# Nishad-Sharma/gpuRaytracer

Measured on AMD Instinct MI355X. Metric: Msamples/sec (pixels×spp) Cornell box 1080p at 1/2/4/8 MI355X; HBM GB/s, higher is better.
Workload: dtype f32; 1 GPU; cornell_1920x1080_256spp_b3; width=1920, height=1080, spp_per_gpu=256, spp_frame=256, bounces=3, parallelism=single GPU

## Files before the change

### gpuraytracer_amd/_native.py

```python
from __future__ import annotations

import ctypes
import os

ABI_VERSION = 11
_HERE = os.path.dirname(os.path.abspath(__file__))
library_path = os.environ.get("RTPT_LIB") or os.path.join(_HERE, "librtpt.so")


class float3(ctypes.Structure):

    _fields_ = [("x", ctypes.c_float), ("y", ctypes.c_float), ("z", ctypes.c_float),
                ("_pad", ctypes.c_float)]

    def __iter__(self):
        return iter((self.x, self.y, self.z))


class float4(ctypes.Structure):
    _fields_ = [("x", ctypes.c_float), ("y", ctypes.c_float), ("z", ctypes.c_float),
                ("w", ctypes.c_float)]


class int2(ctypes.Structure):
    _fields_ = [("x", ctypes.c_int32), ("y", ctypes.c_int32)]


class MaterialGPU(ctypes.Structure):
    _fields_ = [("diffuse", float4), ("metallic", ctypes.c_float),
                ("roughness", ctypes.c_float), ("_pad", ctypes.c_float * 2),
                ("emissive", float3)]


class SphereGPU(ctypes.Structure):
    _fields_ = [("center", float3), ("material", MaterialGPU), ("radius", ctypes.c_float),
                ("_pad", ctypes.c_float * 3)]


class CameraGPU(ctypes.Structure):
    _fields_ = [("position", float3), ("direction", float3), ("up", float3),
                ("resolution", int2), ("horizontalFov", ctypes.c_float),
                ("ev100", ctypes.c_float)]


class SquareLightGPU(ctypes.Structure):
    _fields_ = [("center", float3), ("color", float4), ("emittedRadiance", float3),
                ("width", ctypes.c_float), ("depth", ctypes.c_float),
                ("_pad", ctypes.c_float * 2)]


for _t, _n in ((float3, 16), (MaterialGPU, 48), (SphereGPU, 80), (CameraGPU, 64),
               (SquareLightGPU, 64)):
    assert ctypes.sizeof(_t) == _n, (_t.__name__, ctypes.sizeof(_t))
assert MaterialGPU.emissive.offset == 32 and SphereGPU.radius.offset == 64
assert CameraGPU.resolution.offset == 48 and CameraGPU.horizontalFov.offset == 56
assert SquareLightGPU.width.offset == 48


class SceneDesc(ctypes.Structure):
    _fields_ = [("camera", ctypes.POINTER(CameraGPU)),
                ("materials", ctypes.POINTER(MaterialGPU)),
                ("square_lights", ctypes.POINTER(SquareLightGPU)),
                ("n_square_lights", ctypes.c_uint32),
                ("vertices", ctypes.POINTER(float3)),
                ("n_triangles", ctypes.c_uint32),
                ("spheres", ctypes.POINTER(SphereGPU)),
                ("n_spheres", ctypes.c_uint32),
                ("device", ctypes.c_int32)]


class RenderParamsC(ctypes.Structure):
    _fields_ = [(n, ctypes.c_uint32) for n in
                ("spp", "bounces", "sample_base", "row_start", "row_step", "row_count",
                 "accumulate", "flags")]


class SceneInfo(ctypes.Structure):
    _fields_ = [(n, ctypes.c_uint32) for n in
                ("n_triangles", "n_triangle_pairs", "n_spheres", "lds_bytes",
                 "n_sphere_nodes", "n_triangle_bvh_nodes", "n_box_clusters", "pair_free_mask",
                 "sphere_kernel_lds_bytes", "kernel_layout", "kernel_lds_bytes")]


class CreateOptions(ctypes.Structure):
    _fields_ = [("scene_layout", ctypes.c_uint32), ("lanes_per_pixel", ctypes.c_uint32),
                ("tri_bvh_build", ctypes.c_uint32), ("tri_leaf_max", ctypes.c_uint32),
                ("tri_leaf_cost", ctypes.c_float), ("sphere_leaf_max", ctypes.c_uint32),
                ("sphere_median", ctypes.c_uint32), ("walk_scheduler", ctypes.c_uint32),
                ("walk_leaf_den", ctypes.c_uint32), ("reserved", ctypes.c_uint32 * 7)]


assert ctypes.sizeof(CreateOptions) == 64

LAYOUTS = {"auto": 0, "pairs": 1, "single": 2, "global": 3, "smem": 3, "pairsmem": 4, "sorted": 5, "bvh": 6}
TRI_BUILDS = {"default": 0, "host": 1, "lbvh": 2, "gpusah": 3}
WALKS = {"auto": 0, "lockstep": 1, "free": 2, "sorted": 3}

RT_OK = 0
RT_OUT_DEVICE, RT_OUT_FP16, RT_OUT_NONE, RT_KEEP_SUM, RT_OUT_RGBA8 = 0x1, 0x2, 0x4, 0x8, 0x10
RT_RAYS_ANY, RT_RAYS_EXACT = 0x100, 0x200
RT_AOV_CENTER = 0x400
RT_RAYS_CHUNK = 2048
RT_MAX_BOUNCES = 4
RT_COMM_ID_BYTES = 128
STATUS = {0: "RT_OK", 1: "RT_ERR_INVALID_ARG", 2: "RT_ERR_NO_DEVICE", 3: "RT_ERR_OUT_OF_MEMORY",
          4: "RT_ERR_LAUNCH", 5: "RT_ERR_STATE", 6: "RT_ERR_COMM"}

class LaunchInfo(ctypes.Structure):
    _fields_ = [("kernel", ctypes.c_char * 96)] + [(n, ctypes.c_uint32) for n in
                ("lanes_per_pixel", "halton_tables", "small_index", "block_threads", "grid_x",
                 "grid_y", "lds_bytes")]

    def as_dict(self) -> dict:
        d = {k: getattr(self, k) for k, _ in self._fields_}
        d["kernel"] = self.kernel.decode()
        return d


class BuildStats(ctypes.Structure):
    _fields_ = [("tri_bvh_build", ctypes.c_uint32), ("tri_bvh_nodes", ctypes.c_uint32),
                ("tri_bvh_build_ms", ctypes.c_float), ("scene_compile_ms", ctypes.c_float),
                ("tri_bvh_temp_kib", ctypes.c_uint32)]


class TriBvhDump(ctypes.Structure):
    _fields_ = [("n_triangles", ctypes.c_uint32), ("nodes_per_layout", ctypes.c_uint32),
                ("leaf_max", ctypes.c_uint32), ("margin", ctypes.c_float),
                ("nodes", ctypes.c_void_p), ("sorted", ctypes.c_void_p),
                ("perm", ctypes.c_void_p), ("isect", ctypes.c_void_p)]


assert ctypes.sizeof(TriBvhDump) == 48


class TileLayout(ctypes.Structure):
    _fields_ = [("rows", ctypes.c_uint32), ("rows_max", ctypes.c_uint32),
                ("row_bytes", ctypes.c_uint64), ("tile_bytes", ctypes.c_uint64)]


class Ray(ctypes.Structure):
    _fields_ = [("origin", ctypes.c_float * 3), ("tmin", ctypes.c_float),
                ("dir", ctypes.c_float * 3), ("tmax", ctypes.c_float)]


class RayHit(ctypes.Structure):
    _fields_ = [("t", ctypes.c_float), ("id", ctypes.c_int32)]


class RayDomainInfo(ctypes.Structure):
    _fields_ = [(n, ctypes.c_float) for n in ("origin_max", "dir_len2_min", "dir_len2_max", "tmax_max")]


assert ctypes.sizeof(Ray) == 32 and ctypes.sizeof(RayHit) == 8 and Ray.dir.offset == 16


class AovParams(ctypes.Structure):
    _fields_ = [(n, ctypes.c_uint32) for n in
                ("spp", "sample_base", "row_start", "row_step", "row_count", "flags")]


class AovBuffers(ctypes.Structure):
    _fields_ = [("albedo", ctypes.c_void_p), ("normal_depth", ctypes.c_void_p),
                ("first_hit", ctypes.c_void_p)]


assert ctypes.sizeof(AovParams) == 24 and ctypes.sizeof(AovBuffers) == 24


class MisParamsC(ctypes.Structure):
    _fields_ = [(n, ctypes.c_uint32) for n in
                ("camera_rays", "mis_samples", "row_start", "row_step", "row_count", "flags")]


_P = ctypes.c_void_p
SIGNATURES = {
    "rt_create": (ctypes.c_int, [ctypes.POINTER(SceneDesc), ctypes.POINTER(_P)]),
    "rt_create_ex": (ctypes.c_int, [ctypes.POINTER(SceneDesc), ctypes.POINTER(CreateOptions),
                                    ctypes.POINTER(_P)]),
    "rt_create_options_default": (None, [ctypes.POINTER(CreateOptions)]),
    "rt_set_seeds": (ctypes.c_int, [_P, _P, ctypes.c_int32, ctypes.c_int32]),
    "rt_fill_seeds": (ctypes.c_int, [_P, ctypes.c_uint64]),
    "rt_render": (ctypes.c_int, [_P, ctypes.POINTER(RenderParamsC), _P]),
    "rt_render_async": (ctypes.c_int, [_P, ctypes.POINTER(RenderParamsC), _P, _P]),
    "rt_trace_rays": (ctypes.c_int, [_P, _P, ctypes.c_uint64, ctypes.c_uint32, _P]),
    "rt_trace_rays_async": (ctypes.c_int, [_P, _P, ctypes.c_uint64, ctypes.c_uint32, _P, _P]),
    "rt_render_aov": (ctypes.c_int, [_P, ctypes.POINTER(AovParams), ctypes.POINTER(AovBuffers)]),
    "rt_render_aov_async": (ctypes.c_int, [_P, ctypes.POINTER(AovParams), ctypes.POINTER(AovBuffers), _P]),
    "rt_debug_ray_domain": (ctypes.c_int, [ctypes.POINTER(SceneDesc), ctypes.POINTER(RayDomainInfo)]),
    "rt_last_kernel_ms": (ctypes.c_int, [_P, ctypes.POINTER(ctypes.c_float)]),
    "rt_destroy": (ctypes.c_int, [_P]),
    "rt_last_launch": (ctypes.c_int, [_P, ctypes.POINTER(LaunchInfo)]),
    "rt_build_info": (ctypes.c_int, [_P, ctypes.POINTER(BuildStats)]),
    "rt_debug_tri_bvh": (ctypes.c_int, [_P, ctypes.POINTER(TriBvhDump)]),
    "rt_debug_tri_bvh_host": (ctypes.c_int, [ctypes.POINTER(SceneDesc), ctypes.POINTER(CreateOptions),
                                             ctypes.POINTER(TriBvhDump)]),
    "rt_math_selfcheck": (ctypes.c_int, [ctypes.POINTER(ctypes.c_uint64)]),
    "rt_comm_unique_id": (ctypes.c_int, [_P]),
    "rt_comm_init": (ctypes.c_int, [_P, ctypes.c_int32, ctypes.c_int32, _P]),
    "rt_render_gather": (ctypes.c_int, [_P, ctypes.POINTER(RenderParamsC), _P, _P]),
    "rt_comm_info": (ctypes.c_int, [_P, ctypes.POINTER(ctypes.c_int32), ctypes.POINTER(ctypes.c_int32)]),
    "rt_tile_layout": (ctypes.c_int, [ctypes.c_int32, ctypes.c_int32, ctypes.c_int32, ctypes.c_int32,
                                      ctypes.c_uint32, ctypes.POINTER(TileLayout)]),
    "rt_place_tiles": (ctypes.c_int, [_P, _P, ctypes.c_int32, ctypes.c_uint32, _P, _P]),
    "rt_place_tiles_host": (ctypes.c_int, [_P, ctypes.c_int32, ctypes.c_int32, ctypes.c_int32,
                                           ctypes.c_uint32, _P]),
    "rt_build_sha": (ctypes.c_char_p, []),
    "rt_debug_stats": (ctypes.c_int, [_P, _P, ctypes.c_int]),
    "rt_last_error": (ctypes.c_char_p, [_P]),
    "rt_status_string": (ctypes.c_char_p, [ctypes.c_int]),
    "rt_abi_version": (ctypes.c_int, []),
    "rt_seed_splitmix": (None, [ctypes.c_uint64, _P, ctypes.c_size_t]),
    "rt_scene_cornell_box": (ctypes.c_int, [ctypes.c_int32, ctypes.c_int32,
                                            ctypes.POINTER(CameraGPU),
                                            ctypes.POINTER(MaterialGPU),
                                            ctypes.POINTER(float3),
                                            ctypes.POINTER(SquareLightGPU),
                                            ctypes.POINTER(ctypes.c_uint32)]),
    "rt_scene_random_spheres": (ctypes.c_int, [ctypes.c_int32, ctypes.c_int32, ctypes.c_uint32,
                                               ctypes.c_uint64, ctypes.POINTER(CameraGPU),
                                               ctypes.POINTER(MaterialGPU),
                                               ctypes.POINTER(float3),
                                               ctypes.POINTER(SquareLightGPU),
                                               ctypes.POINTER(ctypes.c_uint32),
                                               ctypes.POINTER(SphereGPU)]),
    "rt_render_mis": (ctypes.c_int, [_P, ctypes.POINTER(MisParamsC), _P, _P]),
    "rt_scene_cornell_box_mis": (ctypes.c_int, [ctypes.c_int32, ctypes.c_int32,
                                                ctypes.POINTER(CameraGPU),
                                                ctypes.POINTER(MaterialGPU),
                                                ctypes.POINTER(float3),
                                                ctypes.POINTER(SquareLightGPU),
                                                ctypes.POINTER(ctypes.c_uint32)]),
    "rt_tonemap_rgba8": (None, [_P, ctypes.c_size_t, _P]),
    "rt_scene_describe": (ctypes.c_int, [ctypes.POINTER(SceneDesc), ctypes.POINTER(SceneInfo)]),
    "rt_scene_describe_ex": (ctypes.c_int, [ctypes.POINTER(SceneDesc), ctypes.POINTER(CreateOptions),
                                            ctypes.POINTER(SceneInfo)]),
    "rt_debug_camera_candidates": (ctypes.c_int, [ctypes.POINTER(SceneDesc)] + [ctypes.c_int32] * 4 + [_P]),
    "rt_debug_shadow_candidates": (ctypes.c_int, [ctypes.POINTER(SceneDesc)] + [ctypes.c_int32] * 4 +
                                   [_P, ctypes.POINTER(ctypes.c_int32)]),
    "rt_debug_cluster_kinds": (ctypes.c_int, [ctypes.POINTER(SceneDesc), ctypes.POINTER(ctypes.c_uint32),
                                              ctypes.c_uint32, ctypes.POINTER(ctypes.c_uint32)]),
    "rt_debug_light_mask": (ctypes.c_int, [ctypes.POINTER(SceneDesc), ctypes.POINTER(ctypes.c_uint64), _P,
                                           ctypes.c_uint32]),
}


class RtError(RuntimeError):

    def __init__(self, status: int, message: str):
        super().__init__(f"{STATUS.get(status, status)}: {message}")
        self.status = status


def _preload_hip_runtime():
    if os.environ.get("RTPT_SYSTEM_HIP") == "1":
        return
    import importlib.util
    spec = importlib.util.find_spec("torch")
    if spec is None or not spec.submodule_search_locations:
        return
    for d in spec.submodule_search_locations:
        cand = os.path.join(d, "lib", "libamdhip64.so")
        if os.path.exists(cand):
            ctypes.CDLL(cand, mode=ctypes.RTLD_GLOBAL)
            return


def _load():
    if not os.path.exists(library_path):
        raise ImportError(
            f"{library_path} is missing: build the HIP extension first "
            "(`make` or `python -c 'import __graft_entry__ as g; g.build()'`). "
            "There is no CPU fallback.")
    _preload_hip_runtime()
    handle = ctypes.CDLL(library_path)
    for name, (res, args) in SIGNATURES.items():
        fn = getattr(handle, name)
        fn.restype = res
        fn.argtypes = args
    if handle.rt_abi_version() != ABI_VERSION:
        raise ImportError(f"librtpt.so ABI {handle.rt_abi_version()} != {ABI_VERSION}")
    if not os.environ.get("RTPT_LIB"):
        from .srchash import have_sources, kernel_source_sha
        built = handle.rt_build_sha().decode()
        if not have_sources() or built == "unknown":
            import warnings
            warnings.warn(f"{library_path}: source hash not checked (library hash {built!r}, "
                          f"sources {'present' if have_sources() else 'absent'})")
        elif built != kernel_source_sha():
            raise ImportError(f"{library_path} was built from other sources (hash {built}, "
                              f"tree {kernel_source_sha()}): rebuild it with `make`")
    return handle


lib = _load()
```

### gpuraytracer_amd/csrc/rt_api.cpp

```cpp
#include <hip/hip_runtime.h>
#include <rccl/rccl.h>

#include <stdio.h>
#include <stdlib.h>
#include <string.h>

#include <algorithm>
#include <chrono>
#include <new>
#include <string>
#include <vector>

#include "../../include/rtpt.h"
#include "rt_beam.hpp"
#include "rt_shaft.hpp"
#include "rt_kernel.hpp"
#include "rt_scene.hpp"

constexpr uint32_t kDefaultTriBuild = RT_TRI_BVH_GPU_SAH;

struct rt_ctx {
    int device = 0;
    hipStream_t stream = nullptr;
    rt::CompiledScene scene;
    float4* d_tri_isect = nullptr;
    float4* d_tri_shade = nullptr;
    float4* d_pair_isect = nullptr;
    float4* d_clusters = nullptr;
    uint32_t* d_sph_lds = nullptr;
    uint16_t* d_sph_lds_id = nullptr;
    uint4* d_sph_box = nullptr;
    float4* d_sph_isect = nullptr;
    float4* d_sph_shade = nullptr;
    float4* d_sph_nodes = nullptr;
    uint32_t* d_sph_perm = nullptr;
    uint4* d_tri_nodes = nullptr;
    uint32_t tri_build = kDefaultTriBuild;
    float4* d_tri_sorted = nullptr;
    uint32_t* d_tri_perm = nullptr;
    uint32_t tri_bvh_nodes = 0;
    rt::SceneTables tab{};
    bool sph_compact = false;
    uint64_t light_mask = 0;
    uint32_t tri_bvh_build_used = 0;
    uint32_t tri_leaf_max = 1;
    float tri_bvh_build_ms = 0.0f;
    size_t tri_bvh_temp_bytes = 0;
    float scene_compile_ms = 0.0f;
    float4* d_mis_shade = nullptr;
    float4* d_mis_tab = nullptr;
    uint32_t mis_tab_S = 0;
    void* d_out8 = nullptr;
    size_t out8_cap = 0;
    void* d_rays = nullptr;
    size_t rays_cap = 0;
    void* d_hits = nullptr;
    size_t hits_cap = 0;
    void* d_aov[3] = {nullptr, nullptr, nullptr};
    size_t aov_cap[3] = {0, 0, 0};
    void* d_mis_part = nullptr;
    size_t mis_part_cap = 0;
    uint32_t* d_seeds = nullptr;
    bool seeds_ready = false;
    uint32_t seed_max = 0xFFFFFFFFu;
    float4* d_sum = nullptr;
    size_t sum_cap = 0;
    bool sum_valid = false;
    uint32_t sum_row_start = 0, sum_row_step = 0, sum_row_count = 0;
    uint32_t sum_first = 0, sum_samples = 0;
    void* d_out = nullptr;
    size_t out_cap = 0;
    hipEvent_t ev0 = nullptr, ev1 = nullptr;
    bool timed = false;
    rt::LaunchInfo launch{};
    bool launched = false;
    ncclComm_t comm = nullptr;
    int rank = 0, world = 1;
    void* d_tile = nullptr;
    size_t tile_cap = 0;
    void* d_gather = nullptr;
    size_t gather_cap = 0;
    hipEvent_t ev_tiles = nullptr;
    bool tiles_pending = false;
    uint32_t lanes = 0;
    rt::SceneMem scene_mem = rt::SceneMem::kAuto;
    uint32_t walk = 0;
    uint32_t walk_leaf_den = 0;
    std::string err;
};

namespace {

thread_local std::string g_create_err = "no error";

int fail(rt_ctx* ctx, int status, const std::string& msg) {
    if (ctx)
        ctx->err = msg;
    else
        g_create_err = msg;
    return status;
}

int hip_fail(rt_ctx* ctx, int status, const char* what, hipError_t e) {
    return fail(ctx, status, std::string(what) + ": " + hipGetErrorString(e));
}

struct DeviceGuard {
    int prev = -1;
    explicit DeviceGuard(int dev) {
        if (hipGetDevice(&prev) != hipSuccess) prev = -1;
        if (prev != dev) (void)hipSetDevice(dev);
    }
    ~DeviceGuard() {
        int cur = -1;
        if (prev >= 0 && hipGetDevice(&cur) == hipSuccess && cur != prev) (void)hipSetDevice(prev);
    }
};

template <typename T>
hipError_t upload(T** dptr, const void* src, size_t bytes, hipStream_t s) {
    *dptr = nullptr;
    if (bytes == 0) return hipSuccess;
    hipError_t e = hipMalloc((void**)dptr, bytes);
    if (e != hipSuccess) return e;
    e = hipMemcpyAsync(*dptr, src, bytes, hipMemcpyHostToDevice, s);
    if (e != hipSuccess) return e;
    return hipStreamSynchronize(s);
}

rt::SceneTables scene_tables(const rt::CompiledScene& s, uint32_t nTN, const rt_ctx* c) {
    rt::SceneTables t{};
    t.nT = (uint32_t)s.tri_isect.size();
    t.nP = (uint32_t)s.pair_isect.size();
    t.nS = (uint32_t)s.sph_isect.size();
    t.nN = s.sph_layout_nodes;
    t.nTN = nTN;
    t.nC = (uint32_t)(s.clusters.size() / (4 * rt::kCluF4));
    t.pair_free = s.pair_free_mask;
    if (!c) return t;
    t.tri_isect = c->d_tri_isect;
    t.pair_isect = c->d_pair_isect;
    t.clusters = c->d_clusters;
    t.sph_isect = c->d_sph_isect;
    t.sph_nodes = c->d_sph_nodes;
    t.sph_perm = c->d_sph_perm;
    t.sph_box = rt::sphere_compact_usable(s) ? c->d_sph_box : nullptr;
    t.tri_nodes = c->d_tri_nodes;
    t.tri_sorted = c->d_tri_sorted;
    t.tri_perm = c->d_tri_perm;
    return t;
}

void set_tables(rt::KParams* K, const rt::SceneTables& t) {
    K->tri_isect = t.tri_isect;
    K->pair_isect = t.pair_isect;
    K->clusters = t.clusters;
    K->sph_isect = t.sph_isect;
    K->sph_nodes = t.sph_nodes;
    K->sph_perm = t.sph_perm;
    K->sph_box = t.sph_box;
    K->tri_nodes = t.tri_nodes;
    K->tri_sorted = t.tri_sorted;
    K->tri_perm = t.tri_perm;
    K->nT = t.nT;
    K->nP = t.nP;
    K->nS = t.nS;
    K->nN = t.nN;
    K->nTN = t.nTN;
    K->nC = t.nC;
    K->pair_free = t.pair_free;
}

void release(rt_ctx* c) {
    if (!c) return;
    DeviceGuard g(c->device);
    if (c->tiles_pending) (void)hipEventSynchronize(c->ev_tiles);
    (void)hipFree(c->d_tri_isect);
    (void)hipFree(c->d_tri_shade);
    (void)hipFree(c->d_pair_isect);
    (void)hipFree(c->d_clusters);
    (void)hipFree(c->d_sph_lds);
    (void)hipFree(c->d_sph_lds_id);
    (void)hipFree(c->d_sph_box);
    (void)hipFree(c->d_sph_isect);
    (void)hipFree(c->d_sph_shade);
    (void)hipFree(c->d_sph_nodes);
    (void)hipFree(c->d_sph_perm);
    (void)hipFree(c->d_tri_nodes);
    (void)hipFree(c->d_tri_sorted);
    (void)hipFree(c->d_tri_perm);
    (void)hipFree(c->d_mis_shade);
    (void)hipFree(c->d_mis_tab);
    (void)hipFree(c->d_out8);
    (void)hipFree(c->d_mis_part);
    (void)hipFree(c->d_rays);
    (void)hipFree(c->d_hits);
    for (void* b : c->d_aov) (void)hipFree(b);
    (void)hipFree(c->d_seeds);
    (void)hipFree(c->d_sum);
    (void)hipFree(c->d_out);
    if (c->comm) (void)ncclCommDestroy(c->comm);
    (void)hipFree(c->d_tile);
    (void)hipFree(c->d_gather);
    if (c->ev_tiles) (void)hipEventDestroy(c->ev_tiles);
    if (c->ev0) (void)hipEventDestroy(c->ev0);
    if (c->ev1) (void)hipEventDestroy(c->ev1);
    if (c->stream) (void)hipStreamDestroy(c->stream);
}

bool resolve_rows(const rt_ctx* c, const rt_render_params* p, uint32_t* start, uint32_t* step,
                  uint32_t* count) {
    const uint32_t H = (uint32_t)c->scene.cam.H;
    *start = p->row_start;
    *step = p->row_step ? p->row_step : 1u;
    if (*start >= H) return false;
    const uint32_t avail = (H - 1u - *start) / *step + 1u;
    *count = p->row_count ? p->row_count : avail;
    return *count <= avail;
}

int render_impl(rt_ctx* c, const rt_render_params* p, void* out, bool out_is_device,
                hipStream_t stream, bool sync) {
    if (!p) return fail(c, RT_ERR_INVALID_ARG, "params is null");
    if (p->bounces > RT_MAX_BOUNCES)
        return fail(c, RT_ERR_INVALID_ARG,
                    "bounces > 4: Halton dimensions would leave primes[24] (sampling.metal:97)");
    if (!c->seeds_ready) return fail(c, RT_ERR_STATE, "seeds not set (rt_set_seeds/rt_fill_seeds)");
    uint32_t start, step, count;
    if (!resolve_rows(c, p, &start, &step, &count))
        return fail(c, RT_ERR_INVALID_ARG, "row partition outside the frame");
    const bool want_out = !(p->flags & RT_OUT_NONE);
    const bool keep_sum = (p->flags & RT_KEEP_SUM) != 0;
    if (want_out && !out) return fail(c, RT_ERR_INVALID_ARG, "out is null");
    if (p->accumulate) {
        if (!c->sum_valid || c->sum_row_start != start || c->sum_row_step != step ||
            c->sum_row_count != count ||
            (uint64_t)c->sum_first + c->sum_samples != (uint64_t)p->sample_base)
            return fail(c, RT_ERR_STATE,
                        "accumulate: context sum does not end at sample_base for these rows "
                        "(render with RT_KEEP_SUM first)");
    }
    const uint64_t total = (uint64_t)(p->accumulate ? c->sum_samples : 0u) + p->spp;
    if (total == 0 || total > 0xFFFFFFFFull)
        return fail(c, RT_ERR_INVALID_ARG, "samples in the sum must be in [1, 2^32)");

    const size_t W = (size_t)c->scene.cam.W;
    const size_t pixels = (size_t)count * W;
    if ((p->flags & RT_OUT_FP16) && (p->flags & RT_OUT_RGBA8))
        return fail(c, RT_ERR_INVALID_ARG, "RT_OUT_FP16 and RT_OUT_RGBA8 are exclusive");
    const size_t px_bytes = (p->flags & RT_OUT_RGBA8) ? 4u : (p->flags & RT_OUT_FP16) ? 8u : 16u;
    hipError_t e;
    if (keep_sum || p->accumulate) {
        if (c->sum_cap < pixels) {
            (void)hipFree(c->d_sum);
            c->d_sum = nullptr;
            c->sum_cap = 0;
            c->sum_valid = false;
            if ((e = hipMalloc((void**)&c->d_sum, pixels * sizeof(float4))) != hipSuccess)
                return hip_fail(c, RT_ERR_OUT_OF_MEMORY, "hipMalloc(sum)", e);
            c->sum_cap = pixels;
        }
    }
    void* kout = nullptr;
    if (want_out) {
        if (out_is_device) {
            kout = out;
        } else {
            if (c->out_cap < pixels * px_bytes) {
                (void)hipFree(c->d_out);
                c->d_out = nullptr;
                c->out_cap = 0;
                if ((e = hipMalloc(&c->d_out, pixels * px_bytes)) != hipSuccess)
                    return hip_fail(c, RT_ERR_OUT_OF_MEMORY, "hipMalloc(out staging)", e);
                c->out_cap = pixels * px_bytes;
            }
            kout = c->d_out;
        }
    }

    rt::KParams K;
    memset(&K, 0, sizeof(K));
    set_tables(&K, c->tab);
    K.tri_shade = c->d_tri_shade;
    K.light_mask = c->light_mask;
    K.sph_lds = c->sph_compact ? c->d_sph_lds : nullptr;
    K.sph_lds_id = c->d_sph_lds_id;
    K.sph_shade = c->d_sph_shade;
    K.seeds = c->d_seeds;
    K.sum = (keep_sum || p->accumulate) ? c->d_sum : nullptr;
    K.out = kout;
    K.nE = c->scene.sph_lds_entries;
    const rt::CamConst& cam = c->scene.cam;
    memcpy(K.cam_pos, cam.pos, sizeof(K.cam_pos));
    memcpy(K.cam_u, cam.u, sizeof(K.cam_u));
    memcpy(K.cam_v, cam.v, sizeof(K.cam_v));
    memcpy(K.cam_w, cam.w, sizeof(K.cam_w));
    K.halfW = cam.halfW;
    K.halfH = cam.halfH;
    K.W = cam.W;
    K.H = cam.H;
    memcpy(K.light_center, c->scene.light.center, sizeof(K.light_center));
    {
        uint32_t by, bz;
        memcpy(&by, &K.light_center[1], 4);
        memcpy(&bz, &K.light_center[2], 4);
        K.light_plain = (by != 0x80000000u && bz != 0x80000000u) ? 1u : 0u;
    }
    memcpy(K.light_color, c->scene.light.color, sizeof(K.light_color));
    K.spp = p->spp;
    K.sample_base = p->sample_base;
    K.row_start = start;
    K.row_step = step;
    K.row_count = count;
    K.accumulate = p->accumulate ? 1u : 0u;
    K.samples_total = (uint32_t)total;
    K.flags = ((p->flags & RT_OUT_FP16) ? rt::kOutFp16 : 0u) | ((p->flags & RT_OUT_RGBA8) ? rt::kOutRgba8 : 0u);
    K.lanes = c->lanes;
    K.walk = c->walk;
    K.walk_leaf_den = c->walk_leaf_den;
    {
        const uint64_t imax = (uint64_t)c->seed_max + p->sample_base + (p->spp ? p->spp - 1u : 0u);
        K.max_index = imax > 0xFFFFFFFFull ? 0xFFFFFFFFu : (uint32_t)imax;
    }

    if (keep_sum && !p->accumulate) c->sum_valid = false;
    (void)hipEventRecord(c->ev0, stream);
    e = rt::launch_path_trace(K, p->bounces, c->scene_mem, stream, &c->launch);
    if (e != hipSuccess) return hip_fail(c, RT_ERR_LAUNCH, "path_trace launch", e);
    c->launched = true;
    (void)hipEventRecord(c->ev1, stream);
    c->timed = true;
    if (keep_sum || p->accumulate) {
        c->sum_valid = true;
        c->sum_row_start = start;
        c->sum_row_step = step;
        c->sum_row_count = count;
        if (!p->accumulate) c->sum_first = p->sample_base;
        c->sum_samples = (uint32_t)total;
    }
    if (want_out && !out_is_device) {
        if ((e = hipMemcpyAsync(out, kout, pixels * px_bytes, hipMemcpyDeviceToHost, stream)) !=
            hipSuccess)
            return hip_fail(c, RT_ERR_LAUNCH, "hipMemcpyAsync(out)", e);
    }
    if (sync) {
        if ((e = hipStreamSynchronize(stream)) != hipSuccess)
            return hip_fail(c, RT_ERR_LAUNCH, "path_trace execution", e);
        uint32_t short_end = 0;
        if (rt::lds_check_result(&short_end) == hipSuccess && short_end)
            return fail(c, RT_ERR_LAUNCH, "LDS overflow: staged records end at byte " + std::to_string(short_end) +
                                              ", past the dispatch's dynamic LDS");
    }
    return RT_OK;
}

int ensure_staging(rt_ctx* c, void** buf, size_t* cap, size_t bytes, const char* what);

int nccl_fail(rt_ctx* ctx, const char* what, ncclResult_t r) {
    return fail(ctx, RT_ERR_COMM, std::string(what) + ": " + ncclGetErrorString(r));
}

size_t pixel_bytes(uint32_t flags) {
    return (flags & RT_OUT_RGBA8) ? 4u : (flags & RT_OUT_FP16) ? 8u : 16u;
}

struct TileLayout {
    uint32_t rows, rows_max;
    size_t row_bytes, tile_bytes;
};

TileLayout tile_layout(uint32_t W, uint32_t H, uint32_t N, uint32_t rank, uint32_t flags) {
    TileLayout L;
    L.rows = rank < H ? (H - 1u - rank) / N + 1u : 0u;
    L.rows_max = (H + N - 1u) / N;
    L.row_bytes = (size_t)W * pixel_bytes(flags);
    L.tile_bytes = (size_t)L.rows_max * L.row_bytes;
    return L;
}

bool tile_args_ok(int32_t W, int32_t H, int32_t N) { return W > 0 && H > 0 && N > 0; }

int place_tiles_impl(rt_ctx* c, const void* gathered, uint32_t N, uint32_t flags, void* frame,
                     hipStream_t stream) {
    const uint32_t W = (uint32_t)c->scene.cam.W, H = (uint32_t)c->scene.cam.H;
    const TileLayout L = tile_layout(W, H, N, 0, flags);
    const bool dev = (flags & RT_OUT_DEVICE) != 0;
    const size_t frame_bytes = (size_t)H * L.row_bytes;
    void* dst = frame;
    int st;
    if (!dev) {
        if ((st = ensure_staging(c, &c->d_out, &c->out_cap, frame_bytes, "hipMalloc(frame staging)")) != RT_OK)
            return st;
        dst = c->d_out;
    }
    hipError_t e = rt::launch_place_tiles(gathered, dst, L.row_bytes, L.tile_bytes, H, N, stream);
    if (e != hipSuccess) return hip_fail(c, RT_ERR_LAUNCH, "place_tiles launch", e);
    if (!dev) {
        if ((e = hipStreamSynchronize(stream)) != hipSuccess ||
            (e = hipMemcpyAsync(frame, dst, frame_bytes, hipMemcpyDeviceToHost, stream)) != hipSuccess ||
            (e = hipStreamSynchronize(stream)) != hipSuccess)
            return hip_fail(c, RT_ERR_LAUNCH, "frame copy to host", e);
    }
    return RT_OK;
}

int render_gather_impl(rt_ctx* c, const rt_render_params* p, void* frame, hipStream_t stream) {
    if (!p) return fail(c, RT_ERR_INVALID_ARG, "params is null");
    if (!c->comm) return fail(c, RT_ERR_STATE, "no communicator (rt_comm_init)");
    if (p->row_start || p->row_step > 1 || p->row_count)
        return fail(c, RT_ERR_INVALID_ARG, "rt_render_gather partitions the rows itself: "
                                           "params must name the whole frame (row_start 0, "
                                           "row_step 0 or 1, row_count 0)");
    if ((p->flags & RT_OUT_FP16) && (p->flags & RT_OUT_RGBA8))
        return fail(c, RT_ERR_INVALID_ARG, "RT_OUT_FP16 and RT_OUT_RGBA8 are exclusive");
    const bool want_out = !(p->flags & RT_OUT_NONE);
    const bool dev = (p->flags & RT_OUT_DEVICE) != 0;
    if (want_out && c->rank == 0 && !frame) return fail(c, RT_ERR_INVALID_ARG, "frame is null on rank 0");
    const uint32_t H = (uint32_t)c->scene.cam.H, W = (uint32_t)c->scene.cam.W, N = (uint32_t)c->world;
    const TileLayout L = tile_layout(W, H, N, (uint32_t)c->rank, p->flags);
    hipError_t e;
    if (c->tiles_pending && (e = hipStreamWaitEvent(stream, c->ev_tiles, 0)) != hipSuccess)
        return hip_fail(c, RT_ERR_LAUNCH, "hipStreamWaitEvent(previous gather)", e);
    int st;
    if (want_out && (st = ensure_staging(c, &c->d_tile, &c->tile_cap, L.tile_bytes, "hipMalloc(tile)")) != RT_OK)
        return st;
    if (L.rows > 0) {
        rt_render_params q = *p;
        q.row_start = (uint32_t)c->rank;
        q.row_step = N;
        q.row_count = L.rows;
        q.flags = p->flags | RT_OUT_DEVICE;
        if ((st = render_impl(c, &q, c->d_tile, true, stream, false)) != RT_OK) return st;
    }
    if (!want_out) return RT_OK;
    if (c->rank == 0 && (st = ensure_staging(c, &c->d_gather, &c->gather_cap, L.tile_bytes * N,
                                             "hipMalloc(gather)")) != RT_OK)
        return st;
// ... 348 lines not shown

int rt_abi_version(void) { return RTPT_ABI_VERSION; }

const char* rt_status_string(int s) {
    switch (s) {
        case RT_OK: return "RT_OK";
        case RT_ERR_INVALID_ARG: return "RT_ERR_INVALID_ARG";
        case RT_ERR_NO_DEVICE: return "RT_ERR_NO_DEVICE";
        case RT_ERR_OUT_OF_MEMORY: return "RT_ERR_OUT_OF_MEMORY";
        case RT_ERR_LAUNCH: return "RT_ERR_LAUNCH";
        case RT_ERR_STATE: return "RT_ERR_STATE";
        case RT_ERR_COMM: return "RT_ERR_COMM";
        default: return "RT_ERR_UNKNOWN";
    }
}

const char* rt_last_error(const rt_ctx* ctx) {
    return ctx ? ctx->err.c_str() : g_create_err.c_str();
}

int rt_create(const rt_scene_desc* d, rt_ctx** out_ctx) { return rt_create_ex(d, nullptr, out_ctx); }

int rt_create_ex(const rt_scene_desc* d, const rt_create_options* opt, rt_ctx** out_ctx) {
    if (!out_ctx) return fail(nullptr, RT_ERR_INVALID_ARG, "out_ctx is null");
    *out_ctx = nullptr;
    if (!d) return fail(nullptr, RT_ERR_INVALID_ARG, "scene desc is null");
    if (!d->camera) return fail(nullptr, RT_ERR_INVALID_ARG, "camera is null");
    if (!d->square_lights || d->n_square_lights < 1)
        return fail(nullptr, RT_ERR_INVALID_ARG, "square_lights[0] is required (raytrace.metal:22)");
    Resolved ro;
    const char* why = nullptr;
    if (!resolve_options(opt, &ro, &why)) return fail(nullptr, RT_ERR_INVALID_ARG, why);
    int count = 0;
    hipError_t e = hipGetDeviceCount(&count);
    if (e != hipSuccess || count <= 0)
        return fail(nullptr, RT_ERR_NO_DEVICE,
                    std::string("no HIP device: ") + (e != hipSuccess ? hipGetErrorString(e) : "count 0"));
    if (d->device < 0 || d->device >= count)
        return fail(nullptr, RT_ERR_NO_DEVICE, "device ordinal out of range");

    rt_ctx* c = new (std::nothrow) rt_ctx();
    if (!c) return fail(nullptr, RT_ERR_OUT_OF_MEMORY, "host allocation");
    c->device = d->device;
    c->lanes = ro.lanes;
    c->tri_build = ro.tri_build;
    c->scene_mem = ro.mem;
    c->walk = ro.walk;
    c->walk_leaf_den = ro.walk_leaf_den;
    DeviceGuard g(c->device);
    const char* err = nullptr;
    using clk = std::chrono::steady_clock;
    const auto t_compile = clk::now();
    if (!rt::compile_scene(*d->camera, d->materials, d->vertices, d->n_triangles,
                           d->square_lights[0], d->spheres, d->n_spheres, &c->scene, &err, ro.build)) {
        delete c;
        return fail(nullptr, RT_ERR_INVALID_ARG, err);
    }
    c->scene_compile_ms = std::chrono::duration<float, std::milli>(clk::now() - t_compile).count();
    int status = RT_OK;
    std::string msg;
    do {
        if ((e = hipStreamCreateWithFlags(&c->stream, hipStreamNonBlocking)) != hipSuccess) {
            status = RT_ERR_NO_DEVICE; msg = std::string("hipStreamCreate: ") + hipGetErrorString(e); break;
        }
        if ((e = hipEventCreate(&c->ev0)) != hipSuccess || (e = hipEventCreate(&c->ev1)) != hipSuccess ||
            (e = hipEventCreateWithFlags(&c->ev_tiles, hipEventDisableTiming)) != hipSuccess) {
            status = RT_ERR_NO_DEVICE; msg = std::string("hipEventCreate: ") + hipGetErrorString(e); break;
        }
        const rt::CompiledScene& s = c->scene;
        if ((e = upload(&c->d_tri_isect, s.tri_isect.data(), s.tri_isect.size() * sizeof(rt::TriIsect), c->stream)) != hipSuccess ||
            (e = upload(&c->d_tri_shade, s.tri_shade.data(), s.tri_shade.size() * sizeof(rt::TriShade), c->stream)) != hipSuccess ||
            (e = upload(&c->d_pair_isect, s.pair_isect.data(), s.pair_isect.size() * sizeof(rt::PairIsect), c->stream)) != hipSuccess ||
            (e = upload(&c->d_clusters, s.clusters.data(), s.clusters.size() * sizeof(float), c->stream)) != hipSuccess ||
            (e = upload(&c->d_sph_lds, s.sph_lds.data(), s.sph_lds.size() * sizeof(uint32_t), c->stream)) != hipSuccess ||
            (e = upload(&c->d_sph_lds_id, s.sph_lds_id.data(), s.sph_lds_id.size() * sizeof(uint16_t), c->stream)) != hipSuccess ||
            (e = upload(&c->d_sph_box, s.sph_box.data(), s.sph_box.size() * sizeof(uint32_t), c->stream)) != hipSuccess ||
            (e = upload(&c->d_sph_isect, s.sph_isect.data(), s.sph_isect.size() * sizeof(rt::SphIsect), c->stream)) != hipSuccess ||
            (e = upload(&c->d_sph_shade, s.sph_shade.data(), s.sph_shade.size() * sizeof(rt::SphShade), c->stream)) != hipSuccess ||
            (e = upload(&c->d_sph_nodes, s.sph_nodes.data(), s.sph_nodes.size() * sizeof(rt::BvhNode), c->stream)) != hipSuccess ||
            (e = upload(&c->d_sph_perm, s.sph_perm.data(), s.sph_perm.size() * sizeof(uint32_t), c->stream)) != hipSuccess ||
            (e = upload(&c->d_mis_shade, s.mis_shade.data(), s.mis_shade.size() * sizeof(rt::MisShade), c->stream)) != hipSuccess) {
            status = RT_ERR_OUT_OF_MEMORY; msg = std::string("scene upload: ") + hipGetErrorString(e); break;
        }
        const uint32_t nT = (uint32_t)s.tri_isect.size();
        const size_t lds_pairs = rt::kernel_lds_bytes(nT, (uint32_t)s.pair_isect.size(), 0, 0);
        const size_t lds_single = rt::kernel_lds_bytes(nT, 0, 0, 0);
        const bool need_bvh = nT > 0 && (c->scene_mem == rt::SceneMem::kTriBvh ||
                                         (c->scene_mem == rt::SceneMem::kAuto &&
                                          (nT > rt::kTriBvhMinTriangles ||
                                           std::min(lds_pairs, lds_single) > rt::kMaxLdsBytes)));
        if (need_bvh) {
            const size_t nn = 2 * (size_t)nT - 1;
            const auto t_build = clk::now();
            if (c->tri_build == RT_TRI_BVH_GPU_SAH) {
                if ((e = hipMalloc((void**)&c->d_tri_nodes, rt::kTriCompactLayouts * nn * sizeof(uint4))) != hipSuccess ||
                    (e = hipMalloc((void**)&c->d_tri_sorted, 3 * (size_t)nT * sizeof(float4))) != hipSuccess ||
                    (e = hipMalloc((void**)&c->d_tri_perm, (size_t)nT * sizeof(uint32_t))) != hipSuccess) {
                    status = RT_ERR_OUT_OF_MEMORY; msg = std::string("hipMalloc(triangle BVH): ") + hipGetErrorString(e); break;
                }
                uint32_t total = 0;
                size_t temp = 0;
                if ((e = rt::build_tri_gsah(c->d_tri_isect, nT, s.margin, ro.tri_leaf_max, ro.tri_leaf_cost,
                                            c->d_tri_nodes, c->d_tri_sorted, c->d_tri_perm, &total, &temp,
                                            c->stream)) != hipSuccess) {
                    status = (e == hipErrorInvalidValue) ? RT_ERR_INVALID_ARG
                             : (e == hipErrorOutOfMemory) ? RT_ERR_OUT_OF_MEMORY : RT_ERR_LAUNCH;
                    msg = std::string("triangle BVH build: ") + hipGetErrorString(e); break;
                }
                c->tri_bvh_nodes = total;
                c->tri_bvh_temp_bytes = temp;
            } else if (c->tri_build == RT_TRI_BVH_GPU_LBVH) {
                if ((e = hipMalloc((void**)&c->d_tri_nodes, rt::kTriCompactLayouts * nn * sizeof(uint4))) != hipSuccess ||
                    (e = hipMalloc((void**)&c->d_tri_sorted, 3 * (size_t)nT * sizeof(float4))) != hipSuccess ||
                    (e = hipMalloc((void**)&c->d_tri_perm, (size_t)nT * sizeof(uint32_t))) != hipSuccess) {
                    status = RT_ERR_OUT_OF_MEMORY; msg = std::string("hipMalloc(triangle BVH): ") + hipGetErrorString(e); break;
                }
                if ((e = rt::build_tri_lbvh(c->d_tri_isect, nT, s.tri_lo, s.tri_hi, s.margin, c->d_tri_nodes,
                                            c->d_tri_sorted, c->d_tri_perm, c->stream)) != hipSuccess) {
                    status = (e == hipErrorInvalidValue) ? RT_ERR_INVALID_ARG : RT_ERR_LAUNCH;
                    msg = std::string("triangle BVH build: ") + hipGetErrorString(e); break;
                }
            } else {
                std::vector<uint32_t> nodes, perm;
                std::vector<rt::TriIsect> sorted;
                if (!rt::build_tri_sah(s.tri_isect, s.margin, &nodes, &sorted, &perm, ro.tri_leaf_max,
                                       ro.tri_leaf_cost)) {
                    status = RT_ERR_INVALID_ARG; msg = "triangle BVH build: too many triangles (2^24)"; break;
                }
                if ((e = upload(&c->d_tri_nodes, nodes.data(), nodes.size() * sizeof(uint32_t), c->stream)) != hipSuccess ||
                    (e = upload(&c->d_tri_sorted, sorted.data(), sorted.size() * sizeof(rt::TriIsect), c->stream)) != hipSuccess ||
                    (e = upload(&c->d_tri_perm, perm.data(), perm.size() * sizeof(uint32_t), c->stream)) != hipSuccess) {
                    status = RT_ERR_OUT_OF_MEMORY; msg = std::string("triangle BVH upload: ") + hipGetErrorString(e); break;
                }
                c->tri_bvh_nodes = (uint32_t)(nodes.size() / (4 * rt::kTriCompactLayouts));
            }
            if (c->tri_build == RT_TRI_BVH_GPU_LBVH) c->tri_bvh_nodes = (uint32_t)nn;
            c->tri_leaf_max = c->tri_build == RT_TRI_BVH_GPU_LBVH ? 1u : std::min(128u, std::max(1u, ro.tri_leaf_max));
            c->tri_bvh_build_used = c->tri_build;
            c->tri_bvh_build_ms = std::chrono::duration<float, std::milli>(clk::now() - t_build).count();
        }
        const size_t npx = (size_t)s.cam.W * (size_t)s.cam.H;
        if ((e = hipMalloc((void**)&c->d_seeds, npx * sizeof(uint32_t))) != hipSuccess) {
            status = RT_ERR_OUT_OF_MEMORY; msg = std::string("hipMalloc(seeds): ") + hipGetErrorString(e); break;
        }
    } while (0);
    if (status != RT_OK) {
        release(c);
        delete c;
        return fail(nullptr, status, msg);
    }
    c->sph_compact = rt::sphere_compact_usable(c->scene);
    c->tab = scene_tables(c->scene, c->tri_bvh_nodes, c);
    c->light_mask = rt::light_mask(c->scene);
    *out_ctx = c;
    return RT_OK;
}

int rt_set_seeds(rt_ctx* c, const uint32_t* seeds, int32_t width, int32_t height) {
    if (!c) return fail(nullptr, RT_ERR_INVALID_ARG, "ctx is null");
    if (!seeds) return fail(c, RT_ERR_INVALID_ARG, "seeds is null");
    if (width != c->scene.cam.W || height != c->scene.cam.H)
        return fail(c, RT_ERR_INVALID_ARG, "seed texture size must equal the camera resolution");
    DeviceGuard g(c->device);
    const size_t bytes = (size_t)width * (size_t)height * sizeof(uint32_t);
    hipError_t e = hipMemcpyAsync(c->d_seeds, seeds, bytes, hipMemcpyHostToDevice, c->stream);
    if (e == hipSuccess) e = hipStreamSynchronize(c->stream);
    if (e != hipSuccess) return hip_fail(c, RT_ERR_LAUNCH, "seed upload", e);
    uint32_t mx = 0;
    for (size_t k = 0, n = (size_t)width * (size_t)height; k < n; ++k) mx = seeds[k] > mx ? seeds[k] : mx;
    c->seed_max = mx;
    c->seeds_ready = true;
    return RT_OK;
}

int rt_fill_seeds(rt_ctx* c, uint64_t key) {
    if (!c) return fail(nullptr, RT_ERR_INVALID_ARG, "ctx is null");
    DeviceGuard g(c->device);
    const uint64_t n = (uint64_t)c->scene.cam.W * (uint64_t)c->scene.cam.H;
    hipError_t e = rt::launch_fill_seeds(c->d_seeds, key, n, c->stream);
    if (e == hipSuccess) e = hipStreamSynchronize(c->stream);
    if (e != hipSuccess) return hip_fail(c, RT_ERR_LAUNCH, "fill_seeds", e);
    c->seed_max = 0xFFFFFu;
    c->seeds_ready = true;
    return RT_OK;
}

int rt_render(rt_ctx* c, const rt_render_params* p, void* out) {
    if (!c) return fail(nullptr, RT_ERR_INVALID_ARG, "ctx is null");
    DeviceGuard g(c->device);
    const bool dev = p && (p->flags & RT_OUT_DEVICE);
    return render_impl(c, p, out, dev, c->stream, true);
}

int rt_render_async(rt_ctx* c, const rt_render_params* p, void* out_device, void* hip_stream) {
    if (!c) return fail(nullptr, RT_ERR_INVALID_ARG, "ctx is null");
    DeviceGuard g(c->device);
    return render_impl(c, p, out_device, true, (hipStream_t)hip_stream, false);
}

int rt_trace_rays(rt_ctx* c, const rt_ray* rays, uint64_t n, uint32_t flags, rt_ray_hit* hits) {
    if (!c) return fail(nullptr, RT_ERR_INVALID_ARG, "ctx is null");
    DeviceGuard g(c->device);
    return trace_rays_impl(c, rays, n, flags, hits, (flags & RT_OUT_DEVICE) != 0, c->stream, true);
}

int rt_trace_rays_async(rt_ctx* c, const rt_ray* rays_dev, uint64_t n, uint32_t flags, rt_ray_hit* hits_dev,
                        void* hip_stream) {
    if (!c) return fail(nullptr, RT_ERR_INVALID_ARG, "ctx is null");
    DeviceGuard g(c->device);
    return trace_rays_impl(c, rays_dev, n, flags, hits_dev, true, (hipStream_t)hip_stream, false);
}

int rt_render_aov(rt_ctx* c, const rt_aov_params* p, const rt_aov_buffers* b) {
    if (!c) return fail(nullptr, RT_ERR_INVALID_ARG, "ctx is null");
    DeviceGuard g(c->device);
    return render_aov_impl(c, p, b, p && (p->flags & RT_OUT_DEVICE), c->stream, true);
}

int rt_render_aov_async(rt_ctx* c, const rt_aov_params* p, const rt_aov_buffers* b_dev, void* hip_stream) {
    if (!c) return fail(nullptr, RT_ERR_INVALID_ARG, "ctx is null");
    DeviceGuard g(c->device);
    return render_aov_impl(c, p, b_dev, true, (hipStream_t)hip_stream, false);
}

int rt_debug_ray_domain(const rt_scene_desc* d, rt_ray_domain_info* info) {
    if (!d || !info || !d->camera || !d->square_lights)
        return fail(nullptr, RT_ERR_INVALID_ARG, "null argument");
    rt::CompiledScene s;
    const char* err = nullptr;
    if (!rt::compile_scene(*d->camera, d->materials, d->vertices, d->n_triangles, d->square_lights[0],
                           d->spheres, d->n_spheres, &s, &err))
        return fail(nullptr, RT_ERR_INVALID_ARG, err);
    const rt::RayDomain D = rt::ray_domain(s.extent);
    info->origin_max = D.origin_max;
    info->dir_len2_min = D.dir_len2_min;
    info->dir_len2_max = D.dir_len2_max;
    info->tmax_max = D.tmax_max;
    return RT_OK;
}

int rt_last_kernel_ms(rt_ctx* c, float* ms) {
    if (!c || !ms) return fail(c, RT_ERR_INVALID_ARG, "null argument");
    if (!c->timed) return fail(c, RT_ERR_STATE, "no render or ray query yet");
    DeviceGuard g(c->device);
    hipError_t e = hipEventSynchronize(c->ev1);
    if (e == hipSuccess) e = hipEventElapsedTime(ms, c->ev0, c->ev1);
    if (e != hipSuccess) return hip_fail(c, RT_ERR_LAUNCH, "hipEventElapsedTime", e);
    return RT_OK;
}

int rt_comm_unique_id(uint8_t id[RT_COMM_ID_BYTES]) {
    if (!id) return fail(nullptr, RT_ERR_INVALID_ARG, "id is null");
    static_assert(sizeof(ncclUniqueId) == RT_COMM_ID_BYTES, "ncclUniqueId size");
    ncclUniqueId u;
    const ncclResult_t r = ncclGetUniqueId(&u);
    if (r != ncclSuccess) return nccl_fail(nullptr, "ncclGetUniqueId", r);
    memcpy(id, &u, sizeof(u));
    return RT_OK;
}

int rt_comm_init(rt_ctx* c, int32_t rank, int32_t world, const uint8_t id[RT_COMM_ID_BYTES]) {
    if (!c) return fail(nullptr, RT_ERR_INVALID_ARG, "ctx is null");
    if (!id) return fail(c, RT_ERR_INVALID_ARG, "id is null");
    if (world < 1 || rank < 0 || rank >= world)
        return fail(c, RT_ERR_INVALID_ARG, "need 0 <= rank < world");
    if (c->comm) return fail(c, RT_ERR_STATE, "context already has a communicator");
    DeviceGuard g(c->device);
    ncclUniqueId u;
    memcpy(&u, id, sizeof(u));
    ncclComm_t comm = nullptr;
    const ncclResult_t r = ncclCommInitRank(&comm, world, u, rank);
    if (r != ncclSuccess) return nccl_fail(c, "ncclCommInitRank", r);
    c->comm = comm;
    c->rank = rank;
    c->world = world;
    return RT_OK;
}

int rt_render_gather(rt_ctx* c, const rt_render_params* p, void* frame, void* hip_stream) {
    if (!c) return fail(nullptr, RT_ERR_INVALID_ARG, "ctx is null");
    DeviceGuard g(c->device);
    hipStream_t s = (hipStream_t)hip_stream;
    return render_gather_impl(c, p, frame, s);
}

int rt_comm_info(const rt_ctx* c, int32_t* count, int32_t* rank) {
    if (!c || !count || !rank) return fail(nullptr, RT_ERR_INVALID_ARG, "null argument");
    rt_ctx* m = const_cast<rt_ctx*>(c);
    if (!c->comm) return fail(m, RT_ERR_STATE, "rt_comm_info: no communicator (rt_comm_init first)");
    int n = 0, r = 0;
    ncclResult_t res = ncclCommCount(c->comm, &n);
    if (res != ncclSuccess) return nccl_fail(m, "ncclCommCount", res);
    res = ncclCommUserRank(c->comm, &r);
    if (res != ncclSuccess) return nccl_fail(m, "ncclCommUserRank", res);
    *count = n;
    *rank = r;
    return RT_OK;
}

int rt_tile_layout(int32_t width, int32_t height, int32_t world, int32_t rank, uint32_t flags,
                   rt_tile_layout_info* out) {
    if (!out || !tile_args_ok(width, height, world) || rank < 0 || rank >= world)
        return RT_ERR_INVALID_ARG;
    const TileLayout L = tile_layout((uint32_t)width, (uint32_t)height, (uint32_t)world, (uint32_t)rank, flags);
    out->rows = L.rows;
    out->rows_max = L.rows_max;
// ... 111 lines not shown
    info->halton_tables = c->launch.tables;
    info->small_index = c->launch.small;
    info->block_threads = c->launch.threads;
    info->grid_x = c->launch.grid_x;
    info->grid_y = c->launch.grid_y;
    info->lds_bytes = c->launch.lds;
    return RT_OK;
}

#ifndef RT_SRC_SHA
#define RT_SRC_SHA "unknown"
#endif
const char* rt_build_sha(void) { return RT_SRC_SHA; }

int rt_destroy(rt_ctx* c) {
    if (!c) return RT_OK;
    release(c);
    delete c;
    return RT_OK;
}

int rt_scene_describe(const rt_scene_desc* d, rt_scene_info* info) {
    return rt_scene_describe_ex(d, nullptr, info);
}

int rt_scene_describe_ex(const rt_scene_desc* d, const rt_create_options* opt, rt_scene_info* info) {
    if (!d || !info || !d->camera || !d->square_lights)
        return fail(nullptr, RT_ERR_INVALID_ARG, "null argument");
    Resolved ro;
    const char* why = nullptr;
    if (!resolve_options(opt, &ro, &why)) return fail(nullptr, RT_ERR_INVALID_ARG, why);
    rt::CompiledScene s;
    const char* err = nullptr;
    if (!rt::compile_scene(*d->camera, d->materials, d->vertices, d->n_triangles,
                           d->square_lights[0], d->spheres, d->n_spheres, &s, &err, ro.build))
        return fail(nullptr, RT_ERR_INVALID_ARG, err);
    rt::SceneTables t = scene_tables(s, 0, nullptr);
    info->n_triangles = t.nT;
    info->n_triangle_pairs = t.nP;
    info->n_box_clusters = t.nC;
    info->pair_free_mask = t.pair_free;
    info->n_spheres = t.nS;
    info->n_sphere_nodes = t.nN;
    const size_t lds = rt::kernel_lds_bytes(info->n_triangles, info->n_triangle_pairs, info->n_spheres,
                                            s.sph_layout_nodes);
    const size_t lds_single = rt::kernel_lds_bytes(info->n_triangles, 0, 0, 0);
    const bool bvh = info->n_triangles > 0 &&
                     (ro.mem == rt::SceneMem::kTriBvh ||
                      (ro.mem == rt::SceneMem::kAuto && (info->n_triangles > rt::kTriBvhMinTriangles ||
                                                         std::min(lds, lds_single) > rt::kMaxLdsBytes)));
    info->n_triangle_bvh_nodes = t.nTN = bvh ? 2 * info->n_triangles - 1 : 0u;
    info->sphere_kernel_lds_bytes = (rt::sphere_compact_usable(s) && info->n_triangle_pairs > 0 && !bvh &&
                                     ro.mem == rt::SceneMem::kAuto && lds <= rt::kSphPairLdsMaxBytes)
                                        ? (uint32_t)lds
                                        : 0u;
    const size_t lds_clu =
        lds + (t.nS ? 0u : 16 * rt::staged_f4<size_t>(rt::kLayPairClu, t.nT, t.nP, t.nC).clu);
    info->lds_bytes = (!bvh && lds <= rt::kMaxLdsBytes)
                          ? (uint32_t)(lds_clu <= rt::kMaxLdsBytes ? lds_clu : lds)
                          : 0u;
    const rt::KernelChoice kc = rt::choose_kernel(t, rt::sphere_compact_usable(s), 3, ro.mem, ro.walk);
    info->kernel_layout = (uint32_t)kc.layout;
    info->kernel_lds_bytes = (uint32_t)kc.lds_bytes;
    return RT_OK;
}

int rt_debug_camera_candidates(const rt_scene_desc* d, int32_t x0, int32_t x1, int32_t y0, int32_t y1,
                               uint8_t* may_hit) {
    if (!d || !may_hit || !d->camera || !d->square_lights || x1 < x0 || y1 < y0 || x0 < 0 || y0 < 0)
        return fail(nullptr, RT_ERR_INVALID_ARG, "null argument or empty rectangle");
    rt::CompiledScene s;
    const char* err = nullptr;
    if (!rt::compile_scene(*d->camera, d->materials, d->vertices, d->n_triangles, d->square_lights[0],
                           d->spheres, d->n_spheres, &s, &err))
        return fail(nullptr, RT_ERR_INVALID_ARG, err);
    memset(may_hit, 1, d->n_triangles);
    const rt::CamConst& c = s.cam;
    const rt::Beam beam = rt::make_beam(rt::f3{c.pos[0], c.pos[1], c.pos[2]}, rt::f3{c.u[0], c.u[1], c.u[2]},
                                        rt::f3{c.v[0], c.v[1], c.v[2]}, rt::f3{c.w[0], c.w[1], c.w[2]}, c.halfW,
                                        c.halfH, (float)c.W, (float)c.H, (float)(uint32_t)x0, (float)(uint32_t)x1,
                                        (float)(uint32_t)y0, (float)(uint32_t)y1);
    for (size_t k = 0; k < s.pair_isect.size(); ++k)
        if (rt::beam_excludes_pair(beam, s.pair_isect[k].q)) may_hit[2 * k] = may_hit[2 * k + 1] = 0;
    return RT_OK;
}

int rt_debug_shadow_candidates(const rt_scene_desc* d, int32_t x0, int32_t x1, int32_t y0, int32_t y1,
                               uint8_t* may_occlude, int32_t* available) {
    if (!d || !may_occlude || !available || !d->camera || !d->square_lights || x1 < x0 || y1 < y0 || x0 < 0 ||
        y0 < 0)
        return fail(nullptr, RT_ERR_INVALID_ARG, "null argument or empty rectangle");
    rt::CompiledScene s;
    const char* err = nullptr;
    if (!rt::compile_scene(*d->camera, d->materials, d->vertices, d->n_triangles, d->square_lights[0],
                           d->spheres, d->n_spheres, &s, &err))
        return fail(nullptr, RT_ERR_INVALID_ARG, err);
    memset(may_occlude, 1, d->n_triangles);
    *available = 0;
    const size_t nP = s.pair_isect.size();
    if (nP == 0) return RT_OK;
    const rt::CamConst& c = s.cam;
    const rt::Beam beam = rt::make_beam(rt::f3{c.pos[0], c.pos[1], c.pos[2]}, rt::f3{c.u[0], c.u[1], c.u[2]},
                                        rt::f3{c.v[0], c.v[1], c.v[2]}, rt::f3{c.w[0], c.w[1], c.w[2]}, c.halfW,
                                        c.halfH, (float)c.W, (float)c.H, (float)(uint32_t)x0, (float)(uint32_t)x1,
                                        (float)(uint32_t)y0, (float)(uint32_t)y1);
    const rt::ShaftLight L = rt::shaft_light(rt::f3{s.light.center[0], s.light.center[1], s.light.center[2]});
    std::vector<uint8_t> keep(nP, 0);
    bool ok = true;
    for (size_t k = 0; k < nP; ++k) {
        if (rt::beam_excludes_pair(beam, s.pair_isect[k].q)) continue;
        for (int tb = 0; tb < 2; ++tb) {
            const float* sh = s.tri_shade[2 * k + tb].s;
            if (sh[3] != 0.0f) continue;
            const rt::ShaftSrc S = rt::shaft_source(beam, s.pair_isect[k].q, tb, rt::f3{sh[0], sh[1], sh[2]}, L);
            ok = ok && S.ok;
            for (size_t j = 0; j < nP; ++j)
                if (!rt::shaft_excludes_pair(S, L, s.pair_isect[j].q)) keep[j] = 1;
        }
    }
    if (!ok) return RT_OK;
    *available = 1;
    for (size_t j = 0; j < nP; ++j) may_occlude[2 * j] = may_occlude[2 * j + 1] = keep[j];
    return RT_OK;
}

int rt_debug_cluster_kinds(const rt_scene_desc* d, uint32_t* flags, uint32_t capacity, uint32_t* n_clusters) {
    if (!d || !n_clusters || (!flags && capacity) || !d->camera || !d->square_lights)
        return fail(nullptr, RT_ERR_INVALID_ARG, "null argument");
    rt::CompiledScene s;
    const char* err = nullptr;
    if (!rt::compile_scene(*d->camera, d->materials, d->vertices, d->n_triangles, d->square_lights[0],
                           d->spheres, d->n_spheres, &s, &err))
        return fail(nullptr, RT_ERR_INVALID_ARG, err);
    const size_t rec = 4 * rt::kCluF4, nC = s.clusters.size() / rec;
    *n_clusters = (uint32_t)nC;
    for (size_t c = 0; c < nC && c < capacity; ++c) memcpy(&flags[c], &s.clusters[c * rec + 15], 4);
    return RT_OK;
}

int rt_debug_light_mask(const rt_scene_desc* d, uint64_t* mask, float* records, uint32_t capacity_triangles) {
    if (!d || !mask || (!records && capacity_triangles) || !d->camera || !d->square_lights)
        return fail(nullptr, RT_ERR_INVALID_ARG, "null argument");
    rt::CompiledScene s;
    const char* err = nullptr;
    if (!rt::compile_scene(*d->camera, d->materials, d->vertices, d->n_triangles, d->square_lights[0],
                           d->spheres, d->n_spheres, &s, &err))
        return fail(nullptr, RT_ERR_INVALID_ARG, err);
    *mask = rt::light_mask(s);
    for (size_t k = 0; k < s.tri_shade.size() && k < capacity_triangles; ++k)
        memcpy(records + 16 * k, s.tri_shade[k].s, sizeof(s.tri_shade[k].s));
    return RT_OK;
}

int rt_debug_stats(rt_ctx* c, uint64_t* out, int n) {
    if (!c || !out || n <= 0) return fail(c, RT_ERR_INVALID_ARG, "null argument");
    DeviceGuard g(c->device);
    hipError_t e = rt::read_debug_stats(reinterpret_cast<unsigned long long*>(out), n);
    if (e == hipErrorNotSupported) return fail(c, RT_ERR_STATE, "not an RT_STATS build");
    if (e != hipSuccess) return hip_fail(c, RT_ERR_LAUNCH, "read stats", e);
    return RT_OK;
}

void rt_seed_splitmix(uint64_t key, uint32_t* seeds, size_t n) {
    if (!seeds) return;
    for (size_t p = 0; p < n; ++p) seeds[p] = rt::seed_splitmix(key, p);
}

static void fill_scene_arrays(const rt::Scene& s, CameraGPU* camera, MaterialGPU* materials,
                              rt_float3* vertices, SquareLightGPU* light) {
    *camera = rt::convert_camera(s.camera);
    for (size_t k = 0; k < s.triangles.size(); ++k) {
        materials[k] = rt::convert_material(s.triangles[k].material);
        for (int v = 0; v < 3; ++v) vertices[3 * k + v] = rt::to_abi(s.triangles[k].vertices[v]);
    }
    *light = rt::convert_square_light(s.light);
}

int rt_scene_cornell_box(int32_t width, int32_t height, CameraGPU* camera, MaterialGPU* materials,
                         rt_float3* vertices, SquareLightGPU* light, uint32_t* n_triangles) {
    if (!camera || !materials || !vertices || !light || !n_triangles || width <= 0 || height <= 0)
        return RT_ERR_INVALID_ARG;
    const rt::Scene s = rt::init_cornell_box(width, height);
    fill_scene_arrays(s, camera, materials, vertices, light);
    *n_triangles = (uint32_t)s.triangles.size();
    return RT_OK;
}

int rt_render_mis(rt_ctx* ctx, const rt_mis_params* params, float* out_rgba32f, uint8_t* out_rgba8) {
    if (!ctx) return fail(nullptr, RT_ERR_INVALID_ARG, "ctx is null");
    DeviceGuard g(ctx->device);
    return render_mis_impl(ctx, params, out_rgba32f, out_rgba8);
}

int rt_scene_cornell_box_mis(int32_t width, int32_t height, CameraGPU* camera, MaterialGPU* materials,
                             rt_float3* vertices, SquareLightGPU* light, uint32_t* n_triangles) {
    if (!camera || !materials || !vertices || !light || !n_triangles || width <= 0 || height <= 0)
        return RT_ERR_INVALID_ARG;
    const rt::Scene s = rt::init_cornell_box_mis(width, height);
    fill_scene_arrays(s, camera, materials, vertices, light);
    *n_triangles = (uint32_t)s.triangles.size();
    return RT_OK;
}

int rt_scene_random_spheres(int32_t width, int32_t height, uint32_t n_spheres, uint64_t seed,
                            CameraGPU* camera, MaterialGPU* materials, rt_float3* vertices,
                            SquareLightGPU* light, uint32_t* n_triangles, SphereGPU* spheres) {
    if (!camera || !materials || !vertices || !light || !n_triangles || width <= 0 ||
        height <= 0 || (n_spheres && !spheres))
        return RT_ERR_INVALID_ARG;
    const rt::Scene s = rt::init_random_spheres(width, height, n_spheres, seed);
    fill_scene_arrays(s, camera, materials, vertices, light);
    *n_triangles = (uint32_t)s.triangles.size();
    for (uint32_t k = 0; k < n_spheres; ++k) spheres[k] = rt::convert_sphere(s.spheres[k]);
    return RT_OK;
}

}
```

### gpuraytracer_amd/csrc/rt_halton.hpp

```cpp
#pragma once
#include <hip/hip_runtime.h>

#include "rt_kernel.hpp"

namespace rt {
namespace {

constexpr uint32_t kPrimes[24] = RT_PRIMES_INIT;

template <uint32_t D>
__device__ __forceinline__ float halton(uint32_t i) {
    static_assert(D < 24, "Halton dimension outside primes[]");
    constexpr uint32_t b = kPrimes[D];
    constexpr float invB = 1.0f / (float)b;
    float f = 1.0f;
    float r = 0.0f;
    while (i > 0) {
        f = f * invB;
        r = r + f * (float)(i % b);
        i = i / b;
    }
    return r;
}

constexpr int halton_digits(uint32_t b, uint64_t imax) {
    uint64_t cap = 1;
    int n = 0;
    while (cap < imax) {
        cap *= b;
        ++n;
    }
    return n;
}

constexpr float recip_up(uint32_t n) {
    float c = 1.0f / (float)n;
    if ((double)c * (double)n < 1.0) c = __builtin_bit_cast(float, __builtin_bit_cast(uint32_t, c) + 1u);
    return c;
}

template <uint32_t b>
__device__ __forceinline__ float digit_step(float x, float& digit) {
    constexpr float c = recip_up(b);
    const float q = __builtin_floorf(x * c);
    digit = __builtin_fmaf(q, -(float)b, x);
    return q;
}

constexpr uint32_t kSmallIndexMax = 1594323;
constexpr int kSmallIndexBits = 21;
static_assert(kSmallIndexMax <= (1u << kSmallIndexBits), "float digit steps need x < 2^21");
template <uint32_t D>
__device__ __forceinline__ float halton_small(uint32_t i) {
    constexpr uint32_t b = kPrimes[D];
    if constexpr (b == 2) {
        return (float)(__builtin_bitreverse32(i) >> (32 - kSmallIndexBits)) *
               (1.0f / (float)(1u << kSmallIndexBits));
    } else {
        constexpr int nd = halton_digits(b, kSmallIndexMax);
        constexpr float invB = 1.0f / (float)b;
        float x = (float)i;
        float f = 1.0f;
        float r = 0.0f;
#pragma unroll
        for (int k = 0; k < nd; ++k) {
            f = f * invB;
            float digit;
            x = digit_step<b>(x, digit);
            r = r + f * digit;
        }
        return r;
    }
}

constexpr int kTabDigits[24] = {0, 6, 4, 3, 2, 2, 0, 2, 2, 2, 2, 0, 0, 0, 0, 0, 0, 0, 0, 0, 0, 0, 0, 0};
constexpr uint32_t ipow(uint32_t b, int k) { return k == 0 ? 1u : b * ipow(b, k - 1); }
constexpr uint32_t tab_size(int D) { return kTabDigits[D] ? ipow(kPrimes[D], kTabDigits[D]) : 0u; }
constexpr uint32_t tab_offset(int D) { return D == 0 ? 0u : tab_offset(D - 1) + tab_size(D - 1); }
constexpr uint32_t kHaltonTabFloats = tab_offset(24);
constexpr float f_after(uint32_t b, int k) {
    float f = 1.0f;
    for (int j = 0; j < k; ++j) f = f * (1.0f / (float)b);
    return f;
}

template <uint32_t D>
__device__ __forceinline__ void fill_halton_table(float* tab, uint32_t tid, uint32_t nthreads) {
    constexpr uint32_t b = kPrimes[D];
    constexpr int k = kTabDigits[D];
    constexpr float invB = 1.0f / (float)b;
    constexpr uint32_t off = tab_offset(D), size = tab_size(D);
    for (uint32_t v0 = tid; v0 < size; v0 += nthreads) {
        uint32_t v = v0;
        float f = 1.0f;
        float r = 0.0f;
#pragma unroll
        for (int j = 0; j < k; ++j) {
            f = f * invB;
            r = r + f * (float)(v % b);
            v = v / b;
        }
        tab[off + v0] = r;
    }
}

__device__ __forceinline__ void fill_halton_tables(float* tab, uint32_t tid, uint32_t nthreads) {
    fill_halton_table<1>(tab, tid, nthreads);
    fill_halton_table<2>(tab, tid, nthreads);
    fill_halton_table<3>(tab, tid, nthreads);
    fill_halton_table<4>(tab, tid, nthreads);
    fill_halton_table<5>(tab, tid, nthreads);
    fill_halton_table<7>(tab, tid, nthreads);
    fill_halton_table<8>(tab, tid, nthreads);
    fill_halton_table<9>(tab, tid, nthreads);
    fill_halton_table<10>(tab, tid, nthreads);
    static_assert(kHaltonTabFloats == 729 + 625 + 343 + 121 + 169 + 361 + 529 + 841 + 961,
                  "table list");
}

template <uint32_t D>
__device__ __forceinline__ float halton_tab(uint32_t i, const float* tab) {
    constexpr uint32_t b = kPrimes[D];
    constexpr int k = kTabDigits[D];
    constexpr int nd = halton_digits(b, kSmallIndexMax);
    constexpr float invB = 1.0f / (float)b;
    constexpr uint32_t bk = ipow(b, k), off = tab_offset(D);
    static_assert(k > 0 && k < nd, "dimension without a table");
    float low;
    float x = digit_step<bk>((float)i, low);
    float r = tab[off + (uint32_t)low];
    constexpr float fk = f_after(b, k);
    float f = fk;
#pragma unroll
    for (int j = k; j < nd; ++j) {
        f = f * invB;
        float digit;
        x = digit_step<b>(x, digit);
        r = r + f * digit;
    }
    return r;
}

template <uint32_t D, bool SMALL, bool TAB = false>
__device__ __forceinline__ float halton_dim(uint32_t i, const float* tab = nullptr) {
    if constexpr (TAB && SMALL && kTabDigits[D] > 0)
        if (tab != nullptr) return halton_tab<D>(i, tab);
    if (SMALL) return halton_small<D>(i);
    return halton<D>(i);
}

}
}
```

### gpuraytracer_amd/csrc/rt_kernel.hip

```cpp
#include <hip/hip_runtime.h>
#include <hip/hip_fp16.h>

#include <stddef.h>
#include <stdio.h>
#ifdef RT_LDS_CHECK
#include <hsa/hsa.h>
#endif

#include "rt_kernel.hpp"
#include "rt_halton.hpp"
#include "rt_beam.hpp"
#include "rt_shaft.hpp"
#include "rt_pixel.hpp"
#include "rt_trace.hpp"

namespace rt {

#ifdef RT_LDS_CHECK
__device__ uint32_t g_lds_overflow;
__device__ __forceinline__ bool lds_short(size_t end) {
    const uint32_t grp = ((const uint32_t*)__builtin_amdgcn_dispatch_ptr())[7];
    const size_t dyn = grp - __builtin_amdgcn_groupstaticsize();
    if (end <= dyn) return false;
    if (threadIdx.x == 0) atomicMax(&g_lds_overflow, (uint32_t)end);
    return true;
}
static_assert(offsetof(hsa_kernel_dispatch_packet_t, group_segment_size) == 28, "AQL packet layout");
#define RT_LDS_GUARD(end)            \
    do {                             \
        if (lds_short(end)) return;  \
    } while (0)
#else
#define RT_LDS_GUARD(end) ((void)0)
#endif

namespace {

#ifndef RT_CENSUS
#define RT_CENSUS 0
#endif
template <typename T>
__device__ __forceinline__ T cz(T v) {
    asm volatile("" : "+v"(v));
    return v;
}
__device__ __forceinline__ f3 cz(f3 v) { return f3{cz(v.x), cz(v.y), cz(v.z)}; }
__device__ __forceinline__ void cz_sink(float v) { asm volatile("" ::"v"(v)); }
__device__ __forceinline__ void cz_sink(f3 v) {
    cz_sink(v.x);
    cz_sink(v.y);
    cz_sink(v.z);
}

struct PathState {
    f3 o, d, acc, thr;
    uint32_t i;
};

template <int b, int B, int GEO, bool SPH, bool SMALL, bool FUSE = false, bool STASH = false>
__device__ __forceinline__ bool shade(const KParams& P, const SceneView& sv, PathState& s, int id,
                                      float t, int* nid = nullptr, float* nt = nullptr) {
    f3 N, right, fwd, diffuse;
    if constexpr (GEO == kGeoPairClu && !SPH) {
        if ((P.light_mask >> (uint32_t)id) & 1ull) {
            const float4 s3 = P.tri_shade[4 * id + 3];
            s.acc = f3{s3.x, s3.y, s3.z};
            return false;
        }
        const float4* sh = P.tri_shade + 4 * id;
        const float4 s0 = sh[0], s1 = sh[1], s2 = sh[2];
        N = f3{s0.x, s0.y, s0.z};
        right = f3{s1.x, s1.y, s1.z};
        fwd = f3{s2.x, s2.y, s2.z};
        diffuse = f3{s1.w, s2.w, sh[3].w};
    } else if (!SPH || (uint32_t)id < sv.nT) {
        const float4* sh = P.tri_shade + 4 * id;
        const float4 s0 = sh[0];
        const float4 s3 = sh[3];
        if (s0.w != 0.0f) {
            s.acc = f3{s3.x, s3.y, s3.z};
            return false;
        }
        const float4 s1 = sh[1], s2 = sh[2];
        N = f3{s0.x, s0.y, s0.z};
        right = f3{s1.x, s1.y, s1.z};
        fwd = f3{s2.x, s2.y, s2.z};
        diffuse = f3{s1.w, s2.w, s3.w};
    } else {
        const uint32_t k = (uint32_t)id - sv.nT;
        const float4* sh = P.sph_shade + 3 * k;
        const float4 s0 = sh[0];
        if (s0.w != 0.0f) {
            const float4 s1 = sh[1];
            s.acc = f3{s1.x, s1.y, s1.z};
            return false;
        }
        const float4 S = sh[2];
        N = normalize((s.o + s.d * t) - f3{S.x, S.y, S.z});
        shading_frame(N, &right, &fwd);
        diffuse = f3{s0.x, s0.y, s0.z};
    }
    f3 p = (s.o + s.d * t) + N * 1e-3f;

#if RT_CENSUS == 4
    {
        const uint32_t i2 = cz(s.i);
        float h = halton_dim<2 + 5 * b, SMALL, GEO == kGeoPairClu>(i2, sv.htab) +
                  halton_dim<3 + 5 * b, SMALL, GEO == kGeoPairClu>(i2, sv.htab);
        if (b + 1 < B)
            h = h + halton_dim<4 + 5 * b, SMALL, GEO == kGeoPairClu>(i2, sv.htab) +
                halton_dim<5 + 5 * b, SMALL, GEO == kGeoPairClu>(i2, sv.htab);
        cz_sink(h);
    }
#endif
    const float ux = halton_dim<2 + 5 * b, SMALL, GEO == kGeoPairClu>(s.i, sv.htab) * 2.0f - 1.0f;
    const float uy = halton_dim<3 + 5 * b, SMALL, GEO == kGeoPairClu>(s.i, sv.htab) * 2.0f - 1.0f;
#if RT_CENSUS == 5
    {
        const f3 o2 = cz(s.o), dd = cz(s.d), N2 = cz(N), r2 = cz(right), f2 = cz(fwd), df = cz(diffuse);
        const float t2 = cz(t), ux2 = cz(ux), uy2 = cz(uy);
        const f3 p2 = (o2 + dd * t2) + N2 * 1e-3f;
        const f3 q2 = (ld_f3(P.light_center) + f3{0.25f, 0.0f, 0.0f} * ux2) + f3{0.0f, 0.0f, 0.25f} * uy2;
        f3 L2 = q2 - p2;
        const float dist2 = length(L2);
        const float inv2 = 1.0f / fmaxf(dist2, 1e-3f);
        L2 = L2 * inv2;
        f3 lc2 = ld_f3(P.light_color) * (inv2 * inv2);
        lc2 = lc2 * saturate(dot(-L2, f3{0.0f, -1.0f, 0.0f}));
        lc2 = lc2 * saturate(dot(N2, L2));
        const f3 c2 = lc2 * (cz(s.thr) * df);
        cz_sink(c2);
        cz_sink(f3{fminf(p2.x, q2.x), fminf(p2.y, q2.y), fminf(p2.z, q2.z)});
        cz_sink(f3{fmaxf(p2.x, q2.x), fmaxf(p2.y, q2.y), fmaxf(p2.z, q2.z)});
        if (b + 1 < B) {
            float sp2, cp2;
            sincos_pt(6.28318548f * cz(ux), &sp2, &cp2);
            const float ct2 = sqrtf(cz(uy));
            const float st2 = sqrtf(1.0f - ct2 * ct2);
            cz_sink((r2 * (st2 * cp2) + N2 * ct2) + f2 * (st2 * sp2));
        }
    }
#endif
    const f3 lcen = ld_f3(P.light_center);
    f3 q;
    if (P.light_plain)
        q = f3{lcen.x + 0.25f * ux, lcen.y, lcen.z + 0.25f * uy};
    else
        q = (lcen + f3{0.25f, 0.0f, 0.0f} * ux) + f3{0.0f, 0.0f, 0.25f} * uy;
    f3 L = q - p;
    constexpr bool CR = GEO != kGeoTriBvh;
    const float dist = CR ? length(L) : length_ieee(L);
    const float inv = CR ? rcp_cr(fmaxf(dist, 1e-3f)) : 1.0f / fmaxf(dist, 1e-3f);
    L = L * inv;
    f3 lc = ld_f3(P.light_color) * (inv * inv);
    lc = lc * saturate(L.y);
    lc = lc * saturate(dot(N, L));
    s.thr = s.thr * diffuse;
    const f3 contrib = lc * s.thr;
    const f3 seg_lo{fminf(p.x, q.x), fminf(p.y, q.y), fminf(p.z, q.z)};
    const f3 seg_hi{fmaxf(p.x, q.x), fmaxf(p.y, q.y), fmaxf(p.z, q.z)};
    f3 d2{0.0f, 0.0f, 0.0f};
    if (b + 1 < B) {
        const float cu = halton_dim<4 + 5 * b, SMALL, GEO == kGeoPairClu>(s.i, sv.htab);
        const float cv = halton_dim<5 + 5 * b, SMALL, GEO == kGeoPairClu>(s.i, sv.htab);
        float sp, cp;
        sincos_pt(6.28318548f * cu, &sp, &cp);
        const float ct = CR ? sqrt_cr(cv) : sqrtf(cv);
        const float st = CR ? sqrt_cr(1.0f - ct * ct) : sqrtf(1.0f - ct * ct);
        d2 = (right * (st * cp) + N * ct) + fwd * (st * sp);
    }
    if (FUSE && b + 1 < B) {
        const FusedHit h = fused_shadow_closest(sv, p, L, dist - 1e-3f, seg_lo, seg_hi, d2);
        if (!h.occluded) s.acc = s.acc + contrib;
        s.d = d2;
        s.o = p;
        *nid = h.id;
        *nt = h.t;
        return true;
    }
    const bool lit = (GEO == kGeoTriBvh && b == 0) || contrib.x != 0.0f || contrib.y != 0.0f ||
                     contrib.z != 0.0f;
    if constexpr (STASH) {
        constexpr uint32_t SS = kSphBlockThreads;
        uint32_t t = threadIdx.x;
        asm volatile("" : "+v"(t));
        float* st = sv.xstash;
        st[t] = contrib.x;
        st[SS + t] = contrib.y;
        st[2 * SS + t] = contrib.z;
        if (b + 1 < B) {
            st[3 * SS + t] = d2.x;
            st[4 * SS + t] = d2.y;
            st[5 * SS + t] = d2.z;
        }
        const bool occluded =
            lit && any_hit<GEO, SPH, b == 0 && !SPH>(sv, p, L, 0.0f, dist - 1e-3f, seg_lo, seg_hi);
        uint32_t t2 = threadIdx.x;
        asm volatile("" : "+v"(t2));
        if (lit && !occluded)
            s.acc = s.acc + f3{st[t2], st[SS + t2], st[2 * SS + t2]};
        if (b + 1 < B) {
            s.d = f3{st[3 * SS + t2], st[4 * SS + t2], st[5 * SS + t2]};
            s.o = p;
        }
        return true;
    }
#if RT_CENSUS == 3
    if (lit) {
        f3 p2 = cz(p), L2 = cz(L);
        cz_sink(any_hit<GEO, SPH, b == 0 && !SPH>(sv, p2, L2, 0.0f, cz(dist) - 1e-3f, cz(seg_lo), cz(seg_hi)) ? 1.0f
                                                                                                            : 0.0f);
    }
#endif
    if (lit && !any_hit<GEO, SPH, b == 0 && !SPH>(sv, p, L, 0.0f, dist - 1e-3f, seg_lo, seg_hi))
        s.acc = s.acc + contrib;
    if (b + 1 < B) {
        s.d = d2;
        s.o = p;
    }
    return true;
}

template <int b, int B, int GEO, bool SPH, bool SMALL>
__device__ __forceinline__ bool bounce(const KParams& P, const SceneView& sv, PathState& s) {
    float t = 1000.0f;
    const int id = closest_hit<GEO, SPH, b == 0, (b == 0 ? 0 : 1)>(sv, s.o, s.d, 0.001f, &t);
#if RT_CENSUS == 2
    {
        f3 o2 = cz(s.o), d2 = cz(s.d);
        float t2 = cz(1000.0f);
        const int id2 = closest_hit<GEO, SPH, b == 0, (b == 0 ? 0 : 1)>(sv, o2, d2, 0.001f, &t2);
        cz_sink(t2 + (float)id2);
    }
#endif
    if (id < 0) return false;
    return shade<b, B, GEO, SPH, SMALL, false, GEO == kGeoSphLds>(P, sv, s, id, t);
}

template <int b, int B, int GEO, bool SPH, bool SMALL>
struct BounceChain {
    __device__ __forceinline__ static void run(const KParams& P, const SceneView& sv,
                                               PathState& s) {
#ifdef RT_STATS
        if constexpr (!SPH && GEO != kGeoTriBvh) {
            const unsigned long long t0 = clock64();
            const unsigned long long live = (unsigned long long)__popcll(__ballot(1));
            const bool ok = bounce<b, B, GEO, SPH, SMALL>(P, sv, s);
            const unsigned long long dt = clock64() - t0;
            RT_STAT(16 + b, dt);
            RT_STAT(20 + b, dt * live);
            if (!ok) return;
            BounceChain<b + 1, B, GEO, SPH, SMALL>::run(P, sv, s);
            return;
        }
#endif
        if (!bounce<b, B, GEO, SPH, SMALL>(P, sv, s)) return;
        BounceChain<b + 1, B, GEO, SPH, SMALL>::run(P, sv, s);
    }
};
template <int B, int GEO, bool SPH, bool SMALL>
struct BounceChain<B, B, GEO, SPH, SMALL> {
    __device__ __forceinline__ static void run(const KParams&, const SceneView&, PathState&) {}
};

template <int b, int B, int GEO, bool SMALL>
struct FusedChain {
    __device__ __forceinline__ static void run(const KParams& P, const SceneView& sv,
                                               PathState& s, int id, float t) {
        int nid = -1;
        float nt = 0.0f;
        if (!shade<b, B, GEO, false, SMALL, true>(P, sv, s, id, t, &nid, &nt)) return;
        if (b + 1 < B && nid >= 0) FusedChain<b + 1, B, GEO, SMALL>::run(P, sv, s, nid, nt);
    }
};
template <int B, int GEO, bool SMALL>
struct FusedChain<B, B, GEO, SMALL> {
    __device__ __forceinline__ static void run(const KParams&, const SceneView&, PathState&, int,
                                               float) {}
};

template <int B, int GEO, bool SPH, bool SMALL>
__device__ __forceinline__ void trace_path(const KParams& P, const SceneView& sv, PathState& s) {
    if (geo_pairs(GEO) && !SPH && B > 1) {
        float t = 1000.0f;
        const int id = closest_hit<GEO, false, true, 0>(sv, s.o, s.d, 0.001f, &t);
        if (id >= 0) FusedChain<0, B, GEO, SMALL>::run(P, sv, s, id, t);
    } else {
        BounceChain<0, B, GEO, SPH, SMALL>::run(P, sv, s);
    }
}

template <int k>
__device__ __forceinline__ float row_shl(float v) {
    if constexpr (k == 0) {
        return v;
    } else {
        return __int_as_float(__builtin_amdgcn_update_dpp(0, __float_as_int(v), 0x100 + k, 0xF, 0xF, false));
    }
}
template <int L, int k>
struct row_sum_in_order {
    __device__ __forceinline__ static void run(f3& acc, f3 c, uint32_t n0, uint32_t spp) {
        if (n0 + (uint32_t)k < spp)
            acc = acc + f3{row_shl<k>(c.x), row_shl<k>(c.y), row_shl<k>(c.z)};
        row_sum_in_order<L, k + 1>::run(acc, c, n0, spp);
    }
};
template <int L>
struct row_sum_in_order<L, L> {
    __device__ __forceinline__ static void run(f3&, f3, uint32_t, uint32_t) {}
};

__device__ __forceinline__ void store_pixel(const KParams& P, size_t o, float r, float g, float b) {
    if (P.flags & kOutRgba8) {
        const uint8_t cr = tonemap_channel(__half2float(__float2half_rn(r)));
        const uint8_t cg = tonemap_channel(__half2float(__float2half_rn(g)));
        const uint8_t cb = tonemap_channel(__half2float(__float2half_rn(b)));
        reinterpret_cast<uchar4*>(P.out)[o] = make_uchar4(cr, cg, cb, 255);
    } else if (P.flags & kOutFp16) {
        ushort4 h;
        h.x = __half_as_ushort(__float2half_rn(r));
        h.y = __half_as_ushort(__float2half_rn(g));
        h.z = __half_as_ushort(__float2half_rn(b));
        h.w = __half_as_ushort(__float2half_rn(1.0f));
        reinterpret_cast<ushort4*>(P.out)[o] = h;
    } else {
        reinterpret_cast<float4*>(P.out)[o] = make_float4(r, g, b, 1.0f);
    }
}

__device__ __forceinline__ void finish_pixel(const KParams& P, size_t o, f3 lum) {
    if (P.sum) P.sum[o] = make_float4(lum.x, lum.y, lum.z, (float)P.samples_total);
    if (P.out) {
        const float fs = (float)P.samples_total;
        const float r = lum.x / fs, g = lum.y / fs, bl = lum.z / fs;
        store_pixel(P, o, r, g, bl);
    }
}

constexpr uint32_t kSortBuckets = 9;
constexpr uint32_t kSortA = 0;
constexpr uint32_t kSortB = kBlockThreads;
constexpr uint32_t kSortC = 2 * kBlockThreads;
constexpr uint32_t kSortD = 3 * kBlockThreads;
constexpr uint32_t kSortLum = kSortD + kBlockThreads / 2;
constexpr uint32_t kSortCnt = kSortLum + 3 * kBlockThreads / 4;
constexpr uint32_t kSortF4 = kSortCnt + (kSortBuckets * 4 + 3) / 4;

__device__ __forceinline__ uint32_t sort_octant(f3 d) {
    return (d.x > 0.0f ? 4u : 0u) | (d.y > 0.0f ? 2u : 0u) | (d.z > 0.0f ? 1u : 0u);
}

__device__ __forceinline__ void sort_paths(float4* lds, PathState& s, uint32_t& owner,
                                           bool& alive) {
    const uint32_t tid = threadIdx.x, wave = tid >> 6, lane = tid & 63u;
    uint32_t* counts = reinterpret_cast<uint32_t*>(lds + kSortCnt);
    const uint32_t key = alive ? sort_octant(s.d) : 8u;
    uint32_t my_count = 0, slot = 0;
#pragma unroll
    for (uint32_t k = 0; k < kSortBuckets - 1; ++k) {
        const unsigned long long m = __ballot(key == k);
        if (lane == k) my_count = (uint32_t)__popcll(m);
        if (key == k) slot = (uint32_t)__popcll(m & ((1ull << lane) - 1ull));
    }
    if (lane < kSortBuckets - 1) counts[lane * 4u + wave] = my_count;
    __syncthreads();
    const uint32_t idx = lane & 31u;
    const uint32_t c = counts[idx];
    uint32_t v = c;
#pragma unroll
    for (uint32_t off = 1; off < 32; off <<= 1) {
        const uint32_t t = __shfl_up(v, off);
        if (idx >= off) v += t;
    }
    const uint32_t live = __shfl(v, 31);
    slot += __shfl(v - c, (int)(key * 4u + wave));
    if (alive) {
        lds[kSortA + slot] = make_float4(s.o.x, s.o.y, s.o.z, s.thr.x);
        lds[kSortB + slot] = make_float4(s.d.x, s.d.y, s.d.z, s.thr.y);
        lds[kSortC + slot] = make_float4(s.acc.x, s.acc.y, s.acc.z, s.thr.z);
        reinterpret_cast<uint2*>(lds + kSortD)[slot] = make_uint2(s.i, owner);
    }
    s.thr = f3{0.0f, 0.0f, 0.0f};
    s.acc = f3{0.0f, 0.0f, 0.0f};
    __syncthreads();
    alive = tid < live;
    if (alive) {
        const float4 a = lds[kSortA + tid], bq = lds[kSortB + tid];
        const uint2 dd = reinterpret_cast<const uint2*>(lds + kSortD)[tid];
        s.o = f3{a.x, a.y, a.z};
        s.d = f3{bq.x, bq.y, bq.z};
        s.i = dd.x;
        owner = dd.y;
    }
}

__device__ __forceinline__ void load_thr_acc(const float4* lds, PathState& s) {
    const uint32_t tid = threadIdx.x;
    const float4 c = lds[kSortC + tid];
    s.thr = f3{lds[kSortA + tid].w, lds[kSortB + tid].w, c.w};
    s.acc = f3{c.x, c.y, c.z};
}

__device__ __forceinline__ void deliver(float4* lds, uint32_t owner, f3 acc) {
    float* sum = reinterpret_cast<float*>(lds + kSortLum);
    sum[owner] = sum[owner] + acc.x;
    sum[kBlockThreads + owner] = sum[kBlockThreads + owner] + acc.y;
    sum[2 * kBlockThreads + owner] = sum[2 * kBlockThreads + owner] + acc.z;
}

template <int b, int B, int GEO, bool SPH, bool SMALL>
struct SortedChain {
    __device__ __forceinline__ static void run(const KParams& P, const SceneView& sv, float4* lds,
                                               PathState& s, uint32_t& owner, bool& alive) {
        if (b > 0) sort_paths(lds, s, owner, alive);
        if (alive) {
            float t = 1000.0f;
            constexpr bool cull = GEO == kGeoTriBvh ? b == 0 : true;
            const int id = closest_hit<GEO, SPH, cull, (b == 0 ? 0 : 1)>(sv, s.o, s.d, 0.001f, &t);
            if (b > 0) load_thr_acc(lds, s);
            alive = id >= 0 && shade<b, B, GEO, SPH, SMALL>(P, sv, s, id, t);
            if (!alive || b + 1 == B) deliver(lds, owner, s.acc);
        }
        SortedChain<b + 1, B, GEO, SPH, SMALL>::run(P, sv, lds, s, owner, alive);
    }
};
template <int B, int GEO, bool SPH, bool SMALL>
struct SortedChain<B, B, GEO, SPH, SMALL> {
    __device__ __forceinline__ static void run(const KParams&, const SceneView&, float4*,
                                               PathState&, uint32_t&, bool&) {}
};


}

constexpr int kMinWavesPerEu = 8;
constexpr int kMinWavesPerEuSph = 8;
#ifndef RT_CLU_WAVES
#define RT_CLU_WAVES 7
#endif
constexpr int kMinWavesPerEuClu = RT_CLU_WAVES;
constexpr uint32_t block_threads(int geo) { return geo == kGeoSphLds ? kSphBlockThreads : kBlockThreads; }
constexpr uint32_t waves_per_row(int geo) { return block_threads(geo) >= 128 ? 2u : 1u; }
constexpr uint32_t waves_per_col(int geo) { return block_threads(geo) / 64u / waves_per_row(geo); }

template <int B, int GEO, bool SPH, bool SMALL, int L = 1>
#ifndef RT_TRI_WAVES
#define RT_TRI_WAVES 8
#endif
__global__ __launch_bounds__(block_threads(GEO),
                             SPH ? kMinWavesPerEuSph
                                 : (GEO == kGeoPairClu ? kMinWavesPerEuClu
                                                       : (GEO == kGeoTriBvh ? RT_TRI_WAVES : kMinWavesPerEu)))
void path_trace_kernel(KParams P) {
    constexpr uint32_t NT = block_threads(GEO), WR = waves_per_row(GEO), WC = waves_per_col(GEO);
    extern __shared__ float4 lds[];
    SceneView sv;
    const SceneTables T = tables_of(P);
    if (geo_staged(GEO)) {
        const StagedF4<uint32_t> n = staged_f4(GEO, T.nT, T.nP, T.nC);
        RT_LDS_GUARD(16 * (size_t)(n.rec + n.clu) + (GEO == kGeoPairClu ? 4 * (size_t)kHaltonTabFloats : 0));
        stage_records<GEO, NT>(lds, T);
        if (GEO == kGeoSphLds) {
            __shared__ float sph_stash[GEO == kGeoSphLds ? 6 * kSphBlockThreads : 1];
            sv.xstash = sph_stash;
        }
        if (GEO == kGeoPairClu) {
            const uint32_t tab0 = n.rec + n.clu;
            const bool tab = halton_tables_on(GEO, SMALL, P.spp, L);
            sv.htab = tab ? reinterpret_cast<const float*>(lds + tab0) : nullptr;
            if (tab) fill_halton_tables(reinterpret_cast<float*>(lds + tab0), threadIdx.x, NT);
        }
        __syncthreads();
    }
    bind_scene<GEO, SPH>(sv, T, lds);

    const uint32_t kWX = (L == 1) ? 8u : P.wave_w, kWY = (64u / L) / kWX;
    uint32_t bx, by;
    xcd_tile(bx, by);
    auto pixel_of = [&](uint32_t t, uint32_t& x, uint32_t& j) {
        const uint32_t lane = t & 63u, wave = t >> 6, pix = lane / L;
        x = bx * (WR * kWX) + (wave % WR) * kWX + (pix % kWX);
        j = by * (WC * kWY) + (wave / WR) * kWY + (pix / kWX);
    };
    if constexpr (RT_CAM_CAND && GEO == kGeoPairClu) {
        if (sv.nP - 1u < 32u) {
            const uint32_t wave = wave_uniform(threadIdx.x >> 6);
            const uint32_t wx0 = bx * (WR * kWX) + (wave % WR) * kWX;
            const uint32_t wj0 = by * (WC * kWY) + (wave / WR) * kWY;
            const float y0 = (float)(P.row_start + wj0 * P.row_step);
            const float y1 = (float)(P.row_start + (wj0 + kWY - 1u) * P.row_step);
            const Beam beam = make_beam(ld_f3(P.cam_pos), ld_f3(P.cam_u), ld_f3(P.cam_v), ld_f3(P.cam_w), P.halfW,
                                        P.halfH, (float)P.W, (float)P.H, (float)wx0, (float)(wx0 + kWX - 1u), y0, y1);
            const uint32_t k = threadIdx.x & 63u;
            const uint32_t kc = min(k, sv.nP - 1u);
            const bool keep = !beam_excludes_pair(beam, reinterpret_cast<const float*>(sv.pair + kPairF4 * kc));
            sv.cam_mask = wave_uniform((uint32_t)__builtin_amdgcn_ballot_w64(k < sv.nP && keep));
            sv.cam_avail = true;
            if constexpr (RT_SHD_CAND) {
                const uint32_t tb = k >> 5, kt = min(k & 31u, sv.nP - 1u);
                bool occ = false, bad = (sv.cam_mask & (sv.cam_mask - 1u)) != 0u;
                if (sv.cam_mask != 0u && !bad) {
                    const uint32_t sp = (uint32_t)__builtin_ctz(sv.cam_mask);
                    const float4 s0 = P.tri_shade[4 * (2u * sp + tb)];
                    if (s0.w == 0.0f) {
                        const ShaftLight lq = shaft_light(ld_f3(P.light_center));
                        const ShaftSrc src = shaft_source(beam, reinterpret_cast<const float*>(sv.pair + kPairF4 * sp),
                                                          (int)tb, f3{s0.x, s0.y, s0.z}, lq);
                        bad = !src.ok;
                        occ = !shaft_excludes_pair(src, lq, reinterpret_cast<const float*>(sv.pair + kPairF4 * kt));
                    }
                }
                const unsigned long long ob = __builtin_amdgcn_ballot_w64((k & 31u) < sv.nP && occ);
                sv.shd_mask = wave_uniform((uint32_t)ob | (uint32_t)(ob >> 32));
                sv.shd_avail = __builtin_amdgcn_ballot_w64(bad) == 0ull && sv.nC <= 32u;
                if (sv.nC != 0u) {
                    const uint32_t kc2 = min(k, sv.nC - 1u);
                    const uint32_t all = __float_as_uint(reinterpret_cast<const float*>(sv.clu + kCluF4 * kc2)[22]);
                    sv.shd_cskip = wave_uniform(
                        (uint32_t)__builtin_amdgcn_ballot_w64(k < sv.nC && (all & sv.shd_mask) == 0u));
                }
            }
        }
    }
    constexpr bool kRemat = GEO == kGeoPairClu || GEO == kGeoSphLds;
    auto opaque_tid = []() {
        uint32_t t = threadIdx.x;
        if constexpr (kRemat) asm volatile("" : "+v"(t));
        return t;
    };
    {
        uint32_t x, j;
        pixel_of(threadIdx.x, x, j);
        if (x >= (uint32_t)P.W || j >= P.row_count) return;
    }
    __shared__ uint32_t seed_s[NT];
    __shared__ float lum_s[L > 1 ? 3 * (NT / L) : 1];
    f3 lum{0.0f, 0.0f, 0.0f};
    {
        const uint32_t t = threadIdx.x, sub = t % L;
        uint32_t x, j;
        pixel_of(t, x, j);
        const uint32_t y = P.row_start + j * P.row_step;
        seed_s[t] = P.seeds[(size_t)y * (size_t)P.W + x] + P.sample_base;
        if (P.accumulate) {
            const float4 prev = P.sum[(size_t)j * (size_t)P.W + x];
            lum = f3{prev.x, prev.y, prev.z};
        }
        const uint32_t slot = t / L;
        if (L > 1 && sub == 0) {
            lum_s[3 * slot] = lum.x;
            lum_s[3 * slot + 1] = lum.y;
            lum_s[3 * slot + 2] = lum.z;
        }
    }
    const f3 cu = ld_f3(P.cam_u), cv = ld_f3(P.cam_v), cw = ld_f3(P.cam_w);
    const float fW = (float)P.W, fH = (float)P.H;
    const uint32_t rounds = (P.spp + (L - 1)) / L;
    for (uint32_t r = 0; r < rounds; ++r) {
#ifdef RT_STATS
        const unsigned long long t_round = clock64();
#endif
        const uint32_t t = opaque_tid(), sub = t % L;
        const uint32_t n = (L == 1) ? r : min(r * L + sub, P.spp - 1u);
        PathState s;
        s.acc = f3{0.0f, 0.0f, 0.0f};
        {
            uint32_t x, j;
            pixel_of(t, x, j);
            const float fx = (float)x, fy = (float)(P.row_start + j * P.row_step);
            s.i = seed_s[t] + n;
            const float jx = halton_dim<0, SMALL>(s.i);
            const float jy = halton_dim<1, SMALL, GEO == kGeoPairClu>(s.i, sv.htab);
            s.d = camera_dir<GEO == kGeoTriBvh>(P, cu, cv, cw, fW, fH, fx, fy, jx, jy);
            s.o = ld_f3(P.cam_pos);
            s.thr = f3{1.0f, 1.0f, 1.0f};
#if RT_CENSUS == 1
            {
                const uint32_t i2 = cz(s.i);
                const float jx2 = halton_dim<0, SMALL>(i2);
                const float jy2 = halton_dim<1, SMALL, GEO == kGeoPairClu>(i2, sv.htab);
                cz_sink(camera_dir(P, cu, cv, cw, fW, fH, cz(fx), cz(fy), jx2, jy2));
            }
#endif
#ifndef RT_TIMING_NO_TRACE
            trace_path<B, GEO, SPH, SMALL>(P, sv, s);
#else
            s.acc = s.d;
#endif
        }
        if (L == 1) {
            lum = lum + s.acc;
        } else if (L <= 16 && !SPH) {
            const uint32_t t2 = opaque_tid(), sub2 = t2 % L, slot = t2 / L;
            f3 acc{lum_s[3 * slot], lum_s[3 * slot + 1], lum_s[3 * slot + 2]};
#if RT_CENSUS == 6
            {
                f3 a2 = cz(acc);
                row_sum_in_order<L, 0>::run(a2, cz(s.acc), r * L, P.spp);
                cz_sink(a2);
            }
#endif
            row_sum_in_order<L, 0>::run(acc, s.acc, r * L, P.spp);
            if (sub2 == 0) {
                lum_s[3 * slot] = acc.x;
                lum_s[3 * slot + 1] = acc.y;
                lum_s[3 * slot + 2] = acc.z;
            }
        } else {
            const uint32_t t2 = opaque_tid(), lane = t2 & 63u, sub2 = t2 % L, slot = t2 / L;
            const int base = (int)(lane - sub2);
            f3 c[L];
#pragma unroll
            for (int k = 0; k < L; ++k)
                c[k] = f3{__shfl(s.acc.x, base + k), __shfl(s.acc.y, base + k),
                          __shfl(s.acc.z, base + k)};
            if (sub2 == 0) {
                f3 acc{lum_s[3 * slot], lum_s[3 * slot + 1], lum_s[3 * slot + 2]};
#pragma unroll
                for (int k = 0; k < L; ++k)
                    if (r * L + (uint32_t)k < P.spp) acc = acc + c[k];
                lum_s[3 * slot] = acc.x;
                lum_s[3 * slot + 1] = acc.y;
                lum_s[3 * slot + 2] = acc.z;
            }
        }
#ifdef RT_STATS
        if (!SPH && GEO != kGeoTriBvh) {
            RT_STAT(24, clock64() - t_round);
            RT_STAT(25, 1);
        }
#endif
    }
    uint32_t t = threadIdx.x;
    asm volatile("" : "+v"(t));
    if (L > 1) {
        if (t % L != 0) return;
        const uint32_t slot = t / L;
        lum = f3{lum_s[3 * slot], lum_s[3 * slot + 1], lum_s[3 * slot + 2]};
    }
    uint32_t x, j;
    pixel_of(t, x, j);
    const size_t o = (size_t)j * (size_t)P.W + x;
    if (P.sum) P.sum[o] = make_float4(lum.x, lum.y, lum.z, (float)P.samples_total);
    if (P.out) {
        const float fs = (float)P.samples_total;
        const float r = lum.x / fs, g = lum.y / fs, bl = lum.z / fs;
        store_pixel(P, o, r, g, bl);
    }
}

#include "rt_free.hpp"

#ifndef RT_SORTED_BVH_WAVES
#define RT_SORTED_BVH_WAVES 4
#endif
template <int B, int GEO, bool SPH, bool SMALL>
__global__ __launch_bounds__(kBlockThreads, GEO == kGeoPairLds ? kMinWavesPerEu : RT_SORTED_BVH_WAVES)
void path_trace_sorted_kernel(
    KParams P) {
    extern __shared__ float4 lds[];
    SceneView sv;
    const SceneTables T = tables_of(P);
    RT_LDS_GUARD(16 * (size_t)(kSortF4 + staged_f4(GEO, T.nT, T.nP, T.nC).rec));
    float4* scene = lds + kSortF4;
    stage_records<GEO, kBlockThreads>(scene, T);
    bind_scene<GEO, SPH>(sv, T, scene);

    const uint32_t tid = threadIdx.x, lane = tid & 63u, wave = tid >> 6;
    const uint32_t x = blockIdx.x * kTile + (wave & 1u) * 8u + (lane & 7u);
    const uint32_t j = blockIdx.y * kTile + (wave >> 1) * 8u + (lane >> 3);
    const bool valid = x < (uint32_t)P.W && j < P.row_count;
    const uint32_t y = P.row_start + j * P.row_step;
    const size_t o = (size_t)j * (size_t)P.W + x;
    const uint32_t seed = valid ? P.seeds[(size_t)y * (size_t)P.W + x] : 0u;
    float* sum = reinterpret_cast<float*>(lds + kSortLum);
    {
        float4 prev = make_float4(0.0f, 0.0f, 0.0f, 0.0f);
        if (valid && P.accumulate) prev = P.sum[o];
        sum[tid] = prev.x;
        sum[kBlockThreads + tid] = prev.y;
        sum[2 * kBlockThreads + tid] = prev.z;
    }
    __syncthreads();
    const float fx = (float)x, fy = (float)y, fW = (float)P.W, fH = (float)P.H;
    for (uint32_t n = 0; n < P.spp; ++n) {
        PathState s;
        s.i = seed + (P.sample_base + n);
        s.acc = f3{0.0f, 0.0f, 0.0f};
        s.thr = f3{1.0f, 1.0f, 1.0f};
        s.o = ld_f3(P.cam_pos);
        s.d = f3{0.0f, 0.0f, 0.0f};
        if (valid) {
            const float jx = halton_dim<0, SMALL>(s.i), jy = halton_dim<1, SMALL>(s.i);
            s.d = camera_dir(P, ld_f3(P.cam_u), ld_f3(P.cam_v), ld_f3(P.cam_w), fW, fH, fx, fy, jx, jy);
        }
        uint32_t owner = tid;
        bool alive = valid;
        SortedChain<0, B, GEO, SPH, SMALL>::run(P, sv, lds, s, owner, alive);
        __syncthreads();
    }
    if (!valid) return;
    finish_pixel(P, o, f3{sum[tid], sum[kBlockThreads + tid], sum[2 * kBlockThreads + tid]});
}

__global__ void math_check_kernel(uint32_t lo, uint32_t n, unsigned long long* bad) {
    for (uint32_t i = blockIdx.x * blockDim.x + threadIdx.x; i < n; i += gridDim.x * blockDim.x) {
        const float x = __uint_as_float(lo + i);
        float y = x;
        asm volatile("" : "+v"(y));
        const float s = sqrt_cr(x), sr = sqrtf(y);
        const float r = rcp_cr(x), rr = 1.0f / y;
        const bool sbad = !(__float_as_uint(s) == __float_as_uint(sr) || (s != s && sr != sr));
        const bool rbad = !(__float_as_uint(r) == __float_as_uint(rr) || (r != r && rr != rr));
        if (sbad) atomicAdd(&bad[0], 1ull);
        if (rbad) atomicAdd(&bad[1], 1ull);
    }
}

__global__ void fill_seeds_kernel(uint32_t* seeds, uint64_t key, uint64_t n) {
    for (uint64_t p = (uint64_t)blockIdx.x * blockDim.x + threadIdx.x; p < n;
         p += (uint64_t)gridDim.x * blockDim.x) {
        uint64_t z = key + p + 0x9E3779B97F4A7C15ULL;
        z = (z ^ (z >> 30)) * 0xBF58476D1CE4E5B9ULL;
        z = (z ^ (z >> 27)) * 0x94D049BB133111EBULL;
        z = z ^ (z >> 31);
        seeds[p] = (uint32_t)(z & 0xFFFFFu);
    }
}

template <typename U>
__global__ void place_tiles_kernel(const U* __restrict__ gathered, U* __restrict__ frame, uint32_t row_u,
                                   size_t tile_u, uint32_t H, uint32_t N) {
    for (uint32_t y = blockIdx.y; y < H; y += gridDim.y) {
// ... 58 lines not shown
    I.tables = halton_tables_on(GEO, SMALL, P.spp, (uint32_t)L) ? 1u : 0u;
    I.small = SMALL ? 1u : 0u;
    I.threads = threads;
    I.grid_x = grid.x;
    I.grid_y = grid.y;
    I.lds = (uint32_t)lds;
}

inline hipError_t allow_lds(const void* kernel, size_t bytes) {
    if (bytes <= 65536) return hipSuccess;
    return hipFuncSetAttribute(kernel, hipFuncAttributeMaxDynamicSharedMemorySize, (int)bytes);
}

template <int B, int GEO, bool SPH, bool SMALL, int L>
hipError_t launch_tl(const KParams& P, size_t lds_bytes, hipStream_t stream) {
    KParams Q = P;
    if (L > 1) Q.wave_w = (P.row_step > 1) ? 64u / L : (L == 4 ? 4u : 2u);
    constexpr uint32_t WR = waves_per_row(GEO), WC = waves_per_col(GEO);
    const uint32_t WX = (L == 1) ? 8u : Q.wave_w;
    const uint32_t TX = WR * WX, TY = WC * ((64u / L) / WX);
    const dim3 grid((P.W + TX - 1) / TX, (P.row_count + TY - 1) / TY);
    if (GEO == kGeoSphLds) {
        const hipError_t e = allow_lds((const void*)path_trace_kernel<B, GEO, SPH, SMALL, L>, lds_bytes);
        if (e != hipSuccess) return e;
    }
    note_launch<B, GEO, SPH, SMALL, L>("path_trace_kernel", Q, grid, block_threads(GEO), lds_bytes);
    hipLaunchKernelGGL((path_trace_kernel<B, GEO, SPH, SMALL, L>), grid, dim3(block_threads(GEO)),
                       lds_bytes, stream, Q);
    return hipGetLastError();
}

template <int B, int GEO, bool SPH, bool SMALL>
hipError_t launch_t(const KParams& P, size_t lds_bytes, hipStream_t stream) {
    if (SMALL) {
        const int lpp = lanes_per_pixel(P, GEO);
        if (lpp == 16) return launch_tl<B, GEO, SPH, SMALL, 16>(P, lds_bytes, stream);
        if (lpp == 4) return launch_tl<B, GEO, SPH, SMALL, 4>(P, lds_bytes, stream);
    }
    return launch_tl<B, GEO, SPH, SMALL, 1>(P, lds_bytes, stream);
}

template <int B, int GEO, bool SPH, bool SMALL>
hipError_t launch_sorted_t(const KParams& P, size_t lds_bytes, hipStream_t stream) {
    const dim3 grid((P.W + kTile - 1) / kTile, (P.row_count + kTile - 1) / kTile);
    note_launch<B, GEO, SPH, SMALL, 1>("path_trace_sorted_kernel", P, grid, kBlockThreads, lds_bytes);
    hipLaunchKernelGGL((path_trace_sorted_kernel<B, GEO, SPH, SMALL>), grid, dim3(kBlockThreads),
                       lds_bytes, stream, P);
    return hipGetLastError();
}

template <int B, int GEO, bool SORTED, bool SPH, bool SMALL>
hipError_t launch_k(const KParams& P, size_t lds_bytes, hipStream_t stream) {
    if constexpr (SORTED)
        return launch_sorted_t<B, GEO, SPH, SMALL>(P, lds_bytes, stream);
    else
        return launch_t<B, GEO, SPH, SMALL>(P, lds_bytes, stream);
}

template <int B, int GEO, bool SORTED, bool SPH>
hipError_t launch_h(const KParams& P, size_t lds_bytes, hipStream_t stream) {
    return P.max_index < kSmallIndexMax ? launch_k<B, GEO, SORTED, SPH, true>(P, lds_bytes, stream)
                                        : launch_k<B, GEO, SORTED, SPH, false>(P, lds_bytes, stream);
}

template <int B, int GEO, bool SORTED = false>
hipError_t launch_g(const KParams& P, size_t lds_bytes, hipStream_t stream) {
    if constexpr (GEO == (SORTED ? kGeoTriBvh : kGeoPairClu))
        return launch_h<B, GEO, SORTED, false>(P, lds_bytes, stream);
    if (GEO == kGeoSphLds || P.nS > 0) return launch_h<B, GEO, SORTED, true>(P, lds_bytes, stream);
    return launch_h<B, GEO, SORTED, false>(P, lds_bytes, stream);
}

template <int B, int GEO, bool SMALL>
hipError_t launch_free_t(const KParams& P, size_t lds_bytes, hipStream_t stream) {
    KParams Q = P;
    Q.wave_w = (P.row_step > 1) ? 64u : 8u;
    const uint32_t TY = 64u / Q.wave_w;
    const dim3 grid((P.W + Q.wave_w - 1) / Q.wave_w, (P.row_count + TY - 1) / TY);
    note_launch<B, GEO, GEO == kGeoSphLds, SMALL, 1>("path_free_kernel", Q, grid, kFreeThreads, lds_bytes);
    hipLaunchKernelGGL((path_free_kernel<B, GEO, SMALL>), grid, dim3(kFreeThreads), lds_bytes, stream,
                       Q);
    return hipGetLastError();
}

template <int B, int GEO>
hipError_t launch_free(const KParams& P, size_t lds_bytes, hipStream_t stream) {
    if constexpr (B < 1) {
        return hipErrorInvalidValue;
    } else {
        return P.max_index < kSmallIndexMax ? launch_free_t<B, GEO, true>(P, lds_bytes, stream)
                                            : launch_free_t<B, GEO, false>(P, lds_bytes, stream);
    }
}

template <int B>
hipError_t launch_b(const KParams& P, int geo, size_t lds_bytes, hipStream_t stream) {
    if (geo == kGeoFreeSph) return launch_free<B, kGeoSphLds>(P, lds_bytes, stream);
    if (geo == kGeoFreeTri) return launch_free<B, kGeoTriBvh>(P, lds_bytes, stream);
    if (geo == kGeoPairSorted) return launch_g<B, kGeoPairLds, true>(P, lds_bytes, stream);
    if (geo == kGeoSortSph) return launch_g<B, kGeoSphLds, true>(P, lds_bytes, stream);
    if (geo == kGeoSortTri) return launch_g<B, kGeoTriBvh, true>(P, lds_bytes, stream);
    switch (geo) {
        case kGeoPairLds: return launch_g<B, kGeoPairLds>(P, lds_bytes, stream);
        case kGeoPairClu: return launch_g<B, kGeoPairClu>(P, lds_bytes, stream);
        case kGeoSphLds: return launch_g<B, kGeoSphLds>(P, lds_bytes, stream);
        case kGeoPairSmem: return launch_g<B, kGeoPairSmem>(P, lds_bytes, stream);
        case kGeoTriBvh: return launch_g<B, kGeoTriBvh>(P, lds_bytes, stream);
        case kGeoTriLds: return launch_g<B, kGeoTriLds>(P, lds_bytes, stream);
        default: return launch_g<B, kGeoTriGlobal>(P, lds_bytes, stream);
    }
}

}

size_t kernel_lds_bytes(uint32_t n_tri, uint32_t n_pairs, uint32_t n_sph, uint32_t n_nodes) {
    (void)n_sph;
    (void)n_nodes;
    return n_pairs ? staged_lds_bytes(kLayPairLds, n_tri, n_pairs, 0) : staged_lds_bytes(kLayTriLds, n_tri, 0, 0);
}

KernelChoice choose_kernel(const SceneTables& t, bool sph_compact, uint32_t bounces, SceneMem mem, uint32_t walk) {
    const uint32_t nP = t.nP, nS = t.nS, nC = t.nC, nTN = t.nTN;
    auto lds = [&](int lay) { return staged_lds_bytes(lay, t.nT, nP, nC); };
    const bool pairs = nP > 0 && mem != SceneMem::kLdsSingle;
    int geo = kGeoTriGlobal;
    if (mem != SceneMem::kSmem && lds(pairs ? kGeoPairLds : kGeoTriLds) <= kMaxLdsBytes)
        geo = pairs ? kGeoPairLds : kGeoTriLds;
    if (mem == SceneMem::kPairSmem && nP > 0) geo = kGeoPairSmem;
    if (nTN > 0 && (mem == SceneMem::kTriBvh || mem == SceneMem::kAuto)) geo = kGeoTriBvh;
    if (geo == kGeoPairLds && nS > 0 && sph_compact && mem == SceneMem::kAuto &&
        lds(kGeoSphLds) <= kSphPairLdsMaxBytes)
        geo = kGeoSphLds;
    if (geo == kGeoPairLds && nC > 0 && nS == 0 && mem == SceneMem::kAuto && lds(kGeoPairClu) <= kMaxLdsBytes)
        geo = kGeoPairClu;
    if (geo == kGeoPairLds && mem == SceneMem::kPairSorted && lds(kGeoPairSorted) <= kMaxLdsBytes)
        geo = kGeoPairSorted;
    if (bounces >= 1 && walk == kWalkFree) {
        if (geo == kGeoSphLds) geo = kGeoFreeSph;
        if (geo == kGeoTriBvh && nS == 0) geo = kGeoFreeTri;
    }
    if (walk == kWalkSorted) {
        if (geo == kGeoSphLds) geo = kGeoSortSph;
        if (geo == kGeoTriBvh && nS == 0) geo = kGeoSortTri;
    }
    return KernelChoice{geo, lds(geo)};
}

namespace {
hipError_t launch_path_trace_impl(const KParams& P, uint32_t bounces, SceneMem mem,
                                  hipStream_t stream) {
    const KernelChoice kc = choose_kernel(tables_of(P), P.sph_lds != nullptr, bounces, mem, P.walk);
    const int geo = kc.layout;
    const size_t lds_total = kc.lds_bytes;
#ifdef RT_LDS_UNDERSIZE
    const size_t lds_req = lds_total >= 16 ? lds_total - 16 : lds_total;
#else
    const size_t lds_req = lds_total;
#endif
#ifdef RT_DEV_ISA
    if (bounces != 3) return hipErrorInvalidValue;
    if (geo == kGeoFreeSph) return launch_free<3, kGeoSphLds>(P, lds_req, stream);
    if (geo == kGeoFreeTri) return launch_free<3, kGeoTriBvh>(P, lds_req, stream);
    if (geo == kGeoSortSph) return launch_g<3, kGeoSphLds, true>(P, lds_req, stream);
    if (geo == kGeoSortTri) return launch_g<3, kGeoTriBvh, true>(P, lds_req, stream);
    if (geo == kGeoTriBvh) return launch_g<3, kGeoTriBvh>(P, lds_req, stream);
    return geo == kGeoPairClu ? launch_g<3, kGeoPairClu>(P, lds_req, stream)
                              : launch_g<3, kGeoSphLds>(P, lds_req, stream);
#endif
    switch (bounces) {
        case 0: return launch_b<0>(P, geo, lds_req, stream);
        case 1: return launch_b<1>(P, geo, lds_req, stream);
        case 2: return launch_b<2>(P, geo, lds_req, stream);
        case 3: return launch_b<3>(P, geo, lds_req, stream);
        case 4: return launch_b<4>(P, geo, lds_req, stream);
        default: return hipErrorInvalidValue;
    }
}
}

hipError_t launch_path_trace(const KParams& P, uint32_t bounces, SceneMem mem,
                             hipStream_t stream, LaunchInfo* info) {
    const hipError_t e = launch_path_trace_impl(P, bounces, mem, stream);
    if (info) *info = g_last;
    return e;
}


hipError_t lds_check_result(uint32_t* end) {
    *end = 0;
#ifdef RT_LDS_CHECK
    hipError_t e = hipMemcpyFromSymbol(end, HIP_SYMBOL(g_lds_overflow), sizeof(uint32_t));
    if (e != hipSuccess) return e;
    const uint32_t zero = 0;
    return hipMemcpyToSymbol(HIP_SYMBOL(g_lds_overflow), &zero, sizeof(zero));
#else
    return hipSuccess;
#endif
}

hipError_t read_debug_stats(unsigned long long* out, int n) {
#if defined(RT_FREE_DEBUG)
    constexpr int kWords = (int)(sizeof(g_free_dbg) / 8);
    if (n > kWords) n = kWords;
    hipError_t e = hipMemcpyFromSymbol(out, HIP_SYMBOL(g_free_dbg), n * sizeof(unsigned long long));
    if (e != hipSuccess) return e;
    static const uint32_t zero[4] = {0, 0, 0, 0};
    return hipMemcpyToSymbol(HIP_SYMBOL(g_free_dbg), zero, sizeof(zero));
#elif defined(RT_STATS)
    if (n > 40) n = 40;
    hipError_t e = hipMemcpyFromSymbol(out, HIP_SYMBOL(g_rt_stats), n * sizeof(unsigned long long));
    if (e != hipSuccess) return e;
    const unsigned long long zero[40] = {0};
    return hipMemcpyToSymbol(HIP_SYMBOL(g_rt_stats), zero, sizeof(zero));
#else
    (void)out;
    (void)n;
    return hipErrorNotSupported;
#endif
}

hipError_t math_selfcheck(unsigned long long bad[2]) {
    unsigned long long* d = nullptr;
    hipError_t e = hipMalloc((void**)&d, 2 * sizeof(unsigned long long));
    if (e != hipSuccess) return e;
    if ((e = hipMemset(d, 0, 2 * sizeof(unsigned long long))) == hipSuccess) {
        hipLaunchKernelGGL(math_check_kernel, dim3(16384), dim3(256), 0, 0, 0u, 0x80000000u, d);
        hipLaunchKernelGGL(math_check_kernel, dim3(16384), dim3(256), 0, 0, 0x80000000u, 0x80000000u, d);
        if ((e = hipGetLastError()) == hipSuccess && (e = hipDeviceSynchronize()) == hipSuccess)
            e = hipMemcpy(bad, d, 2 * sizeof(unsigned long long), hipMemcpyDeviceToHost);
    }
    (void)hipFree(d);
    return e;
}

hipError_t launch_fill_seeds(uint32_t* seeds, uint64_t key, uint64_t n, hipStream_t stream) {
    if (n == 0) return hipSuccess;
    uint64_t blocks = (n + 255) / 256;
    if (blocks > 8192) blocks = 8192;
    hipLaunchKernelGGL(fill_seeds_kernel, dim3((unsigned)blocks), dim3(256), 0, stream, seeds,
                       key, n);
    return hipGetLastError();
}

}
```

### gpuraytracer_amd/csrc/rt_kernel.hpp

```cpp
#pragma once

#include <hip/hip_runtime.h>
#include <stddef.h>
#include <stdint.h>

#include "rt_math.h"
#include "rt_raydomain.h"

namespace rt {

constexpr uint32_t kBlockThreads = 256;
constexpr uint32_t kTile = 16;
constexpr size_t kMaxLdsBytes = 64 * 1024;
constexpr uint32_t kOutFp16 = 0x2u;
constexpr uint32_t kOutRgba8 = 0x10u;
constexpr uint32_t kPairF4 = 7;
constexpr uint32_t kSphBlockThreads = 64;
constexpr size_t kSphPairLdsMaxBytes = 6 * 1024;
constexpr uint32_t kCluF4 = 7;
#ifndef RT_CAM_CAND
#define RT_CAM_CAND 1
#endif
#ifndef RT_SHD_CAND
#define RT_SHD_CAND 1
#endif
#ifndef RT_CLU_ORDER
#define RT_CLU_ORDER 1
#endif
#ifndef RT_CLU_LEAN
#define RT_CLU_LEAN 1
#endif
constexpr uint32_t kTriCompactLayouts = 8;
constexpr uint32_t kTriBvhMinTriangles = 384;

struct SceneTables {
    const float4* tri_isect;
    const float4* pair_isect;
    const float4* clusters;
    const float4* sph_isect;
    const float4* sph_nodes;
    const uint32_t* sph_perm;
    const uint4* sph_box;
    const uint4* tri_nodes;
    const float4* tri_sorted;
    const uint32_t* tri_perm;
    uint32_t nT, nP, nS, nN;
    uint32_t nTN;
    uint32_t nC;
    uint32_t pair_free;
};
struct KParams {
    const float4* tri_isect;
    const float4* pair_isect;
    const float4* tri_shade;
    const float4* sph_isect;
    const float4* sph_nodes;
    const uint32_t* sph_perm;
    const float4* sph_shade;
    const uint32_t* sph_lds;
    const uint16_t* sph_lds_id;
    const uint4* sph_box;
    const uint4* tri_nodes;
    const float4* tri_sorted;
    const uint32_t* tri_perm;
    const uint32_t* seeds;
    float4* sum;
    void* out;
    uint32_t nT, nP, nS, nN;
    uint32_t nE;
    uint32_t nTN;
    float cam_pos[3], cam_u[3], cam_v[3], cam_w[3];
    float halfW, halfH;
    int32_t W, H;
    float light_center[3], light_color[3];
    uint32_t spp, sample_base;
    uint32_t row_start, row_step, row_count;
    uint32_t accumulate;
    uint32_t samples_total;
    uint32_t flags;
    uint32_t max_index;
    uint32_t lanes;
    uint32_t walk;
    uint32_t wave_w;
    uint32_t walk_leaf_den;
    uint32_t light_plain;
    const float4* clusters;
    uint32_t nC;
    uint32_t pair_free;
    uint64_t light_mask;
};

size_t kernel_lds_bytes(uint32_t n_tri, uint32_t n_pairs, uint32_t n_sph, uint32_t n_nodes);

enum KernelLayout : int {
    kLayTriLds = 0,
    kLayPairLds = 1,
    kLayTriGlobal = 2,
    kLayPairSorted = 3,
    kLayPairSmem = 4,
    kLayTriBvh = 5,
    kLayPairClu = 6,
    kLaySphLds = 7,
    kLayFreeSph = 8,
    kLayFreeTri = 9,
    kLaySortSph = 10,
    kLaySortTri = 11,
};
template <typename N>
struct StagedF4 {
    N rec, clu;
};
template <typename N = uint32_t>
__host__ __device__ __forceinline__ constexpr StagedF4<N> staged_f4(int lay, N nT, N nP, N nC) {
    return StagedF4<N>{lay == kLayTriLds ? 3u * nT
                       : (lay == kLayPairLds || lay == kLayPairClu || lay == kLaySphLds || lay == kLayFreeSph ||
                          lay == kLayPairSorted || lay == kLaySortSph)
                           ? kPairF4 * nP
                           : N(0),
                       lay == kLayPairClu ? kCluF4 * nC : N(0)};
}
constexpr uint32_t kHaltonTabLdsFloats = 4679;
constexpr uint32_t kSortLdsF4 = 1097;
__host__ __device__ constexpr size_t staged_lds_bytes(int lay, uint32_t nT, uint32_t nP, uint32_t nC) {
    const StagedF4<size_t> n = staged_f4<size_t>(lay, nT, nP, nC);
    return 16 * (n.rec + n.clu) + (lay == kLayPairClu ? (size_t)4 * kHaltonTabLdsFloats : (size_t)0) +
           ((lay == kLayPairSorted || lay == kLaySortSph || lay == kLaySortTri) ? (size_t)16 * kSortLdsF4 : (size_t)0);
}
constexpr uint32_t kHaltonTabMinRounds = 8;
__host__ __device__ constexpr bool halton_tables_on(int geo, bool small, uint32_t spp, uint32_t L) {
    return geo == kLayPairClu && small && (spp + L - 1) / L >= kHaltonTabMinRounds;
}
struct KernelChoice {
    int layout;
    size_t lds_bytes;
};
struct LaunchInfo {
    char kernel[96];
    uint32_t lanes, tables, small, threads, grid_x, grid_y, lds;
};
constexpr uint32_t kWalkAuto = 0, kWalkLockstep = 1, kWalkFree = 2, kWalkSorted = 3;
enum class SceneMem { kAuto = 0, kLdsSingle = 1, kSmem = 2, kPairSorted = 3, kPairSmem = 4, kTriBvh = 5, kPairLds = 6 };
hipError_t launch_path_trace(const KParams& P, uint32_t bounces, SceneMem mem, hipStream_t stream,
                             LaunchInfo* info);
KernelChoice choose_kernel(const SceneTables& t, bool sph_compact, uint32_t bounces, SceneMem mem, uint32_t walk);
hipError_t read_debug_stats(unsigned long long* out, int n);
hipError_t lds_check_result(uint32_t* end);
struct MisParams {
    SceneTables tab;
    const float4* mis_shade;
    const float4* u_tab;
    float4* out;
    uchar4* out8;
    float cam_pos[3], cam_u[3], cam_v[3], cam_w[3];
    float halfW, halfH;
    int32_t W, H;
    float l_center[3], l_tangent[3], l_bitangent[3], l_radiance[3];
    float l_width, l_depth, l_area, exposure;
    uint32_t camera_rays, S;
    uint32_t row_start, row_step, row_count;
    float4* part;
};
constexpr uint32_t kRaysAny = 0x100u;
constexpr uint32_t kRaysExact = 0x200u;
constexpr uint32_t kRayChunk = 2048;
constexpr int ray_query_layout(int lay) {
    return (lay == kLayFreeSph || lay == kLaySortSph)   ? (int)kLaySphLds
           : (lay == kLayFreeTri || lay == kLaySortTri) ? (int)kLayTriBvh
           : lay == kLayPairSorted                      ? (int)kLayPairLds
                                                        : lay;
}
__host__ __device__ constexpr size_t ray_query_lds_bytes(int lay, uint32_t nT, uint32_t nP, uint32_t nC) {
    const StagedF4<size_t> n = staged_f4<size_t>(lay, nT, nP, nC);
    return 16 * (n.rec + n.clu);
}
struct RayQueryParams {
    SceneTables tab;
    uint32_t sph_compact;
    const float4* rays;
    uint2* hits;
    uint32_t n;
    uint32_t flags;
    RayDomain dom;
};
hipError_t launch_ray_query(const RayQueryParams& P, SceneMem mem, hipStream_t stream, LaunchInfo* info);

constexpr uint32_t kAovCenter = 0x400u;
constexpr uint32_t kAovTabLdsFloats = 729;
__host__ __device__ constexpr size_t aov_lds_bytes(int lay, uint32_t nT, uint32_t nP, uint32_t nC, bool tables) {
    return ray_query_lds_bytes(lay, nT, nP, nC) + (tables ? (size_t)4 * kAovTabLdsFloats : (size_t)0);
}
struct AovParams {
    SceneTables tab;
    uint32_t sph_compact;
    const float4* tri_shade;
    const float4* sph_shade;
    const uint32_t* seeds;
    float4* albedo;
    float4* normal_depth;
    uint2* first_hit;
    float cam_pos[3], cam_u[3], cam_v[3], cam_w[3];
    float halfW, halfH;
    int32_t W, H;
    uint32_t spp, sample_base;
    uint32_t row_start, row_step, row_count;
    uint32_t flags;
    uint32_t max_index;
};
hipError_t launch_aov(const AovParams& P, SceneMem mem, hipStream_t stream, LaunchInfo* info);

hipError_t launch_mis(const MisParams& P, SceneMem mem, hipStream_t stream);
size_t mis_lds_bytes(uint32_t n_tri, uint32_t n_pairs);
size_t mis_part_bytes(uint32_t camera_rays, size_t pixels);

hipError_t build_tri_lbvh(const float4* d_tri, uint32_t n, const float lo[3], const float hi[3],
                          float margin, uint4* d_nodes, float4* d_sorted, uint32_t* d_perm,
                          hipStream_t s);

hipError_t build_tri_gsah(const float4* d_tri, uint32_t n, float margin, uint32_t leaf_max, double trav_cost,
                          uint4* d_nodes, float4* d_sorted, uint32_t* d_perm, uint32_t* total_nodes,
                          size_t* temp_bytes, hipStream_t s);
hipError_t scan_u32(const uint32_t* in, uint32_t* out, uint32_t n, uint32_t* tile_sums, hipStream_t s);

hipError_t launch_fill_seeds(uint32_t* seeds, uint64_t key, uint64_t n, hipStream_t stream);
hipError_t math_selfcheck(unsigned long long bad[2]);

hipError_t launch_place_tiles(const void* gathered, void* frame, size_t row_bytes, size_t tile_bytes,
                              uint32_t H, uint32_t N, hipStream_t stream);

}
```

### gpuraytracer_amd/csrc/rt_trace.hpp

```cpp
#pragma once
#include <hip/hip_runtime.h>

#include "rt_cluorder.hpp"
#include "rt_kernel.hpp"

namespace rt {
namespace {

__device__ __forceinline__ f3 ld_f3(const float* p) { return f3{p[0], p[1], p[2]}; }

__device__ __forceinline__ bool tri_test(const float4& A, const float4& Bq, const float4& C, f3 o,
                                         f3 d, float tmin, float tmax, float* t_out) {
    const f3 v0{A.x, A.y, A.z}, e1{A.w, Bq.x, Bq.y}, e2{Bq.z, Bq.w, C.x}, n{C.y, C.z, C.w};
    const f3 tv = o - v0;
    const f3 c = cross(tv, d);
    const float den = dot(n, d);
    const uint32_t sgn = __float_as_uint(den) & 0x80000000u;
    const uint32_t nsgn = sgn ^ 0x80000000u;
    const float bu = __uint_as_float(__float_as_uint(dot(e2, c)) ^ nsgn);
    const float bv = __uint_as_float(__float_as_uint(dot(e1, c)) ^ sgn);
    const float aden = fabsf(den);
    if (aden > 0.0f && bu >= 0.0f && bv >= 0.0f && bu + bv <= aden) {
        const float tn = __uint_as_float(__float_as_uint(dot(n, tv)) ^ nsgn);
        const float t = tn / aden;
        if (t > tmin && t < tmax) {
            *t_out = t;
            return true;
        }
    }
    return false;
}

struct PairDots {
    float denA, denB;
    uint32_t a1, a2, b1, b2;
    f3 tv;
};

__device__ __forceinline__ PairDots pair_dots(const float4& r0, const float4& r1,
                                              const float4& r2, const float4& r3,
                                              const float4& r4, f3 o, f3 d) {
    PairDots q;
    const f3 v0{r0.x, r0.y, r0.z}, S{r0.w, r1.x, r1.y}, eA{r1.z, r1.w, r2.x};
    const f3 nA{r2.y, r2.z, r2.w}, eB{r3.x, r3.y, r3.z}, nB{r3.w, r4.x, r4.y};
    const uint32_t m = __float_as_uint(r4.z);
    q.tv = o - v0;
    const f3 c = cross(q.tv, d);
    const uint32_t s = __float_as_uint(dot(S, c));
    const uint32_t ea = __float_as_uint(dot(eA, c));
    const uint32_t eb = __float_as_uint(dot(eB, c));
    q.denA = dot(nA, d);
    q.denB = dot(nB, d);
    const uint32_t sA = (__float_as_uint(q.denA) & 0x80000000u) ^ m;
    const uint32_t sB = (__float_as_uint(q.denB) & 0x80000000u) ^ m;
    q.a1 = s ^ sA;
    q.a2 = ea ^ sA ^ 0x80000000u;
    q.b1 = s ^ sB ^ 0x80000000u;
    q.b2 = eb ^ sB;
    return q;
}

__device__ __forceinline__ bool bary_ok(float den, uint32_t t1, uint32_t t2) {
    const float u = __uint_as_float(t1), v = __uint_as_float(t2);
    return fabsf(den) > 0.0f && u >= 0.0f && v >= 0.0f && u + v <= fabsf(den);
}

__device__ __forceinline__ float pair_t(f3 n, f3 tv, float den) {
    const uint32_t nsgn = (__float_as_uint(den) & 0x80000000u) ^ 0x80000000u;
    const float tn = __uint_as_float(__float_as_uint(dot(n, tv)) ^ nsgn);
    return tn / fabsf(den);
}

__device__ __forceinline__ bool sph_test(const float4& S, f3 o, f3 d, float a, float tmin,
                                         float tmax, float* t_out) {
    const f3 oc = o - f3{S.x, S.y, S.z};
    const float b = 2.0f * dot(oc, d);
    const float cc = dot(oc, oc) - S.w;
    const float disc = b * b - (4.0f * a) * cc;
    if (disc > 0.0f) {
        const float sq = sqrtf(disc);
        const float a2 = 2.0f * a;
        float t = (-b - sq) / a2;
        if (!(t > tmin)) t = (-b + sq) / a2;
        if (t > tmin && t < tmax) {
            *t_out = t;
            return true;
        }
    }
    return false;
}

#ifdef RT_STATS
__device__ unsigned long long g_rt_stats[40];
__device__ __forceinline__ void stat_wave(int slot, unsigned long long v) {
    const unsigned long long m = __ballot(1);
    if ((threadIdx.x & 63u) == (unsigned)(__ffsll((long long)m) - 1)) atomicAdd(&g_rt_stats[slot], v);
}
#define RT_STAT(slot, v) stat_wave((slot), (v))
#else
#define RT_STAT(slot, v) ((void)0)
#endif

enum Geo : int {
    kGeoTriLds = 0,
    kGeoPairLds = 1,
    kGeoPairSmem = 4,
    kGeoTriBvh = 5,
    kGeoTriGlobal = 2,
    kGeoPairClu = 6,
    kGeoSphLds = 7,
};

constexpr bool geo_pairs(int g) { return g == kGeoPairLds || g == kGeoPairSmem || g == kGeoSphLds; }

struct SceneView {
    const float4* tri = nullptr;
    const float4* pair = nullptr;
    const float4* sph = nullptr;
    const float4* node = nullptr;
    const uint32_t* sph_perm = nullptr;
    const uint4* tnode = nullptr;
    const float4* tsorted = nullptr;
    const uint32_t* tperm = nullptr;
    uint32_t nTN = 0;
    uint32_t nT = 0, nP = 0, nS = 0, nN = 0;
    const float4* clu = nullptr;
    uint32_t nC = 0;
    uint32_t pair_free = 0;
    uint32_t cam_mask = 0;
    bool cam_avail = false;
    uint32_t shd_mask = 0;
    uint32_t shd_cskip = 0;
    bool shd_avail = false;
    const float* htab = nullptr;
    const uint4* sent = nullptr;
    const uint16_t* sid = nullptr;
    const uint4* sbox = nullptr;
    uint32_t nSB = 0;
    const float4* shade = nullptr;
    float* xstash = nullptr;
};

__host__ __device__ __forceinline__ SceneTables tables_of(const KParams& P) {
    return SceneTables{P.tri_isect, P.pair_isect, P.clusters,   P.sph_isect, P.sph_nodes, P.sph_perm,
                       P.sph_box,   P.tri_nodes,  P.tri_sorted, P.tri_perm,  P.nT,        P.nP,
                       P.nS,        P.nN,         P.nTN,        P.nC,        P.pair_free};
}

constexpr bool geo_staged(int g) {
    return g == kGeoTriLds || g == kGeoPairLds || g == kGeoPairClu || g == kGeoSphLds;
}

template <int GEO, uint32_t NT>
__device__ __forceinline__ void stage_records(float4* lds, const SceneTables& T) {
    const StagedF4<uint32_t> n = staged_f4(GEO, T.nT, T.nP, T.nC);
    const float4* src = GEO == kGeoTriLds ? T.tri_isect : T.pair_isect;
    for (uint32_t k = threadIdx.x; k < n.rec; k += NT) lds[k] = src[k];
    for (uint32_t k = threadIdx.x; k < n.clu; k += NT) lds[n.rec + k] = T.clusters[k];
}

template <int GEO, bool SPH>
__device__ __forceinline__ void bind_scene(SceneView& sv, const SceneTables& T, const float4* lds) {
    sv.nT = T.nT;
    sv.nP = T.nP;
    sv.nS = SPH ? T.nS : 0u;
    sv.tri = geo_staged(GEO) ? lds : T.tri_isect;
    sv.pair = geo_staged(GEO) ? lds : T.pair_isect;
    if (GEO == kGeoPairClu) {
        sv.clu = lds + staged_f4(GEO, T.nT, T.nP, T.nC).rec;
        sv.nC = T.nC;
        sv.pair_free = T.pair_free;
    }
    sv.tnode = T.tri_nodes;
    sv.tsorted = T.tri_sorted;
    sv.tperm = T.tri_perm;
    sv.nTN = T.nTN;
    sv.node = T.sph_nodes;
    sv.sph = T.sph_isect;
    sv.nN = SPH ? T.nN : 0u;
    sv.sph_perm = T.sph_perm;
    sv.sbox = T.sph_box;
    sv.nSB = T.nN;
}

struct RayBox {
    f3 invd, oinv;
};

__device__ __forceinline__ RayBox ray_box(f3 o, f3 d) {
    RayBox r;
    r.invd = f3{safe_rcp(d.x), safe_rcp(d.y), safe_rcp(d.z)};
    r.oinv = f3{o.x * r.invd.x, o.y * r.invd.y, o.z * r.invd.z};
    return r;
}

__device__ __forceinline__ bool node_hit(const float4& n0, const float4& n1, const RayBox& rb,
                                         float tmin, float tmax) {
    const float tx0 = fmaf(n0.x, rb.invd.x, -rb.oinv.x), tx1 = fmaf(n1.x, rb.invd.x, -rb.oinv.x);
    const float ty0 = fmaf(n0.y, rb.invd.y, -rb.oinv.y), ty1 = fmaf(n1.y, rb.invd.y, -rb.oinv.y);
    const float tz0 = fmaf(n0.z, rb.invd.z, -rb.oinv.z), tz1 = fmaf(n1.z, rb.invd.z, -rb.oinv.z);
    const float tnear = vmax3(vmin(tx0, tx1), vmin(ty0, ty1), vmax(vmin(tz0, tz1), tmin));
    const float tfar = vmin3(vmax(tx0, tx1), vmax(ty0, ty1), vmin(vmax(tz0, tz1), tmax));
    return tnear <= tfar;
}

__device__ __forceinline__ uint32_t octant(f3 d) {
    return (__float_as_uint(d.x) >> 31) | ((__float_as_uint(d.y) >> 31) << 1) |
           ((__float_as_uint(d.z) >> 31) << 2);
}

__device__ __forceinline__ uint32_t wave_uniform(uint32_t v) {
    return (uint32_t)__builtin_amdgcn_readfirstlane((int)v);
}

__device__ __forceinline__ void sphere_closest(const float4* __restrict__ node,
                                               const float4* __restrict__ sph,
                                               const uint32_t* __restrict__ perm, uint32_t nN,
                                               uint32_t nT, f3 o, f3 d, float tmin, float& best,
                                               int& id) {
    const float a = dot(d, d);
    const RayBox rb = ray_box(o, d);
    node += 2u * nN * octant(d);
    uint32_t idx = 0;
    while (idx < nN) {
        const float4 n0 = node[2 * idx], n1 = node[2 * idx + 1];
        uint32_t next = __float_as_uint(n0.w);
        if (node_hit(n0, n1, rb, tmin, best)) {
            const uint32_t leaf = __float_as_uint(n1.w);
            if (leaf == 0u) {
                next = idx + 1;
            } else {
                const uint32_t first = leaf & 0xFFFFFFu, end = first + (leaf >> 24);
                for (uint32_t k = first; k < end; ++k) {
                    float t;
                    if (sph_test(sph[k], o, d, a, tmin, 3.0e38f, &t) && t <= best) {
                        const int sid = (int)(nT + perm[k]);
                        if (t < best || sid < id) {
                            best = t;
                            id = sid;
                        }
                    }
                }
            }
        }
        idx = next;
    }
}

__device__ __forceinline__ bool sphere_any(const float4* __restrict__ node,
                                           const float4* __restrict__ sph, uint32_t nN, f3 o,
                                           f3 d, float tmin, float tmax) {
    const float a = dot(d, d);
    const RayBox rb = ray_box(o, d);
    node += 2u * nN * octant(d);
    uint32_t idx = 0;
    while (idx < nN) {
        const float4 n0 = node[2 * idx], n1 = node[2 * idx + 1];
        uint32_t next = __float_as_uint(n0.w);
        if (node_hit(n0, n1, rb, tmin, tmax)) {
            const uint32_t leaf = __float_as_uint(n1.w);
            if (leaf == 0u) {
                next = idx + 1;
            } else {
                const uint32_t first = leaf & 0xFFFFFFu, end = first + (leaf >> 24);
                for (uint32_t k = first; k < end; ++k) {
                    float t;
                    if (sph_test(sph[k], o, d, a, tmin, tmax, &t)) return true;
                }
            }
        }
        idx = next;
    }
    return false;
}

__device__ __forceinline__ float h2f(uint32_t b16) {
    return (float)__builtin_bit_cast(_Float16, (uint16_t)b16);
}

__device__ __forceinline__ bool lds_node_hit(const uint4& e, const RayBox& rb, float tmin,
                                             float tmax) {
    const float4 n0 = make_float4(h2f(e.x & 0xFFFFu), h2f(e.x >> 16), h2f(e.y & 0xFFFFu), 0.0f);
    const float4 n1 = make_float4(h2f(e.y >> 16), h2f(e.z & 0xFFFFu), h2f(e.z >> 16), 0.0f);
    return node_hit(n0, n1, rb, tmin, tmax);
}

__device__ __forceinline__ bool lds_node_hit_nf(const uint4& e, const RayBox& rb, float tmin,
// ... 639 lines not shown
```

### gpuraytracer_amd/host.py

```python
from __future__ import annotations

import ctypes
import os
from dataclasses import dataclass, fields

import numpy as np

from ._native import (LAYOUTS, RT_AOV_CENTER, RT_COMM_ID_BYTES, RT_KEEP_SUM, RT_OK, RT_OUT_DEVICE, RT_OUT_FP16,
                      RT_OUT_NONE, RT_OUT_RGBA8, RT_RAYS_ANY, RT_RAYS_EXACT, TRI_BUILDS, WALKS,
                      AovBuffers, AovParams, BuildStats, CameraGPU, CreateOptions, LaunchInfo, MaterialGPU, MisParamsC, RayDomainInfo,
                      RenderParamsC,
                      RtError, SceneDesc, SceneInfo, SphereGPU, SquareLightGPU, TileLayout, TriBvhDump, float3,
                      lib)

DEFAULT_SEED_KEY = 0x5EED00000000


def _check(status: int, ctx=None):
    if status != RT_OK:
        raise RtError(status, lib.rt_last_error(ctx).decode())


def seed_splitmix(width: int, height: int, key: int = DEFAULT_SEED_KEY) -> np.ndarray:
    n = int(width) * int(height)
    out = np.empty(n, dtype=np.uint32)
    lib.rt_seed_splitmix(ctypes.c_uint64(key), out.ctypes.data_as(ctypes.c_void_p), n)
    return out.reshape(height, width)


def tonemap_rgba8(rgba32f: np.ndarray) -> np.ndarray:
    a = np.ascontiguousarray(rgba32f, dtype=np.float32)
    n = a.size // 4
    out = np.empty(a.shape[:-1] + (4,), dtype=np.uint8)
    lib.rt_tonemap_rgba8(a.ctypes.data_as(ctypes.c_void_p), n,
                         out.ctypes.data_as(ctypes.c_void_p))
    return out


def comm_unique_id() -> bytes:
    buf = (ctypes.c_uint8 * RT_COMM_ID_BYTES)()
    _check(lib.rt_comm_unique_id(buf))
    return bytes(buf)


def _pixel_flags(fp16: bool = False, rgba8: bool = False) -> int:
    return (RT_OUT_FP16 if fp16 else 0) | (RT_OUT_RGBA8 if rgba8 else 0)


def tile_layout(width: int, height: int, world: int, rank: int, fp16: bool = False,
                rgba8: bool = False) -> dict:
    t = TileLayout()
    _check(lib.rt_tile_layout(width, height, world, rank, _pixel_flags(fp16, rgba8), ctypes.byref(t)))
    return {k: getattr(t, k) for k, _ in TileLayout._fields_}


def place_tiles_host(gathered: np.ndarray, width: int, height: int, world: int) -> np.ndarray:
    g = np.ascontiguousarray(gathered)
    fp16, rgba8 = g.dtype == np.uint16, g.dtype == np.uint8
    if g.dtype not in (np.float32, np.uint16, np.uint8):
        raise ValueError("gathered pixels must be float32, uint16 (fp16 bits) or uint8")
    lay = tile_layout(width, height, world, 0, fp16, rgba8)
    if g.nbytes != world * lay["tile_bytes"]:
        raise ValueError(f"gathered holds {g.nbytes} bytes, expected {world} x {lay['tile_bytes']}")
    frame = np.empty((height, width, 4), g.dtype)
    _check(lib.rt_place_tiles_host(g.ctypes.data_as(ctypes.c_void_p), width, height, world,
                                   _pixel_flags(fp16, rgba8), frame.ctypes.data_as(ctypes.c_void_p)))
    return frame


def _tri_bvh_dump(call, n: int, nodes_cap: int) -> dict:
    nodes = np.zeros((8 * nodes_cap, 4), np.uint32)
    srt = np.zeros((n, 12), np.float32)
    perm = np.zeros(n, np.uint32)
    isect = np.zeros((n, 12), np.float32)
    d = TriBvhDump()
    d.nodes, d.sorted, d.perm, d.isect = (a.ctypes.data for a in (nodes, srt, perm, isect))
    call(d)
    total = int(d.nodes_per_layout)
    assert int(d.n_triangles) == n and total <= nodes_cap
    return {"n_triangles": n, "nodes_per_layout": total, "leaf_max": int(d.leaf_max),
            "margin": np.float32(d.margin), "nodes": nodes[:8 * total].reshape(8, total, 4).copy(),
            "sorted": srt, "perm": perm, "isect": isect}


@dataclass
class Options:

    layout: str = "auto"
    lanes: int = 0
    tri_build: str = "default"
    tri_leaf_max: int = 0
    tri_leaf_cost: float = 0.0
    sphere_leaf_max: int = 0
    sphere_median: bool = False
    walk: str = "auto"
    walk_leaf_den: int = 0

    def c(self) -> CreateOptions:
        o = CreateOptions()
        o.scene_layout = LAYOUTS[self.layout]
        o.lanes_per_pixel = self.lanes
        o.tri_bvh_build = TRI_BUILDS[self.tri_build]
        o.tri_leaf_max = self.tri_leaf_max
        o.tri_leaf_cost = self.tri_leaf_cost
        o.sphere_leaf_max = self.sphere_leaf_max
        o.sphere_median = 1 if self.sphere_median else 0
        o.walk_scheduler = WALKS[self.walk]
        o.walk_leaf_den = self.walk_leaf_den
        return o

    _ENV = {"layout": "RTPT_SCENE_MEM", "lanes": "RTPT_LANES", "tri_build": "RTPT_TRI_BUILD",
            "tri_leaf_max": "RTPT_TRI_LEAF", "tri_leaf_cost": "RTPT_TRI_CT",
            "sphere_leaf_max": "RTPT_BVH_LEAF", "walk": "RTPT_WALK"}

    @classmethod
    def from_env(cls, env=None) -> "Options":
        env = os.environ if env is None else env
        o = cls()
        for f in fields(cls):
            v = env.get(cls._ENV.get(f.name, ""))
            if v:
                setattr(o, f.name, type(getattr(o, f.name))(v) if f.type != "str" else v)
        if env.get("RTPT_BVH_SAH") == "0":
            o.sphere_median = True
        return o


class Scene:

    def __init__(self, camera: CameraGPU, materials, vertices, light: SquareLightGPU,
                 spheres=None):
        self.camera = camera
        self.materials = materials
        self.vertices = vertices
        self.light = light
        self.spheres = spheres

    @property
    def n_triangles(self) -> int:
        return len(self.materials)

    @property
    def n_spheres(self) -> int:
        return 0 if self.spheres is None else len(self.spheres)

    @property
    def width(self) -> int:
        return int(self.camera.resolution.x)

    @property
    def height(self) -> int:
        return int(self.camera.resolution.y)

    @classmethod
    def cornell_box(cls, width: int = 800, height: int = 600) -> "Scene":
        cam, light = CameraGPU(), SquareLightGPU()
        mats = (MaterialGPU * 36)()
        verts = (float3 * 108)()
        n = ctypes.c_uint32()
        _check(lib.rt_scene_cornell_box(width, height, ctypes.byref(cam), mats, verts,
                                        ctypes.byref(light), ctypes.byref(n)))
        assert n.value == 36
        return cls(cam, mats, verts, light)

    @classmethod
    def cornell_box_mis(cls, width: int = 800, height: int = 600) -> "Scene":
        cam, light = CameraGPU(), SquareLightGPU()
        mats = (MaterialGPU * 36)()
# ... 251 lines not shown
        cur = torch.cuda.current_stream(rays.device) if stream is None else None
        handle = cur.cuda_stream if stream is None else getattr(stream, "cuda_stream", stream)
        _check(lib.rt_trace_rays_async(self._ctx, ctypes.c_void_p(rays.data_ptr()), n, flags,
                                       ctypes.c_void_p(hits.data_ptr()), ctypes.c_void_p(handle)), self._ctx)
        if cur is not None:
            cur.synchronize()
        return hits[:, 0].view(torch.float32), hits[:, 1]

    def render_aov(self, spp: int = 1, sample_base: int = 0, row_start: int = 0, row_step: int = 1,
                   row_count: int = 0, center: bool = False, albedo: bool = True,
                   normal_depth: bool = True, first_hit: bool = True, out=None, stream=None) -> dict:
        p = AovParams()
        p.spp, p.sample_base = spp, sample_base
        p.row_start, p.row_step, p.row_count = row_start, row_step, row_count
        p.flags = RT_AOV_CENTER if center else 0
        rows = RenderParams(row_start=row_start, row_step=row_step, row_count=row_count).rows(self.scene.height)
        W = self.scene.width
        b = AovBuffers()
        if out is None:
            res = {}
            if albedo:
                res["albedo"] = np.empty((rows, W, 4), np.float32)
            if normal_depth:
                res["normal_depth"] = np.empty((rows, W, 4), np.float32)
            if first_hit:
                res["first_hit"] = np.empty((rows, W), np.dtype([("t", np.float32), ("id", np.int32)]))
            for k, a in res.items():
                setattr(b, k, a.ctypes.data)
            _check(lib.rt_render_aov(self._ctx, ctypes.byref(p), ctypes.byref(b)), self._ctx)
            return res
        import torch
        shapes = {"albedo": ((rows, W, 4), torch.float32), "normal_depth": ((rows, W, 4), torch.float32),
                  "first_hit": ((rows, W, 2), torch.int32)}
        for k, t in out.items():
            if k not in shapes:
                raise ValueError(f"unknown buffer {k!r}")
            shape, dt = shapes[k]
            if (tuple(t.shape) != shape or t.dtype != dt or not t.is_contiguous() or not t.is_cuda
                    or t.device.index != self.device):
                raise ValueError(f"out[{k!r}] must be a contiguous {shape} {dt} tensor on the context's device")
            setattr(b, k, t.data_ptr())
        p.flags |= RT_OUT_DEVICE
        cur = torch.cuda.current_stream(self.device) if stream is None else None
        handle = cur.cuda_stream if stream is None else getattr(stream, "cuda_stream", stream)
        _check(lib.rt_render_aov_async(self._ctx, ctypes.byref(p), ctypes.byref(b), ctypes.c_void_p(handle)),
               self._ctx)
        if cur is not None:
            cur.synchronize()
        return out

    def render_progressive(self, params: RenderParams, batch_spp: int, out, stream=None,
                           gather: bool = False):
        if stream is None:
            import torch
            stream = torch.cuda.current_stream().cuda_stream
        elif hasattr(stream, "cuda_stream"):
            stream = stream.cuda_stream
        total, done = params.spp, 0
        ptr = out if (out is None or isinstance(out, int)) else out.data_ptr()
        while done < total:
            n = min(batch_spp, total - done)
            last = done + n == total
            p = RenderParams(spp=n, bounces=params.bounces, sample_base=params.sample_base + done,
                             row_start=params.row_start, row_step=params.row_step,
                             row_count=params.row_count, accumulate=done > 0, keep_sum=True,
                             fp16=params.fp16, rgba8=params.rgba8)
            flags = RT_OUT_DEVICE if last else (RT_OUT_DEVICE | RT_OUT_NONE)
            fn = lib.rt_render_gather if gather else lib.rt_render_async
            _check(fn(self._ctx, ctypes.byref(p.c(flags)), ctypes.c_void_p(ptr if last else None),
                      ctypes.c_void_p(stream)), self._ctx)
            done += n
        return out

    def accumulate(self, params: RenderParams):
        _check(lib.rt_render(self._ctx, ctypes.byref(params.c(RT_OUT_NONE | RT_KEEP_SUM)), None),
               self._ctx)

    def draw(self, spp: int = 400, bounces: int = 3) -> np.ndarray:
        return self.render(RenderParams(spp=spp, bounces=bounces))

    def render_mis(self, params: MisParams | None = None, out=None, out8=None):
        p = params or MisParams()
        if out is None and out8 is None:
            rows = p.rows(self.scene.height)
            img = np.empty((rows, self.scene.width, 4), dtype=np.float32)
            img8 = np.empty((rows, self.scene.width, 4), dtype=np.uint8)
            _check(lib.rt_render_mis(self._ctx, ctypes.byref(p.c()),
                                     img.ctypes.data_as(ctypes.c_void_p),
                                     img8.ctypes.data_as(ctypes.c_void_p)), self._ctx)
            return img, img8
        ptr = lambda t: None if t is None else ctypes.c_void_p(t if isinstance(t, int) else t.data_ptr())
        _check(lib.rt_render_mis(self._ctx, ctypes.byref(p.c(RT_OUT_DEVICE)), ptr(out), ptr(out8)),
               self._ctx)
        return out, out8

    def comm_init(self, rank: int, world: int, comm_id: bytes):
        if len(comm_id) != RT_COMM_ID_BYTES:
            raise ValueError("comm_id must be the 128 bytes of rt_comm_unique_id()")
        buf = (ctypes.c_uint8 * RT_COMM_ID_BYTES).from_buffer_copy(comm_id)
        _check(lib.rt_comm_init(self._ctx, rank, world, buf), self._ctx)
        self.rank, self.world = rank, world

    def render_gather(self, params: RenderParams | None = None, out=None, stream=None):
        p = params or RenderParams()
        if out is None:
            frame = None
            if getattr(self, "rank", 0) == 0 and not (p.c().flags & RT_OUT_NONE):
                dt = np.uint8 if p.rgba8 else np.uint16 if p.fp16 else np.float32
                frame = np.empty((self.scene.height, self.scene.width, 4), dtype=dt)
            ptr = None if frame is None else frame.ctypes.data_as(ctypes.c_void_p)
            _check(lib.rt_render_gather(self._ctx, ctypes.byref(p.c()), ptr, None), self._ctx)
            return frame
        if stream is None:
            import torch
            stream = torch.cuda.current_stream().cuda_stream
        elif hasattr(stream, "cuda_stream"):
            stream = stream.cuda_stream
        ptr = out if isinstance(out, int) else out.data_ptr()
        _check(lib.rt_render_gather(self._ctx, ctypes.byref(p.c(RT_OUT_DEVICE)), ctypes.c_void_p(ptr),
                                    ctypes.c_void_p(stream)), self._ctx)
        return out

    def comm_info(self) -> tuple[int, int]:
        n, r = ctypes.c_int32(), ctypes.c_int32()
        _check(lib.rt_comm_info(self._ctx, ctypes.byref(n), ctypes.byref(r)), self._ctx)
        return n.value, r.value

    def place_tiles(self, gathered, world: int, out=None, fp16: bool = False, rgba8: bool = False,
                    stream=None):
        gp = gathered if isinstance(gathered, int) else gathered.data_ptr()
        flags = _pixel_flags(fp16, rgba8)
        if stream is None:
            import torch
            stream = torch.cuda.current_stream().cuda_stream
        elif hasattr(stream, "cuda_stream"):
            stream = stream.cuda_stream
        if out is None:
            dt = np.uint8 if rgba8 else np.uint16 if fp16 else np.float32
            frame = np.empty((self.scene.height, self.scene.width, 4), dt)
            _check(lib.rt_place_tiles(self._ctx, ctypes.c_void_p(gp), world, flags,
                                      frame.ctypes.data_as(ctypes.c_void_p), ctypes.c_void_p(stream)),
                   self._ctx)
            return frame
        ptr = out if isinstance(out, int) else out.data_ptr()
        _check(lib.rt_place_tiles(self._ctx, ctypes.c_void_p(gp), world, flags | RT_OUT_DEVICE,
                                  ctypes.c_void_p(ptr), ctypes.c_void_p(stream)), self._ctx)
        return out

    def last_launch(self) -> dict:
        info = LaunchInfo()
        _check(lib.rt_last_launch(self._ctx, ctypes.byref(info)), self._ctx)
        return info.as_dict()

    def build_info(self) -> dict:
        b = BuildStats()
        _check(lib.rt_build_info(self._ctx, ctypes.byref(b)), self._ctx)
        return {k: getattr(b, k) for k, _ in BuildStats._fields_}

    def tri_bvh(self) -> dict:
        sizes = TriBvhDump()
        _check(lib.rt_debug_tri_bvh(self._ctx, ctypes.byref(sizes)), self._ctx)
        return _tri_bvh_dump(lambda d: _check(lib.rt_debug_tri_bvh(self._ctx, ctypes.byref(d)), self._ctx),
                             int(sizes.n_triangles), int(sizes.nodes_per_layout))

    def last_kernel_ms(self) -> float:
        ms = ctypes.c_float()
        _check(lib.rt_last_kernel_ms(self._ctx, ctypes.byref(ms)), self._ctx)
        return float(ms.value)
```

### include/rtpt.h

```cpp
#ifndef RTPT_H
#define RTPT_H

#include "rt_types.h"

#ifdef __cplusplus
extern "C" {
#endif

#define RTPT_ABI_VERSION 11

#define RT_MAX_BOUNCES 4

typedef enum rt_status {
    RT_OK = 0,
    RT_ERR_INVALID_ARG = 1,
    RT_ERR_NO_DEVICE = 2,
    RT_ERR_OUT_OF_MEMORY = 3,
    RT_ERR_LAUNCH = 4,
    RT_ERR_STATE = 5,
    RT_ERR_COMM = 6
} rt_status;

typedef struct rt_ctx rt_ctx;

// ... 104 lines not shown
int rt_place_tiles(rt_ctx* ctx, const void* gathered_device, int32_t world, uint32_t flags,
                   void* frame, void* hip_stream);

int rt_place_tiles_host(const void* gathered, int32_t width, int32_t height, int32_t world,
                        uint32_t flags, void* frame);

typedef struct rt_launch_info {
    char kernel[96];
    uint32_t lanes_per_pixel;
    uint32_t halton_tables;
    uint32_t small_index;
    uint32_t block_threads;
    uint32_t grid_x, grid_y;
    uint32_t lds_bytes;
} rt_launch_info;
int rt_last_launch(const rt_ctx* ctx, rt_launch_info* info);

typedef struct rt_ray {
    float origin[3];
    float tmin;
    float dir[3];
    float tmax;
} rt_ray;

typedef struct rt_ray_hit {
    float t;
    int32_t id;
} rt_ray_hit;

#define RT_RAYS_ANY   0x100u
#define RT_RAYS_EXACT 0x200u
#define RT_RAYS_CHUNK 2048

int rt_trace_rays(rt_ctx* ctx, const rt_ray* rays, uint64_t n, uint32_t flags, rt_ray_hit* hits);

int rt_trace_rays_async(rt_ctx* ctx, const rt_ray* rays_dev, uint64_t n, uint32_t flags,
                        rt_ray_hit* hits_dev, void* hip_stream);

#define RT_AOV_CENTER 0x400u

typedef struct rt_aov_params {
    uint32_t spp;
    uint32_t sample_base;
    uint32_t row_start;
    uint32_t row_step;
    uint32_t row_count;
    uint32_t flags;
} rt_aov_params;

typedef struct rt_aov_buffers {
    float* albedo;
    float* normal_depth;
    rt_ray_hit* first_hit;
} rt_aov_buffers;

int rt_render_aov(rt_ctx* ctx, const rt_aov_params* params, const rt_aov_buffers* buffers);

int rt_render_aov_async(rt_ctx* ctx, const rt_aov_params* params, const rt_aov_buffers* buffers_dev,
                        void* hip_stream);

typedef struct rt_ray_domain_info {
    float origin_max, dir_len2_min, dir_len2_max, tmax_max;
} rt_ray_domain_info;
int rt_debug_ray_domain(const rt_scene_desc* scene, rt_ray_domain_info* info);

typedef struct rt_build_stats {
    uint32_t tri_bvh_build;
    uint32_t tri_bvh_nodes;
    float tri_bvh_build_ms;
    float scene_compile_ms;
    uint32_t tri_bvh_temp_kib;
} rt_build_stats;
int rt_build_info(const rt_ctx* ctx, rt_build_stats* info);

typedef struct rt_tri_bvh_dump {
    uint32_t n_triangles;
    uint32_t nodes_per_layout;
    uint32_t leaf_max;
    float margin;
    uint32_t* nodes;
    float* sorted;
    uint32_t* perm;
    float* isect;
} rt_tri_bvh_dump;

int rt_debug_tri_bvh(const rt_ctx* ctx, rt_tri_bvh_dump* dump);

int rt_debug_tri_bvh_host(const rt_scene_desc* scene, const rt_create_options* opt, rt_tri_bvh_dump* dump);

int rt_math_selfcheck(uint64_t* mismatches);

const char* rt_build_sha(void);

int rt_debug_stats(rt_ctx* ctx, uint64_t* out, int n);

const char* rt_last_error(const rt_ctx* ctx);
const char* rt_status_string(int status);
int rt_abi_version(void);


void rt_seed_splitmix(uint64_t key, uint32_t* seeds, size_t n);

#define RT_CORNELL_TRIANGLES 36
int rt_scene_cornell_box(int32_t width, int32_t height, CameraGPU* camera,
                         MaterialGPU* materials, rt_float3* vertices,
                         SquareLightGPU* light, uint32_t* n_triangles);

#define RT_SPHERE_SCENE_TRIANGLES 12
int rt_scene_random_spheres(int32_t width, int32_t height, uint32_t n_spheres,
                            uint64_t seed, CameraGPU* camera, MaterialGPU* materials,
                            rt_float3* vertices, SquareLightGPU* light,
                            uint32_t* n_triangles, SphereGPU* spheres);

typedef struct rt_mis_params {
    uint32_t camera_rays;
    uint32_t mis_samples;
    uint32_t row_start, row_step, row_count;
    uint32_t flags;
} rt_mis_params;

int rt_render_mis(rt_ctx* ctx, const rt_mis_params* params, float* out_rgba32f,
                  uint8_t* out_rgba8);

int rt_scene_cornell_box_mis(int32_t width, int32_t height, CameraGPU* camera,
                             MaterialGPU* materials, rt_float3* vertices,
                             SquareLightGPU* light, uint32_t* n_triangles);

typedef struct rt_scene_info {
    uint32_t n_triangles;
    uint32_t n_triangle_pairs;
    uint32_t n_spheres;
    uint32_t lds_bytes;
    uint32_t n_sphere_nodes;
    uint32_t n_triangle_bvh_nodes;
    uint32_t n_box_clusters;
    uint32_t pair_free_mask;
    uint32_t sphere_kernel_lds_bytes;
    uint32_t kernel_layout;
    uint32_t kernel_lds_bytes;
} rt_scene_info;
int rt_scene_describe(const rt_scene_desc* scene, rt_scene_info* info);
int rt_scene_describe_ex(const rt_scene_desc* scene, const rt_create_options* opt, rt_scene_info* info);

int rt_debug_camera_candidates(const rt_scene_desc* scene, int32_t x0, int32_t x1, int32_t y0, int32_t y1,
                               uint8_t* may_hit);

int rt_debug_shadow_candidates(const rt_scene_desc* scene, int32_t x0, int32_t x1, int32_t y0, int32_t y1,
                               uint8_t* may_occlude, int32_t* available);

int rt_debug_cluster_kinds(const rt_scene_desc* scene, uint32_t* flags, uint32_t capacity, uint32_t* n_clusters);

int rt_debug_light_mask(const rt_scene_desc* scene, uint64_t* mask, float* records, uint32_t capacity_triangles);

void rt_tonemap_rgba8(const float* rgba32f, size_t n_pixels, uint8_t* rgba8);

#ifdef __cplusplus
}
#endif

#endif
```

Before: 28770 Msamples/s.

## Replace Halton high-digit loops with precomputed global-memory row tables

```diff
diff --git a/gpuraytracer_amd/_native.py b/gpuraytracer_amd/_native.py
--- a/gpuraytracer_amd/_native.py
+++ b/gpuraytracer_amd/_native.py
@@ -115,6 +115,11 @@
         d = {k: getattr(self, k) for k, _ in self._fields_}
         d["kernel"] = self.kernel.decode()
         return d
+
+
+class HaltonHiDim(ctypes.Structure):
+    _fields_ = [(n, ctypes.c_uint32) for n in ("base", "low_digits", "high_digits", "rows", "row_stride", "offset",
+                                               "is_low_table", "used")]
 
 
 class BuildStats(ctypes.Structure):
@@ -241,6 +246,10 @@
                                               ctypes.c_uint32, ctypes.POINTER(ctypes.c_uint32)]),
     "rt_debug_light_mask": (ctypes.c_int, [ctypes.POINTER(SceneDesc), ctypes.POINTER(ctypes.c_uint64), _P,
                                            ctypes.c_uint32]),
+    "rt_debug_halton_hi_layout": (ctypes.c_int, [ctypes.c_uint32, ctypes.POINTER(HaltonHiDim)]),
+    "rt_debug_halton_hi_table": (ctypes.c_int, [_P, ctypes.c_uint64, ctypes.POINTER(ctypes.c_uint64)]),
+    "rt_debug_halton_hi_eval": (ctypes.c_int, [ctypes.c_uint32, _P, ctypes.c_uint64, ctypes.c_uint32, _P]),
+    "rt_debug_halton_probe": (ctypes.c_int, [_P, ctypes.c_uint32, _P, ctypes.c_uint32, _P]),
 }
 
 
diff --git a/gpuraytracer_amd/csrc/rt_api.cpp b/gpuraytracer_amd/csrc/rt_api.cpp
--- a/gpuraytracer_amd/csrc/rt_api.cpp
+++ b/gpuraytracer_amd/csrc/rt_api.cpp
@@ -14,6 +14,7 @@
 #include "../../include/rtpt.h"
 #include "rt_beam.hpp"
 #include "rt_shaft.hpp"
+#include "rt_halton.hpp"
 #include "rt_kernel.hpp"
 #include "rt_scene.hpp"
 
@@ -42,6 +43,7 @@
     rt::SceneTables tab{};
     bool sph_compact = false;
     uint64_t light_mask = 0;
+    float* d_halton_hi = nullptr;
     uint32_t tri_bvh_build_used = 0;
     uint32_t tri_leaf_max = 1;
     float tri_bvh_build_ms = 0.0f;
@@ -117,6 +119,41 @@
     }
 };
 
+const std::vector<float>& halton_hi_host() {
+    static const std::vector<float> hi = [] {
+        std::vector<float> v(rt::kHaltonHiFloats);
+        rt::fill_halton_hi(v.data());
+        return v;
+    }();
+    return hi;
+}
+
+template <int D>
+float halton_hi_eval(uint32_t i, bool wrong, const float* hi) {
+    constexpr uint32_t b = rt::kPrimes[D];
+    constexpr int k = rt::hi_k(D);
+    constexpr float invB = 1.0f / (float)b;
+    constexpr uint32_t bk = rt::ipow(b, k), rows = rt::hi_rows(D);
+    uint32_t x = i / bk, low = i % bk;
+    if constexpr (rt::hi_is_row(D)) {
+        float f = 1.0f, r = 0.0f;
+        for (int j = 0; j < k; ++j) {
+            f = f * invB;
+            r = r + f * (float)(low % b);
+            low = low / b;
+        }
+        if (wrong) x = x + 1u < rows ? x + 1u : x - 1u;
+        const float* row = hi + rt::hi_offset(D) + (size_t)x * rt::hi_stride(D);
+        for (int j = 0; j < rt::hi_m(D); ++j) r = r + row[j];
+        return r;
+    } else {
+        if (wrong) low = low + 1u < rows ? low + 1u : low - 1u;
+        const float r = hi[rt::hi_offset(D) + low];
+        constexpr float f = rt::f_after(b, rt::kHiLowDigits + 1);
+        return r + f * (float)x;
+    }
+}
+
 template <typename T>
 hipError_t upload(T** dptr, const void* src, size_t bytes, hipStream_t s) {
     *dptr = nullptr;
@@ -179,6 +216,7 @@
     (void)hipFree(c->d_tri_shade);
     (void)hipFree(c->d_pair_isect);
     (void)hipFree(c->d_clusters);
+    (void)hipFree(c->d_halton_hi);
     (void)hipFree(c->d_sph_lds);
     (void)hipFree(c->d_sph_lds_id);
     (void)hipFree(c->d_sph_box);
@@ -283,6 +321,7 @@
     set_tables(&K, c->tab);
     K.tri_shade = c->d_tri_shade;
     K.light_mask = c->light_mask;
+    K.halton_hi = c->d_halton_hi;
     K.sph_lds = c->sph_compact ? c->d_sph_lds : nullptr;
     K.sph_lds_id = c->d_sph_lds_id;
     K.sph_shade = c->d_sph_shade;
@@ -937,6 +976,14 @@
     c->sph_compact = rt::sphere_compact_usable(c->scene);
     c->tab = scene_tables(c->scene, c->tri_bvh_nodes, c);
     c->light_mask = rt::light_mask(c->scene);
+    if (rt::choose_kernel(c->tab, c->sph_compact, 1, c->scene_mem, c->walk).layout == rt::kLayPairClu) {
+        const std::vector<float>& hi = halton_hi_host();
+        if ((e = upload(&c->d_halton_hi, hi.data(), hi.size() * sizeof(float), c->stream)) != hipSuccess) {
+            release(c);
+            delete c;
+            return fail(nullptr, RT_ERR_OUT_OF_MEMORY, std::string("Halton row upload: ") + hipGetErrorString(e));
+        }
+    }
     *out_ctx = c;
     return RT_OK;
 }
@@ -1354,6 +1401,81 @@
     return RT_OK;
 }
 
+int rt_debug_halton_hi_layout(uint32_t D, rt_halton_hi_dim* info) {
+    if (!info) return fail(nullptr, RT_ERR_INVALID_ARG, "null argument");
+    if (D >= 24 || rt::hi_k((int)D) == 0) return fail(nullptr, RT_ERR_INVALID_ARG, "dimension without a Halton table");
+    info->base = rt::kPrimes[D];
+    info->low_digits = (uint32_t)rt::hi_k((int)D);
+    info->high_digits = (uint32_t)rt::hi_m((int)D);
+    info->rows = rt::hi_rows((int)D);
+    info->row_stride = rt::hi_stride((int)D);
+    info->offset = rt::hi_offset((int)D);
+    info->is_low_table = rt::hi_is_low((int)D) ? 1u : 0u;
+    info->used = rt::hi_used((int)D) ? 1u : 0u;
+    return RT_OK;
+}
+
+int rt_debug_halton_hi_table(float* out, uint64_t capacity_floats, uint64_t* n_floats) {
+    if (!n_floats || (!out && capacity_floats)) return fail(nullptr, RT_ERR_INVALID_ARG, "null argument");
+    const std::vector<float>& hi = halton_hi_host();
+    *n_floats = hi.size();
+    if (out) memcpy(out, hi.data(), sizeof(float) * (size_t)std::min<uint64_t>(capacity_floats, hi.size()));
+    return RT_OK;
+}
+
+int rt_debug_halton_hi_eval(uint32_t D, const uint32_t* indices, uint64_t n, uint32_t variant, float* out) {
+    if ((!indices || !out) && n) return fail(nullptr, RT_ERR_INVALID_ARG, "null argument");
+    if (D >= 24 || rt::hi_k((int)D) == 0) return fail(nullptr, RT_ERR_INVALID_ARG, "dimension without a Halton table");
+    if (variant > 1) return fail(nullptr, RT_ERR_INVALID_ARG, "variant: 0 (the shipped form) or 1 (the neighbouring row)");
+    for (uint64_t q = 0; q < n; ++q)
+        if (indices[q] >= rt::kSmallIndexMax) return fail(nullptr, RT_ERR_INVALID_ARG, "index >= 3^13");
+    const float* hi = halton_hi_host().data();
+    const bool w = variant == 1;
+    for (uint64_t q = 0; q < n; ++q) {
+        const uint32_t i = indices[q];
+        switch (D) {
+            case 1: out[q] = halton_hi_eval<1>(i, w, hi); break;
+            case 2: out[q] = halton_hi_eval<2>(i, w, hi); break;
+            case 3: out[q] = halton_hi_eval<3>(i, w, hi); break;
+            case 4: out[q] = halton_hi_eval<4>(i, w, hi); break;
+            case 5: out[q] = halton_hi_eval<5>(i, w, hi); break;
+            case 7: out[q] = halton_hi_eval<7>(i, w, hi); break;
+            case 8: out[q] = halton_hi_eval<8>(i, w, hi); break;
+            case 9: out[q] = halton_hi_eval<9>(i, w, hi); break;
+            case 10: out[q] = halton_hi_eval<10>(i, w, hi); break;
+            case 12: out[q] = halton_hi_eval<12>(i, w, hi); break;
+            default: out[q] = halton_hi_eval<13>(i, w, hi); break;
+        }
+    }
+    return RT_OK;
+}
+
+int rt_debug_halton_probe(rt_ctx* c, uint32_t D, const uint32_t* indices, uint32_t n, float* out) {
+    if (!c) return fail(nullptr, RT_ERR_INVALID_ARG, "ctx is null");
+    if ((!indices || !out) && n) return fail(c, RT_ERR_INVALID_ARG, "null argument");
+    if (D >= 24 || rt::hi_k((int)D) == 0) return fail(c, RT_ERR_INVALID_ARG, "dimension without a Halton table");
+    if (!c->d_halton_hi) return fail(c, RT_ERR_STATE, "the context has no Halton rows (no box-cluster layout)");
+    for (uint32_t q = 0; q < n; ++q)
+        if (indices[q] >= rt::kSmallIndexMax) return fail(c, RT_ERR_INVALID_ARG, "index >= 3^13");
+    if (n == 0) return RT_OK;
+    DeviceGuard g(c->device);
+    uint32_t* d_idx = nullptr;
+    float* d_out = nullptr;
+    hipError_t e = upload(&d_idx, indices, (size_t)n * sizeof(uint32_t), c->stream);
+    if (e == hipSuccess) e = hipMalloc((void**)&d_out, (size_t)n * sizeof(float));
+    if (e != hipSuccess) {
+        (void)hipFree(d_idx);
+        return hip_fail(c, RT_ERR_OUT_OF_MEMORY, "Halton probe buffers", e);
+    }
+    e = rt::launch_halton_probe(c->d_halton_hi, D, d_idx, n, d_out, c->stream);
+    if (e == hipSuccess) e = hipMemcpyAsync(out, d_out, (size_t)n * sizeof(float), hipMemcpyDeviceToHost, c->stream);
+    if (e == hipSuccess) e = hipStreamSynchronize(c->stream);
+    (void)hipFree(d_idx);
+    (void)hipFree(d_out);
+    if (e != hipSuccess) return hip_fail(c, RT_ERR_LAUNCH, "Halton probe", e);
+    return RT_OK;
+}
+
 int rt_debug_stats(rt_ctx* c, uint64_t* out, int n) {
     if (!c || !out || n <= 0) return fail(c, RT_ERR_INVALID_ARG, "null argument");
     DeviceGuard g(c->device);
diff --git a/gpuraytracer_amd/csrc/rt_halton.hpp b/gpuraytracer_amd/csrc/rt_halton.hpp
--- a/gpuraytracer_amd/csrc/rt_halton.hpp
+++ b/gpuraytracer_amd/csrc/rt_halton.hpp
@@ -84,6 +84,12 @@
     return f;
 }
 
+}
+}
+#include "rt_halton_hi.hpp"
+namespace rt {
+namespace {
+
 template <uint32_t D>
 __device__ __forceinline__ void fill_halton_table(float* tab, uint32_t tid, uint32_t nthreads) {
     constexpr uint32_t b = kPrimes[D];
@@ -118,8 +124,8 @@
                   "table list");
 }
 
-template <uint32_t D>
-__device__ __forceinline__ float halton_tab(uint32_t i, const float* tab) {
+template <uint32_t D, bool HI = false>
+__device__ __forceinline__ float halton_tab(uint32_t i, const float* tab, const float* hi = nullptr) {
     constexpr uint32_t b = kPrimes[D];
     constexpr int k = kTabDigits[D];
     constexpr int nd = halton_digits(b, kSmallIndexMax);
@@ -129,22 +135,64 @@
     float low;
     float x = digit_step<bk>((float)i, low);
     float r = tab[off + (uint32_t)low];
-    constexpr float fk = f_after(b, k);
-    float f = fk;
+    if constexpr (HI && hi_used(D)) {
+        constexpr int m = hi_m(D);
+        static_assert(m == nd - k && m <= (int)hi_stride(D), "row width");
+        constexpr uint32_t hoff = hi_offset(D), hstride = hi_stride(D);
+        const uint32_t at = ((uint32_t)x * hstride + hoff) * 4u;
+        const float* row = reinterpret_cast<const float*>(reinterpret_cast<const char*>(hi) + at);
+        const float4 c0 = *reinterpret_cast<const float4*>(row);
+        r = r + c0.x;
+        if (m > 1) r = r + c0.y;
+        if (m > 2) r = r + c0.z;
+        if (m > 3) r = r + c0.w;
+        if constexpr (m == 5) {
+            r = r + row[4];
+        } else if constexpr (m == 6) {
+            const float2 c1 = *reinterpret_cast<const float2*>(row + 4);
+            r = (r + c1.x) + c1.y;
+        } else if constexpr (m > 6) {
+            const float4 c1 = *reinterpret_cast<const float4*>(row + 4);
+            r = ((r + c1.x) + c1.y) + c1.z;
+            if (m > 7) r = r + c1.w;
+        }
+        return r;
+    } else {
+        constexpr float fk = f_after(b, k);
+        float f = fk;
 #pragma unroll
-    for (int j = k; j < nd; ++j) {
-        f = f * invB;
-        float digit;
-        x = digit_step<b>(x, digit);
-        r = r + f * digit;
-    }
-    return r;
-}
-
-template <uint32_t D, bool SMALL, bool TAB = false>
-__device__ __forceinline__ float halton_dim(uint32_t i, const float* tab = nullptr) {
+        for (int j = k; j < nd; ++j) {
+            f = f * invB;
+            float digit;
+            x = digit_step<b>(x, digit);
+            r = r + f * digit;
+        }
+        return r;
+    }
+}
+
+template <uint32_t D>
+__device__ __forceinline__ float halton_low(uint32_t i, const float* hi) {
+    constexpr uint32_t b = kPrimes[D];
+    constexpr uint32_t bk = ipow(b, kHiLowDigits);
+    static_assert(hi_is_low(D) && hi_m(D) == 1 && bk < (1u << 23), "one digit after the low table");
+    float low;
+    const float x = digit_step<bk>((float)i, low);
+    constexpr uint32_t hoff = hi_offset(D);
+    const uint32_t at = ((uint32_t)low + hoff) * 4u;
+    const float r = *reinterpret_cast<const float*>(reinterpret_cast<const char*>(hi) + at);
+    constexpr float f = f_after(b, kHiLowDigits + 1);
+    return r + f * x;
+}
+
+constexpr bool kHaltonHi = RT_HALTON_HI != 0;
+
+template <uint32_t D, bool SMALL, bool TAB = false, bool HI = false>
+__device__ __forceinline__ float halton_dim(uint32_t i, const float* tab = nullptr, const float* hi = nullptr) {
     if constexpr (TAB && SMALL && kTabDigits[D] > 0)
-        if (tab != nullptr) return halton_tab<D>(i, tab);
+        if (tab != nullptr) return halton_tab<D, HI>(i, tab, hi);
+    if constexpr (TAB && SMALL && HI && hi_is_low(D) && hi_used(D))
+        if (tab != nullptr) return halton_low<D>(i, hi);
     if (SMALL) return halton_small<D>(i);
     return halton<D>(i);
 }
diff --git a/gpuraytracer_amd/csrc/rt_halton_hi.hpp b/gpuraytracer_amd/csrc/rt_halton_hi.hpp
--- /dev/null
+++ b/gpuraytracer_amd/csrc/rt_halton_hi.hpp
@@ -0,0 +1,92 @@
+#pragma once
+#include <stddef.h>
+#include <stdint.h>
+
+#ifndef RT_HALTON_HI
+#define RT_HALTON_HI 1
+#endif
+
+namespace rt {
+namespace {
+
+constexpr int kHiLowDigits = 3;
+constexpr bool hi_is_row(int D) { return kTabDigits[D] > 0; }
+constexpr bool hi_is_low(int D) { return D == 12 || D == 13; }
+constexpr int hi_k(int D) { return hi_is_row(D) ? kTabDigits[D] : hi_is_low(D) ? kHiLowDigits : 0; }
+constexpr int hi_m(int D) { return hi_k(D) ? halton_digits(kPrimes[D], kSmallIndexMax) - hi_k(D) : 0; }
+constexpr uint32_t hi_rows(int D) {
+    return hi_is_row(D)   ? (kSmallIndexMax + ipow(kPrimes[D], hi_k(D)) - 1u) / ipow(kPrimes[D], hi_k(D))
+           : hi_is_low(D) ? ipow(kPrimes[D], kHiLowDigits)
+                          : 0u;
+}
+constexpr uint32_t hi_stride(int D) { return hi_is_row(D) ? (hi_m(D) <= 4 ? 4u : 8u) : hi_is_low(D) ? 1u : 0u; }
+constexpr uint32_t hi_floats(int D) { return hi_rows(D) * hi_stride(D); }
+constexpr uint32_t hi_offset(int D) { return D == 0 ? 0u : hi_offset(D - 1) + hi_floats(D - 1); }
+constexpr uint32_t kHaltonHiFloats = hi_offset(24);
+static_assert(hi_m(1) == 7 && hi_m(2) == 5 && hi_m(3) == 5 && hi_m(4) == 4 && hi_m(5) == 4 && hi_m(7) == 3 &&
+                  hi_m(8) == 3 && hi_m(9) == 3 && hi_m(10) == 3 && hi_m(12) == 1 && hi_m(13) == 1,
+              "remaining digits per dimension");
+static_assert(hi_rows(4) == 13177 && hi_rows(12) == 68921 && hi_rows(13) == 79507, "row counts");
+static_assert(hi_offset(12) == 8 * (2187 + 2551 + 4649) + 4 * (13177 + 9434 + 4417 + 3014 + 1896 + 1660),
+              "838 KB of rows, then the two low tables");
+static_assert(hi_offset(12) % 4 == 0, "rows start on 16 bytes");
+static_assert(4 * (size_t)kHaltonHiFloats < 1536 * 1024, "the buffer stays well inside one XCD's 4 MB L2");
+
+constexpr bool hi_used(int D) {
+    return RT_HALTON_HI == 1 ? (hi_is_row(D) || hi_is_low(D))
+           : RT_HALTON_HI == 2 ? ((hi_is_row(D) && hi_m(D) >= 4) || hi_is_low(D))
+                               : false;
+}
+
+template <int D>
+inline void fill_halton_hi_dim(float* out) {
+    constexpr uint32_t b = kPrimes[D];
+    constexpr float invB = 1.0f / (float)b;
+    if constexpr (hi_is_row(D)) {
+        constexpr int m = hi_m(D);
+        constexpr uint32_t stride = hi_stride(D);
+        constexpr float fk = f_after(b, hi_k(D));
+        for (uint32_t x0 = 0; x0 < hi_rows(D); ++x0) {
+            uint32_t x = x0;
+            float f = fk;
+            for (uint32_t j = 0; j < stride; ++j) {
+                float c = 0.0f;
+                if (j < (uint32_t)m) {
+                    f = f * invB;
+                    c = f * (float)(x % b);
+                    x = x / b;
+                }
+                out[(size_t)x0 * stride + j] = c;
+            }
+        }
+    } else if constexpr (hi_is_low(D)) {
+        for (uint32_t v0 = 0; v0 < hi_rows(D); ++v0) {
+            uint32_t v = v0;
+            float f = 1.0f;
+            float r = 0.0f;
+            for (int j = 0; j < kHiLowDigits; ++j) {
+                f = f * invB;
+                r = r + f * (float)(v % b);
+                v = v / b;
+            }
+            out[v0] = r;
+        }
+    }
+}
+
+inline void fill_halton_hi(float* out) {
+    fill_halton_hi_dim<1>(out + hi_offset(1));
+    fill_halton_hi_dim<2>(out + hi_offset(2));
+    fill_halton_hi_dim<3>(out + hi_offset(3));
+    fill_halton_hi_dim<4>(out + hi_offset(4));
+    fill_halton_hi_dim<5>(out + hi_offset(5));
+    fill_halton_hi_dim<7>(out + hi_offset(7));
+    fill_halton_hi_dim<8>(out + hi_offset(8));
+    fill_halton_hi_dim<9>(out + hi_offset(9));
+    fill_halton_hi_dim<10>(out + hi_offset(10));
+    fill_halton_hi_dim<12>(out + hi_offset(12));
+    fill_halton_hi_dim<13>(out + hi_offset(13));
+}
+
+}
+}
diff --git a/gpuraytracer_amd/csrc/rt_halton_probe.hip b/gpuraytracer_amd/csrc/rt_halton_probe.hip
--- /dev/null
+++ b/gpuraytracer_amd/csrc/rt_halton_probe.hip
@@ -0,0 +1,44 @@
+#include <hip/hip_runtime.h>
+
+#include "rt_halton.hpp"
+#include "rt_kernel.hpp"
+
+namespace rt {
+namespace {
+
+__global__ __launch_bounds__(kBlockThreads) void halton_probe_kernel(const float* hi, uint32_t dim,
+                                                                     const uint32_t* idx, uint32_t n, float* out) {
+    extern __shared__ float tab[];
+    fill_halton_tables(tab, threadIdx.x, kBlockThreads);
+    __syncthreads();
+    for (uint32_t k = threadIdx.x; k < n; k += kBlockThreads) {
+        const uint32_t i = idx[k];
+        float r;
+        switch (dim) {
+            case 1: r = halton_dim<1, true, true, kHaltonHi>(i, tab, hi); break;
+            case 2: r = halton_dim<2, true, true, kHaltonHi>(i, tab, hi); break;
+            case 3: r = halton_dim<3, true, true, kHaltonHi>(i, tab, hi); break;
+            case 4: r = halton_dim<4, true, true, kHaltonHi>(i, tab, hi); break;
+            case 5: r = halton_dim<5, true, true, kHaltonHi>(i, tab, hi); break;
+            case 7: r = halton_dim<7, true, true, kHaltonHi>(i, tab, hi); break;
+            case 8: r = halton_dim<8, true, true, kHaltonHi>(i, tab, hi); break;
+            case 9: r = halton_dim<9, true, true, kHaltonHi>(i, tab, hi); break;
+            case 10: r = halton_dim<10, true, true, kHaltonHi>(i, tab, hi); break;
+            case 12: r = halton_dim<12, true, true, kHaltonHi>(i, tab, hi); break;
+            default: r = halton_dim<13, true, true, kHaltonHi>(i, tab, hi); break;
+        }
+        out[k] = r;
+    }
+}
+
+}
+
+hipError_t launch_halton_probe(const float* hi, uint32_t dim, const uint32_t* idx, uint32_t n, float* out,
+                               hipStream_t stream) {
+    if (!hi || !idx || !out || dim >= 24 || hi_k((int)dim) == 0) return hipErrorInvalidValue;
+    hipLaunchKernelGGL(halton_probe_kernel, dim3(1), dim3(kBlockThreads), sizeof(float) * kHaltonTabFloats, stream,
+                       hi, dim, idx, n, out);
+    return hipGetLastError();
+}
+
+}
diff --git a/gpuraytracer_amd/csrc/rt_kernel.hip b/gpuraytracer_amd/csrc/rt_kernel.hip
--- a/gpuraytracer_amd/csrc/rt_kernel.hip
+++ b/gpuraytracer_amd/csrc/rt_kernel.hip
@@ -61,11 +61,19 @@
 __device__ __forceinline__ bool shade(const KParams& P, const SceneView& sv, PathState& s, int id,
                                       float t, int* nid = nullptr, float* nt = nullptr) {
     f3 N, right, fwd, diffuse;
+    constexpr bool kRows = kHaltonHi && GEO == kGeoPairClu && !SPH;
+    float ux0 = 0.0f, uy0 = 0.0f;
     if constexpr (GEO == kGeoPairClu && !SPH) {
         if ((P.light_mask >> (uint32_t)id) & 1ull) {
             const float4 s3 = P.tri_shade[4 * id + 3];
             s.acc = f3{s3.x, s3.y, s3.z};
             return false;
+        }
+        if constexpr (kRows) {
+            asm volatile("" : "+v"(s.i) : "v"(t));
+            ux0 = halton_dim<2 + 5 * b, SMALL, true, true>(s.i, sv.htab, sv.hhi) * 2.0f - 1.0f;
+            uy0 = halton_dim<3 + 5 * b, SMALL, true, true>(s.i, sv.htab, sv.hhi) * 2.0f - 1.0f;
+            asm volatile("" : "+v"(id) : "v"(ux0), "v"(uy0));
         }
         const float4* sh = P.tri_shade + 4 * id;
         const float4 s0 = sh[0], s1 = sh[1], s2 = sh[2];
@@ -105,16 +113,16 @@
 #if RT_CENSUS == 4
     {
         const uint32_t i2 = cz(s.i);
-        float h = halton_dim<2 + 5 * b, SMALL, GEO == kGeoPairClu>(i2, sv.htab) +
-                  halton_dim<3 + 5 * b, SMALL, GEO == kGeoPairClu>(i2, sv.htab);
+        float h = halton_dim<2 + 5 * b, SMALL, GEO == kGeoPairClu, kHaltonHi>(i2, sv.htab, sv.hhi) +
+                  halton_dim<3 + 5 * b, SMALL, GEO == kGeoPairClu, kHaltonHi>(i2, sv.htab, sv.hhi);
         if (b + 1 < B)
-            h = h + halton_dim<4 + 5 * b, SMALL, GEO == kGeoPairClu>(i2, sv.htab) +
-                halton_dim<5 + 5 * b, SMALL, GEO == kGeoPairClu>(i2, sv.htab);
+            h = h + halton_dim<4 + 5 * b, SMALL, GEO == kGeoPairClu, kHaltonHi>(i2, sv.htab, sv.hhi) +
+                halton_dim<5 + 5 * b, SMALL, GEO == kGeoPairClu, kHaltonHi>(i2, sv.htab, sv.hhi);
         cz_sink(h);
     }
 #endif
-    const float ux = halton_dim<2 + 5 * b, SMALL, GEO == kGeoPairClu>(s.i, sv.htab) * 2.0f - 1.0f;
-    const float uy = halton_dim<3 + 5 * b, SMALL, GEO == kGeoPairClu>(s.i, sv.htab) * 2.0f - 1.0f;
+    const float ux = kRows ? ux0 : halton_dim<2 + 5 * b, SMALL, GEO == kGeoPairClu>(s.i, sv.htab) * 2.0f - 1.0f;
+    const float uy = kRows ? uy0 : halton_dim<3 + 5 * b, SMALL, GEO == kGeoPairClu>(s.i, sv.htab) * 2.0f - 1.0f;
 #if RT_CENSUS == 5
     {
         const f3 o2 = cz(s.o), dd = cz(s.d), N2 = cz(N), r2 = cz(right), f2 = cz(fwd), df = cz(diffuse);
@@ -161,8 +169,9 @@
     const f3 seg_hi{fmaxf(p.x, q.x), fmaxf(p.y, q.y), fmaxf(p.z, q.z)};
     f3 d2{0.0f, 0.0f, 0.0f};
     if (b + 1 < B) {
-        const float cu = halton_dim<4 + 5 * b, SMALL, GEO == kGeoPairClu>(s.i, sv.htab);
-        const float cv = halton_dim<5 + 5 * b, SMALL, GEO == kGeoPairClu>(s.i, sv.htab);
+        if constexpr (kRows) asm volatile("" : "+v"(s.i) : "v"(dist));
+        const float cu = halton_dim<4 + 5 * b, SMALL, GEO == kGeoPairClu, kHaltonHi>(s.i, sv.htab, sv.hhi);
+        const float cv = halton_dim<5 + 5 * b, SMALL, GEO == kGeoPairClu, kHaltonHi>(s.i, sv.htab, sv.hhi);
         float sp, cp;
         sincos_pt(6.28318548f * cu, &sp, &cp);
         const float ct = CR ? sqrt_cr(cv) : sqrtf(cv);
@@ -469,6 +478,7 @@
             const uint32_t tab0 = n.rec + n.clu;
             const bool tab = halton_tables_on(GEO, SMALL, P.spp, L);
             sv.htab = tab ? reinterpret_cast<const float*>(lds + tab0) : nullptr;
+            if constexpr (kHaltonHi) sv.hhi = P.halton_hi;
             if (tab) fill_halton_tables(reinterpret_cast<float*>(lds + tab0), threadIdx.x, NT);
         }
         __syncthreads();
@@ -571,7 +581,7 @@
             const float fx = (float)x, fy = (float)(P.row_start + j * P.row_step);
             s.i = seed_s[t] + n;
             const float jx = halton_dim<0, SMALL>(s.i);
-            const float jy = halton_dim<1, SMALL, GEO == kGeoPairClu>(s.i, sv.htab);
+            const float jy = halton_dim<1, SMALL, GEO == kGeoPairClu, kHaltonHi>(s.i, sv.htab, sv.hhi);
             s.d = camera_dir<GEO == kGeoTriBvh>(P, cu, cv, cw, fW, fH, fx, fy, jx, jy);
             s.o = ld_f3(P.cam_pos);
             s.thr = f3{1.0f, 1.0f, 1.0f};
@@ -579,7 +589,7 @@
             {
                 const uint32_t i2 = cz(s.i);
                 const float jx2 = halton_dim<0, SMALL>(i2);
-                const float jy2 = halton_dim<1, SMALL, GEO == kGeoPairClu>(i2, sv.htab);
+                const float jy2 = halton_dim<1, SMALL, GEO == kGeoPairClu, kHaltonHi>(i2, sv.htab, sv.hhi);
                 cz_sink(camera_dir(P, cu, cv, cw, fW, fH, cz(fx), cz(fy), jx2, jy2));
             }
 #endif
@@ -944,6 +954,7 @@
     const KernelChoice kc = choose_kernel(tables_of(P), P.sph_lds != nullptr, bounces, mem, P.walk);
     const int geo = kc.layout;
     const size_t lds_total = kc.lds_bytes;
+    if (kHaltonHi && geo == kGeoPairClu && P.halton_hi == nullptr) return hipErrorInvalidValue;
 #ifdef RT_LDS_UNDERSIZE
     const size_t lds_req = lds_total >= 16 ? lds_total - 16 : lds_total;
 #else
diff --git a/gpuraytracer_amd/csrc/rt_kernel.hpp b/gpuraytracer_amd/csrc/rt_kernel.hpp
--- a/gpuraytracer_amd/csrc/rt_kernel.hpp
+++ b/gpuraytracer_amd/csrc/rt_kernel.hpp
@@ -88,6 +88,7 @@
     uint32_t nC;
     uint32_t pair_free;
     uint64_t light_mask;
+    const float* halton_hi;
 };
 
 size_t kernel_lds_bytes(uint32_t n_tri, uint32_t n_pairs, uint32_t n_sph, uint32_t n_nodes);
@@ -221,6 +222,9 @@
                           size_t* temp_bytes, hipStream_t s);
 hipError_t scan_u32(const uint32_t* in, uint32_t* out, uint32_t n, uint32_t* tile_sums, hipStream_t s);
 
+hipError_t launch_halton_probe(const float* hi, uint32_t dim, const uint32_t* idx, uint32_t n, float* out,
+                               hipStream_t stream);
+
 hipError_t launch_fill_seeds(uint32_t* seeds, uint64_t key, uint64_t n, hipStream_t stream);
 hipError_t math_selfcheck(unsigned long long bad[2]);
 
diff --git a/gpuraytracer_amd/csrc/rt_trace.hpp b/gpuraytracer_amd/csrc/rt_trace.hpp
--- a/gpuraytracer_amd/csrc/rt_trace.hpp
+++ b/gpuraytracer_amd/csrc/rt_trace.hpp
@@ -133,6 +133,7 @@
     uint32_t shd_cskip = 0;
     bool shd_avail = false;
     const float* htab = nullptr;
+    const float* hhi = nullptr;
     const uint4* sent = nullptr;
     const uint16_t* sid = nullptr;
     const uint4* sbox = nullptr;
diff --git a/gpuraytracer_amd/host.py b/gpuraytracer_amd/host.py
--- a/gpuraytracer_amd/host.py
+++ b/gpuraytracer_amd/host.py
@@ -14,6 +14,29 @@
                       lib)
 
 DEFAULT_SEED_KEY = 0x5EED00000000
+
+
+def halton_hi_layout(dimension: int) -> dict:
+    from ._native import HaltonHiDim
+    info = HaltonHiDim()
+    _check(lib.rt_debug_halton_hi_layout(dimension, ctypes.byref(info)))
+    return {k: int(getattr(info, k)) for k, _ in HaltonHiDim._fields_}
+
+
+def halton_hi_table() -> np.ndarray:
+    n = ctypes.c_uint64()
+    _check(lib.rt_debug_halton_hi_table(None, 0, ctypes.byref(n)))
+    out = np.empty(n.value, np.float32)
+    _check(lib.rt_debug_halton_hi_table(out.ctypes.data_as(ctypes.c_void_p), n.value, ctypes.byref(n)))
+    return out
+
+
+def halton_hi_eval(dimension: int, indices, variant: int = 0) -> np.ndarray:
+    idx = np.ascontiguousarray(indices, dtype=np.uint32)
+    out = np.empty(idx.shape, np.float32)
+    _check(lib.rt_debug_halton_hi_eval(dimension, idx.ctypes.data_as(ctypes.c_void_p), idx.size, variant,
+                                       out.ctypes.data_as(ctypes.c_void_p)))
+    return out
 
 
 def _check(status: int, ctx=None):
@@ -571,6 +594,13 @@
         _check(lib.rt_last_launch(self._ctx, ctypes.byref(info)), self._ctx)
         return info.as_dict()
 
+    def halton_probe(self, dimension: int, indices) -> np.ndarray:
+        idx = np.ascontiguousarray(indices, dtype=np.uint32)
+        out = np.empty(idx.shape, np.float32)
+        _check(lib.rt_debug_halton_probe(self._ctx, dimension, idx.ctypes.data_as(ctypes.c_void_p), idx.size,
+                                         out.ctypes.data_as(ctypes.c_void_p)), self._ctx)
+        return out
+
     def build_info(self) -> dict:
         b = BuildStats()
         _check(lib.rt_build_info(self._ctx, ctypes.byref(b)), self._ctx)
diff --git a/include/rtpt.h b/include/rtpt.h
--- a/include/rtpt.h
+++ b/include/rtpt.h
@@ -280,6 +280,21 @@
 
 int rt_debug_light_mask(const rt_scene_desc* scene, uint64_t* mask, float* records, uint32_t capacity_triangles);
 
+typedef struct rt_halton_hi_dim {
+    uint32_t base;
+    uint32_t low_digits;
+    uint32_t high_digits;
+    uint32_t rows;
+    uint32_t row_stride;
+    uint32_t offset;
+    uint32_t is_low_table;
+    uint32_t used;
+} rt_halton_hi_dim;
+int rt_debug_halton_hi_layout(uint32_t dimension, rt_halton_hi_dim* info);
+int rt_debug_halton_hi_table(float* out, uint64_t capacity_floats, uint64_t* n_floats);
+int rt_debug_halton_hi_eval(uint32_t dimension, const uint32_t* indices, uint64_t n, uint32_t variant, float* out);
+int rt_debug_halton_probe(rt_ctx* ctx, uint32_t dimension, const uint32_t* indices, uint32_t n, float* out);
+
 void rt_tonemap_rgba8(const float* rgba32f, size_t n_pixels, uint8_t* rgba8);
 
 #ifdef __cplusplus
```

Measured after the change: 28850 Msamples/s, median of 6. Within noise of the previous version (+0.3%).
